# yblin/instant-ngp

Hardware: AMD Instinct MI355X
Metric: training samples/sec + PSNR@30s, NeRF Lego at 1/2/4/8 MI355X (higher is better)
Workload: dtype f16; 1 GPU; NerfNetwork training pass, C2 (configs/nerf/base.json fork: L=4 F=4 T=2^19, density 1x64 + rgb 2x64 fp16 MLPs), fwd+bwd+Adam/EMA; batch_per_gpu=262144, global_batch=262144, parallelism=dp1, launch=hip_graph

## Files before the change

### instant-ngp_amd/csrc/engine.hip

```cpp
#include <algorithm>
#include <cmath>
#include <cstring>
#include <memory>
#include <string>

#include "../../include/ngp_engine.h"
#include "common.h"
#include "engine_internal.h"
#include "grid_scatter.h"
#include "grid.h"
#include "json.h"
#include "mlp.h"
#include "optimizer.h"
#include "profiler.h"
#include "training.h"

static_assert(ngp::DENSITY_LAYOUT_ROW0 == ngp::MLP_LAYOUT_ROW0, "the row-0 density layout of mlp.h and engine_internal.h");

namespace ngp {

int device_cu_count() {
	static int cached = -1;
	if (cached < 0) {
		int dev = 0;
		NGP_HIP(hipGetDevice(&dev));
		NGP_HIP(hipDeviceGetAttribute(&cached, hipDeviceAttributeMultiprocessorCount, dev));
	}
	return cached;
}

struct DevBuf {
	void* p = nullptr;
	size_t bytes = 0;
	uint64_t* epoch = nullptr;
	void* get(size_t need) {
		if (need > bytes) {
			if (p) NGP_HIP(hipFree(p));
			p = nullptr;
			NGP_HIP(hipMalloc(&p, need));
			NGP_HIP(hipMemset(p, 0, need));
			bytes = need;
			if (epoch) ++*epoch;
		}
		return p;
	}
	~DevBuf() { if (p) (void)hipFree(p); }
};

struct Pcg32 {
	uint64_t state = 0x853c49e6748fea9bULL, inc = 0xda3e39cb94b95bdbULL;
	static constexpr uint64_t MULT = 0x5851f42d4c957f2dULL;
	Pcg32(uint64_t initstate, uint64_t initseq = 1u) {
		state = 0u; inc = (initseq << 1u) | 1u; next_uint(); state += initstate; next_uint();
	}
	uint32_t next_uint() {
		uint64_t old = state;
		state = old * MULT + inc;
		uint32_t xs = (uint32_t)(((old >> 18u) ^ old) >> 27u), rot = (uint32_t)(old >> 59u);
		return (xs >> rot) | (xs << ((~rot + 1u) & 31));
	}
	float next_float() { uint32_t u = (next_uint() >> 9) | 0x3f800000u; float f; memcpy(&f, &u, 4); return f - 1.0f; }
	void advance(uint64_t delta) {
		uint64_t cm = MULT, cp = inc, am = 1u, ap = 0u;
		while (delta > 0) {
			if (delta & 1) { am *= cm; ap = ap * cm + cp; }
			cp = (cm + 1) * cp; cm *= cm; delta /= 2;
		}
		state = am * state + ap;
	}
	void uniform(size_t n, float* out, float lo, float hi) {
		Pcg32 r = *this;
		for (size_t k = 0; k < n; ++k) out[k] = r.next_float() * (hi - lo) + lo;
		advance(n);
	}
};

static void init_mlp(const MlpDims& d, Pcg32& rng, float* p, float scale) {
	for (uint32_t l = 0; l <= d.n_hidden; ++l) {
		const uint32_t in = d.layer_in(l), out = d.layer_out(l);
		const float s = sqrtf(6.0f / (float)(in + out)) * scale;
		rng.uniform((size_t)in * out, p + d.layer_off(l), -s, s);
	}
}

static GridDesc parse_grid(uint32_t n_dims, const Json& j) {
	const std::string ot = j.string_or("otype", "HashGrid");
	NGP_CHECK(iequals(ot, "HashGrid") || iequals(ot, "DenseGrid") || iequals(ot, "Grid"),
	          "encoding: HashGrid and DenseGrid are implemented (got " + ot + ")");
	const std::string type = j.string_or("type", iequals(ot, "DenseGrid") ? "Dense" : "Hash");
	NGP_CHECK(iequals(type, "Hash") || iequals(type, "Dense"), "encoding: grid type Hash or Dense (got " + type + ")");
	NGP_CHECK(iequals(j.string_or("interpolation", "Linear"), "Linear"), "encoding: only linear interpolation is implemented");
	GridDesc g;
	grid_desc_init(g, n_dims, (uint32_t)j.number_or("n_levels", 16), (uint32_t)j.number_or("n_features_per_level", 2),
	               iequals(type, "Dense") ? GRID_LOG2_DENSE : (uint32_t)j.number_or("log2_hashmap_size", 19),
	               (uint32_t)j.number_or("base_resolution", 16), (float)j.number_or("per_level_scale", 2.0));
	return g;
}

static uint32_t parse_mlp_hidden(const Json& j, uint32_t* width) {
	const std::string ot = j.string_or("otype", "FullyFusedMLP");
	NGP_CHECK(iequals(ot, "FullyFusedMLP") || iequals(ot, "CutlassMLP") || iequals(ot, "MegakernelMLP"),
	          "network: only FullyFusedMLP-shaped networks are implemented (got " + ot + ")");
	NGP_CHECK(iequals(j.string_or("activation", "ReLU"), "ReLU"), "network: only ReLU hidden activation is implemented");
	NGP_CHECK(iequals(j.string_or("output_activation", "None"), "None"), "network: only output_activation None is implemented");
	*width = (uint32_t)j.number_or("n_neurons", 64);
	return (uint32_t)j.number_or("n_hidden_layers", 2);
}

}

using namespace ngp;

struct ngp_ctx {
	uint32_t n;
	const float* input;
	uint32_t input_stride;
	bool use_inference_params;
	uint64_t generation;
	bool density_only = false;
};

namespace ngp {
struct BwdExtra {
	float* dL_dinput = nullptr;
	uint32_t dinput_stride = 0;
	float dinput_scale = 1.f;
	bool density_only = false;
	const f16* ddens = nullptr;
	uint32_t ddens_stride = 0;
	bool inference = false;
};
}

struct ngp_model {
	bool nerf = true;
	GridDesc grid;
	uint32_t n_pos_dims = 3, n_dir_dims = 3, n_extra_dims = 0, dir_offset = 4, n_input_dims = 3, n_output_dims = 4;
	uint32_t enc_width = 16;
	NerfMlpPlan nplan;
	MlpPlan mplan;
	uint64_t mlp0_params = 0, mlp1_params = 0, grid_params = 0, n_params = 0;
	FragDesc* d_descs = nullptr;
	uint32_t* d_fragmap = nullptr;
	bool frags_current = false;
	uint32_t n_all_frags = 0;
	DevBuf frags, frags_inf, enc, denc, slabs, scatter_ws, out_ws, dl_ws, dsh_ws, dl1_ws;
	int grid_backward_mode = 0;
	uint32_t win_debug = 0;
	ScatterPlan sc_plan;
	uint32_t sc_plan_n = 0;
	bool sc_prepared = false;
	bool sc_hist_done = false;
	bool frags_async = false;
	uint32_t overlap = 0;
	bool fused_hist = true;
	bool fuse_infer = true;
	bool fuse_slabs = true;
	bool fuse_opt = true;
	bool fuse_mlp_opt = true;
	bool grid_bricks = false;
	hipStream_t side = nullptr;
	hipEvent_t ev_fork = nullptr, ev_join = nullptr, ev_frags = nullptr, ev_mlp = nullptr, ev_red = nullptr;
	f16 *params = nullptr, *inference_params = nullptr, *gradients = nullptr;
	void (*inference_hook)(void*, hipStream_t) = nullptr;
	void* inference_hook_ctx = nullptr;
	void sync_inference(hipStream_t s) { if (inference_hook) inference_hook(inference_hook_ctx, s); }
	float max_level = 1.0f;
	const float* max_level_per_sample = nullptr;
	bool grads_valid = true;
	const BwdParts* bwd_parts = nullptr;
	bool parts_ok(uint32_t n) const {
		return use_sorted(n) && fuse_slabs && !(overlap & 4) && !grid_bricks && grid.n_features >= 2;
	}
	uint64_t generation = 0;
	uint64_t ws_epoch = 0;
	std::unique_ptr<ngp_ctx> last_ctx;

	ngp_model() {
		for (DevBuf* b : {&frags, &frags_inf, &enc, &denc, &slabs, &scatter_ws, &out_ws, &dl_ws, &dsh_ws, &dl1_ws}) b->epoch = &ws_epoch;
	}

	~ngp_model() {
		if (d_descs) (void)hipFree(d_descs);
		if (d_fragmap) (void)hipFree(d_fragmap);
		for (hipEvent_t e : {ev_fork, ev_join, ev_frags, ev_mlp, ev_red})
			if (e) (void)hipEventDestroy(e);
		if (side) (void)hipStreamDestroy(side);
	}
	void reserve(uint32_t n) {
		enc.get((size_t)n * enc_width * sizeof(f16));
		denc.get((size_t)n * enc_width * sizeof(f16));
		const uint32_t blocks = nerf ? nerf_mlp_train_blocks(n) : mlp_train_blocks(n);
		slabs.get((size_t)blocks * n_matrix() * sizeof(float));
		frags.get((size_t)n_all_frags * 1024);
		frags_inf.get((size_t)n_all_frags * 1024);
		if (use_sorted(n)) {
			sorted_workspace(n);
			ensure_side_stream();
		}
	}
	void ensure_side_stream() {
		if (side) return;
		NGP_HIP(hipStreamCreateWithFlags(&side, hipStreamNonBlocking));
		NGP_HIP(hipEventCreateWithFlags(&ev_fork, hipEventDisableTiming));
		NGP_HIP(hipEventCreateWithFlags(&ev_join, hipEventDisableTiming));
		NGP_HIP(hipEventCreateWithFlags(&ev_frags, hipEventDisableTiming));
		NGP_HIP(hipEventCreateWithFlags(&ev_mlp, hipEventDisableTiming));
		NGP_HIP(hipEventCreateWithFlags(&ev_red, hipEventDisableTiming));
	}
	bool use_sorted(uint32_t n) const { return grid_backward_mode == 3 || (grid_backward_mode == 0 && n >= 4096); }
	bool grad32_ok(uint32_t n) const { return use_sorted(n) && fuse_slabs && !(overlap & 4) && grid.n_features >= 2; }
	bool side_prepare(uint32_t n) const { return use_sorted(n) && (overlap & 1); }
	const ScatterPlan& sc_plan_for(uint32_t n) {
		if (sc_plan_n != n) {
			sc_plan = make_scatter_plan(grid, n, grid_bricks);
			sc_plan_n = n;
			fb_dirty = true;
		}
		return sc_plan;
	}
	bool fb_dirty = true;
	void clear_brick_fallback(hipStream_t s, void* ws) {
		if (!fb_dirty) return;
		if (sc_plan.bk.LD) NGP_HIP(hipMemsetAsync((char*)ws + sc_plan.off_fb, 0, sc_plan.total - sc_plan.off_fb, s));
		fb_dirty = false;
	}
	void* sorted_workspace(uint32_t n) { return scatter_ws.get(sc_plan_for(n).total); }
	void prepare_grid_backward_async(hipStream_t s, uint32_t n, const float* in, uint32_t stride) {
		if (!side_prepare(n)) return;
		ensure_side_stream();
		void* ws = sorted_workspace(n);
		clear_brick_fallback(s, ws);
		GridBwdArgs b{n, in, stride, nullptr, 0, AoS, nullptr, max_level, max_level_per_sample};
		NGP_HIP(hipEventRecord(ev_fork, s));
		NGP_HIP(hipStreamWaitEvent(side, ev_fork, 0));
		if ((overlap & 2) && !frags_current) {
			prep(side, false);
			NGP_HIP(hipEventRecord(ev_frags, side));
			frags_async = true;
		}
		{
			ProfScope ps("grid_bwd_prepare", side);
			grid_scatter_prepare(grid, b, sc_plan, ws, side);
		}
		NGP_HIP(hipEventRecord(ev_join, side));
		sc_prepared = true;
	}

	const std::vector<FragDesc>& descs() const { return nerf ? nplan.descs : mplan.descs; }
	uint64_t grid_offset() const { return mlp0_params + mlp1_params; }
	uint64_t n_matrix() const { return mlp0_params + mlp1_params; }

	void finalize() {
		grid_params = grid.n_params();
		n_params = mlp0_params + mlp1_params + grid_params;
		const auto& d = descs();
		n_all_frags = (uint32_t)d.size();
		NGP_HIP(hipMalloc(&d_descs, d.size() * sizeof(FragDesc)));
		NGP_HIP(hipMemcpy(d_descs, d.data(), d.size() * sizeof(FragDesc), hipMemcpyHostToDevice));
		std::vector<uint32_t> map(2 * n_matrix(), ~0u);
		for (uint32_t f = 0; f < n_all_frags; ++f)
			for (uint32_t lane = 0; lane < 64; ++lane)
				for (uint32_t j = 0; j < 8; ++j) {
					const FragDesc& q = d[f];
					const uint32_t h = lane >> 5, r = 32 * q.tile + (lane & 31);
					const uint32_t k = q.perm ? 16 * q.step + 8 * (j >> 2) + 4 * h + (j & 3) : 16 * q.step + 8 * h + j;
					uint64_t pi;
					if (!q.transposed) {
						if (!(r < q.out_dim && k < q.in_dim)) continue;
						pi = q.woff + (uint64_t)r * q.in_dim + k;
					} else {
						if (!(r < q.in_dim && k < q.out_dim)) continue;
						pi = q.woff + (uint64_t)k * q.in_dim + r;
					}
					NGP_CHECK(pi < n_matrix() && map[2 * pi + q.transposed] == ~0u, "fragment map: parameter mapped twice");
					map[2 * pi + q.transposed] = (f * 64 + lane) * 8 + j;
				}
		NGP_HIP(hipMalloc(&d_fragmap, map.size() * sizeof(uint32_t)));
		NGP_HIP(hipMemcpy(d_fragmap, map.data(), map.size() * sizeof(uint32_t), hipMemcpyHostToDevice));
	}
	void require_params(bool inference) const {
		NGP_CHECK(inference ? inference_params != nullptr : params != nullptr,
		          "model has no parameters: call ngp_model_set_params or create a trainer first");
	}
	const f16* pick(bool inference) const { return inference ? inference_params : params; }
	bool fused_encoding_ok() const {
		return nerf && !max_level_per_sample && nerf_mlp_fused_encoding_ok(grid, enc_width) && nplan.enc_steps == 1 &&
		       nplan.d_hidden == 1 && nplan.r_hidden >= 1 && nplan.r_hidden <= 3;
	}
	bool fused_inference_ok() const { return fuse_infer && fused_encoding_ok(); }
	f16x8* prep(hipStream_t s, bool inference) {
		f16x8* f = (f16x8*)(inference ? frags_inf : frags).get((size_t)n_all_frags * 1024);
		if (inference) sync_inference(s);
		ProfScope ps("prepare_frags", s);
		prepare_frags(d_descs, n_all_frags, pick(inference), f, s);
		if (!inference) frags_current = true;
		return f;
	}
	void encode(hipStream_t s, uint32_t n, const float* in, uint32_t stride, f16* out, uint32_t out_stride, uint32_t layout, bool inference,
	            bool want_hist = false) {
		if (inference) sync_inference(s);
		GridFwdArgs a{n, in, stride, pick(inference) + grid_offset(), out, out_stride, layout, max_level, max_level_per_sample};
		if (enc_width > grid.n_levels * grid.n_features && layout == AoS && !grid_forward_rows_ok(grid, a)) {
			NGP_HIP(hipMemsetAsync(out, 0, (size_t)n * out_stride * sizeof(f16), s));
		}
		sc_hist_done = false;
		GridHist h;
		const bool fuse = want_hist && fused_hist && use_sorted(n) && !sc_prepared && grid_forward_rows_ok(grid, a) &&
		                  scatter_hist(grid, sc_plan_for(n), sorted_workspace(n), h);
		ProfScope ps("grid_forward", s);
		grid_forward(grid, a, s, fuse ? &h : nullptr);
		sc_hist_done = fuse;
	}
	void run_mlp(hipStream_t s, MlpMode mode, uint32_t n, const float* in, uint32_t stride, const f16* encbuf, f16* out,
	             uint32_t out_stride, uint32_t out_layout, const f16* dL, uint32_t dL_stride, f16* dL_denc, float* slab,
	             bool inference, const BwdExtra* ex = nullptr, f16* dL_dsh = nullptr) {
		f16x8* f;
		if (frags_async && !inference) {
			f = (f16x8*)frags.p;
			NGP_HIP(hipStreamWaitEvent(s, ev_frags, 0));
			frags_async = false;
		} else if (!inference && frags_current && frags.p) {
			f = (f16x8*)frags.p;
		} else {
			f = prep(s, inference);
		}
		if (nerf) {
			NerfMlpArgs a{};
			a.n = n; a.enc = encbuf; a.enc_stride = enc_width; a.coords = in; a.coord_stride = stride; a.dir_offset = dir_offset;
			a.frags = f; a.n_frags = n_all_frags; a.out = out; a.out_stride = out_stride; a.out_layout = out_layout;
			a.dL_dout = dL; a.dL_stride = dL_stride; a.dL_denc = dL_denc; a.denc_stride = enc_width; a.dw_slab = slab;
			a.n_matrix = (uint32_t)n_matrix(); a.density_woff = 0; a.rgb_woff = (uint32_t)mlp0_params;
			a.dL_dsh = dL_dsh;
			if (ex) { a.dL_ddens = ex->ddens; a.ddens_stride = ex->ddens_stride; }
			if (mode == MLP_INFER_ENC) {
				if (inference) sync_inference(s);
				a.table = pick(inference) + grid_offset(); a.max_level = max_level; a.gc = make_grid_const(grid);
			}
			ProfScope ps(mode == MLP_TRAIN ? "mlp_train" : mode == MLP_DENSITY ? "mlp_density"
			             : mode == MLP_INFER_ENC ? "mlp_infer_enc"
			             : mode == MLP_DENSITY_TRAIN ? "mlp_density_train" : "mlp_infer", s);
			nerf_mlp_run(nplan, mode, a, s);
		} else {
			MlpArgs a{};
			a.n = n; a.enc = encbuf; a.enc_stride = enc_width; a.frags = f; a.n_frags = n_all_frags;
			a.out = out; a.out_stride = out_stride; a.out_layout = out_layout; a.dL_dout = dL; a.dL_stride = dL_stride;
			a.dL_denc = dL_denc; a.denc_stride = enc_width; a.dw_slab = slab; a.n_matrix = (uint32_t)n_matrix();
			ProfScope ps(mode == MLP_TRAIN ? "mlp_train" : "mlp_infer", s);
			mlp_run(mplan, mode == MLP_DENSITY ? MLP_INFER : mode, a, s);
		}
	}
	void train_pass(hipStream_t s, uint32_t n, const float* in, uint32_t stride, const f16* encbuf, f16* out, uint32_t out_stride,
	                const void* dL, uint32_t dL_stride, int grad_mode, const BwdExtra& ex = BwdExtra{}, const FusedAdam* fopt = nullptr) {
		NGP_CHECK(gradients || grad_mode == NGP_GRAD_IGNORE, "model has no gradient buffer: call ngp_model_set_params");
		NGP_CHECK(!ex.density_only || (nerf && encbuf), "density backward: a NerfNetwork with its encoding");
		f16* dL_denc = (f16*)denc.get((size_t)n * enc_width * sizeof(f16));
		const uint32_t blocks = nerf ? nerf_mlp_train_blocks(n) : mlp_train_blocks(n);
		float* slab = (float*)slabs.get((size_t)blocks * n_matrix() * sizeof(float));
		f16* dsh = ex.dL_dinput && nerf && !ex.density_only ? (f16*)dsh_ws.get((size_t)n * 16 * sizeof(f16)) : nullptr;
		NGP_CHECK(encbuf, "train_pass: the encoding buffer");
		const MlpMode mode = ex.density_only ? MLP_DENSITY_TRAIN : MLP_TRAIN;
		run_mlp(s, mode, n, in, stride, encbuf, out, out_stride, AoS, (const f16*)dL, dL_stride, dL_denc, slab, ex.inference, &ex,
		        dsh);
		auto input_gradient = [&]() {
			if (!ex.dL_dinput) return;
			ProfScope ps("input_gradient", s);
			if (ex.inference) sync_inference(s);
			InputGradArgs ia{n, in, stride, pick(ex.inference) + grid_offset(), dL_denc, enc_width, max_level, max_level_per_sample, dsh,
			                 dir_offset, ex.dL_dinput, ex.dinput_stride, ex.dinput_scale};
			grid_input_gradient(grid, ia, s);
		};
		if (grad_mode == NGP_GRAD_IGNORE) {
			input_gradient();
			return;
		}
		grads_valid = !(fopt && (fopt->rec || fopt->g32));
		const bool ovl = use_sorted(n) && (overlap & 4);
		const bool fused = use_sorted(n) && !ovl && fuse_slabs && !ex.density_only;
		const uint32_t n_red = ex.density_only ? (uint32_t)mlp0_params : (uint32_t)n_matrix();
		SlabJob sj;
		sj.slabs = slab; sj.n_slabs = blocks; sj.n = n_red; sj.grad = gradients; sj.stride = (uint32_t)n_matrix();
		sj.accumulate = grad_mode == NGP_GRAD_ACCUMULATE;
		FusedAdam f32store;
		if (fopt && fopt->g32) {
			NGP_CHECK(fused && grad_mode == NGP_GRAD_OVERWRITE && !fopt->rec, "fp32 gradient store: fused slab reduction");
			sj.grad32 = fopt->g32;
			f32store.g32 = fopt->g32 + grid_offset();
			fopt = &f32store;
		}
		hipStream_t rs = s;
		if (ovl) {
			ensure_side_stream();
			NGP_HIP(hipEventRecord(ev_mlp, s));
			NGP_HIP(hipStreamWaitEvent(side, ev_mlp, 0));
			rs = side;
		}
		if (!fused) {
			ProfScope ps("reduce_slabs", rs);
			reduce_slabs(slab, blocks, n_red, gradients, grad_mode == NGP_GRAD_ACCUMULATE, rs, (uint32_t)n_matrix());
		}
		if (ovl) NGP_HIP(hipEventRecord(ev_red, side));
		GridBwdArgs b{n, in, stride, dL_denc, enc_width, AoS, gradients + grid_offset(), max_level, max_level_per_sample};
		FusedAdam fmlp;
		if (fopt && fopt->mlp_n) {
			NGP_CHECK(fused && grad_mode == NGP_GRAD_OVERWRITE && fopt->mlp_n == n_matrix(), "fused MLP update: slab reduction not fused");
			fmlp = *fopt;
			fmlp.frags = frags_current ? (f16*)frags.p : nullptr;
			fmlp.fragmap = d_fragmap;
			fopt = &fmlp;
		}
		scatter_grid_grad(s, b, grad_mode != NGP_GRAD_ACCUMULATE, fused ? &sj : nullptr, fopt);
		if (ovl) NGP_HIP(hipStreamWaitEvent(s, ev_red, 0));
		input_gradient();
	}
	void scatter_grid_grad(hipStream_t s, GridBwdArgs b, bool overwrite, const SlabJob* slab = nullptr, const FusedAdam* fopt = nullptr) {
		if (use_sorted(b.n)) {
			void* ws = sorted_workspace(b.n);
			clear_brick_fallback(s, ws);
			if (sc_prepared) {
				NGP_HIP(hipStreamWaitEvent(s, ev_join, 0));
				sc_prepared = false;
			} else {
				ProfScope ps("grid_bwd_prepare", s);
				grid_scatter_prepare(grid, b, sc_plan, ws, s, sc_hist_done);
			}
			sc_hist_done = false;
			ProfScope ps(fopt && fopt->rec ? "grid_backward_adam" : "grid_backward_sorted", s);
			grid_backward_sorted(grid, b, sc_plan, ws, s, overwrite, win_debug, slab, fopt,
			                     bwd_parts && !sc_plan.bk.LD && !(fopt && fopt->rec) ? bwd_parts : nullptr);
			return;
		}
		NGP_CHECK(!slab && !fopt, "fused slab reduction / optimizer need the sorted grid backward");
		if (overwrite) {
			ProfScope ps("grid_grad_zero", s);
			NGP_HIP(hipMemsetAsync(b.grad, 0, grid_params * sizeof(f16), s));
		}
		ProfScope ps("grid_backward", s);
		grid_backward(grid, b, s);
	}
};

struct ngp_trainer {
	ngp_model* model = nullptr;
	AdamConfig cfg;
	uint32_t step = 0;
	uint64_t n = 0;
	void* arena = nullptr;
	float *w32 = nullptr, *m1 = nullptr, *m2 = nullptr, *ema32 = nullptr;
	f16 *w16 = nullptr, *inf16 = nullptr, *g16 = nullptr;
	uint32_t* steps = nullptr;
	float* bias_tab = nullptr;
	AdamRec* rec = nullptr;
	bool inf_stale = false;
	bool w32_stale = false;
	void sync_w32() {
		if (!rec || !w32_stale) return;
		require_full_state("full-precision weights");
		NGP_HIP(hipDeviceSynchronize());
		adam_rec_weights((uint32_t)n, rec, w32, false, nullptr);
		NGP_HIP(hipDeviceSynchronize());
		w32_stale = false;
	}
	void materialize(hipStream_t s, bool force = false) {
		if (!rec || (!inf_stale && !force)) return;
		require_full_state("inference (EMA) parameters");
		AdamState st{w32, w16, g16, nullptr, nullptr, nullptr, nullptr, inf16, nullptr, nullptr, nullptr, 0, nullptr, rec};
		ema_materialize(cfg, (uint32_t)n, step, st, s);
		inf_stale = false;
	}
	static void materialize_hook(void* self, hipStream_t s) { ((ngp_trainer*)self)->materialize(s); }
	void bind_model() {
		ngp_model_set_params(model, w16, cfg.ema_decay > 0.f ? inf16 : w16, g16);
		if (rec) { model->inference_hook = materialize_hook; model->inference_hook_ctx = this; }
	}
	uint32_t* ctl = nullptr;
	ngp_allreduce_fn allreduce = nullptr;
	void* allreduce_user = nullptr;
	uint32_t world = 1;
	static constexpr uint64_t SHARD_PAD = 2048;
	uint32_t dp_rank = 0;
	bool dp_rank_known = false;
	bool shard_opt = true;
	bool shards_valid = true;
	float* g32 = nullptr;
	uint64_t g32_count = 0;
	uint64_t n_pad = 0;
	uint32_t dp_parts = 1;
	bool dp_wire16 = false;
	std::vector<uint64_t> pb;
	hipStream_t xs = nullptr;
	hipEvent_t ev_part[BwdParts::MAX] = {}, ev_xs = nullptr;
	struct PartStep {
		hipStream_t s = nullptr;
		ngp::Exchange e;
		float loss_scale = 1.f;
		const uint32_t* step_base = nullptr;
		uint32_t step_add = 0;
		bool wire16 = false, overlap = false;
		uint32_t issued = 0;
		int rc = NGP_OK;
	} ps_;
	BwdParts bparts;
	~ngp_trainer() {
		if (arena) (void)hipFree(arena);
		if (bias_tab) (void)hipFree(bias_tab);
		if (g32) (void)hipFree(g32);
		for (hipEvent_t ev : ev_part)
			if (ev) (void)hipEventDestroy(ev);
		if (ev_xs) (void)hipEventDestroy(ev_xs);
		if (xs) (void)hipStreamDestroy(xs);
	}
	ngp::Exchange exchange() const {
		ngp::Exchange e;
		e.fn = allreduce; e.user = allreduce_user; e.rank = dp_rank; e.world = world; e.world_factor = (float)world;
		e.rank_known = dp_rank_known;
		return e;
	}
	bool sharded(const ngp::Exchange& e) const {
// ... 62 lines not shown
	}
	static void part_done(void* self, uint32_t j, hipStream_t) { ((ngp_trainer*)self)->issue_part(j); }
	const BwdParts* begin_shard_step(hipStream_t s, float loss_scale, const ngp::Exchange& e, const uint32_t* step_base,
	                                 uint32_t step_add, uint32_t n_batch, bool stores_input) {
		ps_ = PartStep{};
		ps_.s = s; ps_.e = e; ps_.loss_scale = loss_scale; ps_.step_base = step_base; ps_.step_add = step_add;
		ps_.wire16 = dp_wire16;
		ngp_model* m = model;
		if (pb.size() < 3 || !m->parts_ok(n_batch) || !(stores_input || dp_wire16)) return nullptr;
		ensure_exchange_stream();
		ps_.overlap = true;
		const ScatterPlan& p = m->sc_plan_for(n_batch);
		if (p.bk.LD || pb[1] < m->grid_offset()) { ps_.overlap = false; return nullptr; }
		bparts = BwdParts{};
		bparts.k = (uint32_t)pb.size() - 1;
		const uint64_t go = m->grid_offset();
		for (uint32_t j = 0; j < bparts.k; ++j)
			bparts.vb_end[j] = j + 1 == bparts.k ? p.n_buckets : scatter_bucket_at_param(m->grid, p, pb[j + 1] > go ? pb[j + 1] - go : 0);
		bparts.after = part_done;
		bparts.user = this;
		return &bparts;
	}
	int shard_step(bool stored) {
		PartStep& q = ps_;
		hipStream_t s = q.s;
		ngp_model* m = model;
		if (q.issued == 0) {
			q.overlap = false;
			if (!stored && !q.wire16) widen_f16(g16, g32, n, s);
		}
		while (q.rc == NGP_OK && q.issued + 1 < pb.size()) issue_part((uint32_t)pb.size() - 2 - q.issued);
		if (q.rc != NGP_OK) return NGP_ERROR;
		if (q.overlap) {
			NGP_HIP(hipEventRecord(ev_xs, xs));
			NGP_HIP(hipStreamWaitEvent(s, ev_xs, 0));
		}
		if (!mlp_owned() && m->n_matrix() > 0) m->prep(s, false);
		inf_stale = w32_stale = true;
		if (q.e.world > 1) shards_valid = false;
		return NGP_OK;
	}
	void sync_device_step() { NGP_HIP(hipMemcpy(ctl, &step, sizeof(uint32_t), hipMemcpyHostToDevice)); }
	void run_step(hipStream_t s, float loss_scale, const uint32_t* step_base, uint32_t step_add, uint64_t n_first = 0) {
		ngp_model* m = model;
		const bool own = m->params == w16;
		AdamState st{w32, w16, g16, m1, m2, steps, ema32, inf16,
		             own && m->frags_current ? (f16*)m->frags.p : nullptr, m->d_fragmap, step_base, step_add,
		             step_base ? (const AdamConfig*)(ctl + CTL_CFG) : nullptr, rec, bias_tab};
		ProfScope ps("optimizer", s);
		adam_ema_update(cfg, (uint32_t)(n_first ? n_first : n), (uint32_t)m->n_matrix(), loss_scale, st, s);
		if (rec) inf_stale = w32_stale = true;
	}
	bool fused_update_ok(uint32_t n_batch) const {
		const ngp_model* m = model;
		return rec && !allreduce && m->fuse_opt && m->use_sorted(n_batch) && m->grid.n_features >= 2 && m->n_matrix() % 4 == 0 &&
		       m->grid_offset() % 2 == 0 && m->params == w16 && m->gradients == g16;
	}
	FusedAdam fused_update(float loss_scale, uint32_t n_batch) const {
		FusedAdam fa;
		const uint64_t go = model->grid_offset();
		fa.w16 = w16 + go; fa.rec = rec + go / 2;
		fa.loss_scale = loss_scale; fa.cfg = cfg; fa.step_add = step;
		fa.bias_tab = bias_tab;
		if (mlp_opt_in_backward(n_batch)) {
			fa.mlp_n = (uint32_t)model->n_matrix();
			fa.mlp_w16 = w16;
			fa.mlp_rec = rec;
		}
		return fa;
	}
	bool mlp_opt_in_backward(uint32_t n_batch) const {
		const ngp_model* m = model;
		return m->fuse_mlp_opt && m->fuse_slabs && !(m->overlap & 4) && m->use_sorted(n_batch) && m->n_matrix() > 0;
	}
	void mlp_step_done() {
		if (rec) inf_stale = w32_stale = true;
	}
};

struct ngp_graph {
	hipGraph_t graph = nullptr;
	hipGraphExec_t exec = nullptr;
	ngp_trainer* trainer = nullptr;
	uint32_t steps_per_launch = 1;
	uint64_t ws_epoch = 0;
	bool shards_stale = false;
	bool g16_stale = false;
	void launched() {
		trainer->step += steps_per_launch;
		if (steps_per_launch && trainer->rec) trainer->inf_stale = trainer->w32_stale = true;
		if (shards_stale) trainer->shards_valid = false;
		if (g16_stale) trainer->model->grads_valid = false;
	}
	~ngp_graph() {
		if (exec) (void)hipGraphExecDestroy(exec);
		if (graph) (void)hipGraphDestroy(graph);
	}
};

__global__ static void k_one_hot_f16(f16* out, uint32_t n, uint32_t width, uint32_t dim, f16 v) {
	const uint64_t i = blockIdx.x * (uint64_t)blockDim.x + threadIdx.x;
	if (i < (uint64_t)n * width) out[i] = (i % width) == dim ? v : (f16)0.f;
}
static void fill_one_hot_f16(f16* out, uint32_t n, uint32_t width, uint32_t dim, float v, hipStream_t s) {
	k_one_hot_f16<<<div_round_up((uint64_t)n * width, 256), 256, 0, s>>>(out, n, width, dim, (f16)v);
	NGP_HIP(hipGetLastError());
}

static thread_local std::string g_last_error;

#define NGP_TRY(...)                        \
	try {                                   \
		__VA_ARGS__;                        \
		return NGP_OK;                      \
	} catch (const std::exception& e) {     \
		g_last_error = e.what();            \
		return NGP_ERROR;                   \
	}

#define NGP_ARG(cond)                                                          \
	do {                                                                       \
		if (!(cond)) { g_last_error = "invalid argument: " #cond; return NGP_INVALID; } \
	} while (0)

static hipStream_t S(void* s) { return (hipStream_t)s; }

namespace ngp {
void set_last_error(const char* msg) { g_last_error = msg; }
}

extern "C" {

const char* ngp_last_error(void) { return g_last_error.c_str(); }
const char* ngp_version(void) { return "ngp-mi355x 0.1 (gfx950)"; }

int ngp_device_info(int* cu_count, char* name, size_t name_len) {
	NGP_TRY({
		int dev = 0;
		NGP_HIP(hipGetDevice(&dev));
		hipDeviceProp_t p;
		NGP_HIP(hipGetDeviceProperties(&p, dev));
		if (cu_count) *cu_count = p.multiProcessorCount;
		if (name && name_len) { strncpy(name, p.gcnArchName, name_len - 1); name[name_len - 1] = 0; }
	});
}

int ngp_malloc(void** ptr, size_t bytes) { NGP_ARG(ptr); NGP_TRY(NGP_HIP(hipMalloc(ptr, bytes))); }
int ngp_free(void* ptr) { NGP_TRY(NGP_HIP(hipFree(ptr))); }
int ngp_memcpy(void* dst, const void* src, size_t bytes, int kind) { NGP_TRY(NGP_HIP(hipMemcpy(dst, src, bytes, (hipMemcpyKind)kind))); }
int ngp_stream_synchronize(void* stream) { NGP_TRY(NGP_HIP(hipStreamSynchronize(S(stream)))); }

static void apply_env_options(ngp_model* m) {
	const char* env = getenv("NGP_MODEL_OPTS");
	if (!env || !*env) return;
	std::string all = env;
	size_t pos = 0;
	while (pos < all.size()) {
		size_t end = all.find(',', pos);
		if (end == std::string::npos) end = all.size();
		const std::string kv = all.substr(pos, end - pos);
		pos = end + 1;
		if (kv.empty()) continue;
		const size_t eq = kv.find('=');
		NGP_CHECK(eq != std::string::npos, "NGP_MODEL_OPTS: expected key=value, got " + kv);
		if (ngp_model_set_option(m, kv.substr(0, eq).c_str(), atof(kv.c_str() + eq + 1)) != NGP_OK) throw Error(g_last_error);
	}
}

int ngp_nerf_network_create(uint32_t n_pos_dims, uint32_t n_dir_dims, uint32_t n_extra_dims, uint32_t dir_offset,
                            const char* pos_encoding_json, const char* dir_encoding_json, const char* density_network_json,
                            const char* rgb_network_json, ngp_model** out) {
	NGP_ARG(out && pos_encoding_json && density_network_json && rgb_network_json);
	NGP_TRY({
		auto m = std::make_unique<ngp_model>();
		m->nerf = true;
		NGP_CHECK(n_pos_dims == 3, "NerfNetwork: n_pos_dims must be 3");
		NGP_CHECK(n_dir_dims == 3, "NerfNetwork: n_dir_dims must be 3");
		NGP_CHECK(n_extra_dims == 0, "NerfNetwork: extra dims (latent codes) are not implemented");
		m->n_pos_dims = n_pos_dims; m->n_dir_dims = n_dir_dims; m->n_extra_dims = n_extra_dims; m->dir_offset = dir_offset;
		m->grid = parse_grid(3, Json::parse(pos_encoding_json));
		if (dir_encoding_json) {
			Json d = Json::parse(dir_encoding_json);
			const Json* sh = &d;
			if (iequals(d.string_or("otype", ""), "Composite")) sh = &d["nested"].arr.at(0);
			NGP_CHECK(iequals(sh->string_or("otype", ""), "SphericalHarmonics") && (int)sh->number_or("degree", 4) == 4,
			          "NerfNetwork: dir_encoding must be SphericalHarmonics of degree 4");
		}
		uint32_t wd, wr;
		const uint32_t dh = parse_mlp_hidden(Json::parse(density_network_json), &wd);
		const uint32_t rh = parse_mlp_hidden(Json::parse(rgb_network_json), &wr);
		NGP_CHECK(wd == wr, "NerfNetwork: density and rgb networks must share n_neurons");
		m->enc_width = next_multiple(m->grid.n_levels * m->grid.n_features, 16);
		m->nplan = make_nerf_mlp_plan(m->enc_width, wd, dh, rh);
		m->mlp0_params = m->nplan.density.n_params();
		m->mlp1_params = m->nplan.rgb.n_params();
		m->n_input_dims = dir_offset + n_dir_dims + n_extra_dims;
		m->n_output_dims = 4;
		m->finalize();
		apply_env_options(m.get());
		*out = m.release();
	});
}

int ngp_network_with_input_encoding_create(uint32_t n_input_dims, uint32_t n_output_dims, const char* encoding_json,
                                           const char* network_json, ngp_model** out) {
	NGP_ARG(out && encoding_json && network_json);
	NGP_TRY({
		auto m = std::make_unique<ngp_model>();
		m->nerf = false;
		NGP_CHECK(n_input_dims == 2 || n_input_dims == 3, "NetworkWithInputEncoding: 2 or 3 input dims");
		NGP_CHECK(n_output_dims >= 1 && n_output_dims <= 16, "NetworkWithInputEncoding: 1..16 outputs");
		m->n_pos_dims = n_input_dims; m->n_input_dims = n_input_dims; m->n_output_dims = n_output_dims;
		m->grid = parse_grid(n_input_dims, Json::parse(encoding_json));
		uint32_t w;
		const uint32_t hid = parse_mlp_hidden(Json::parse(network_json), &w);
		m->enc_width = next_multiple(m->grid.n_levels * m->grid.n_features, 16);
		m->mplan = make_mlp_plan(m->enc_width, w, hid, 16);
		m->mlp0_params = m->mplan.mlp.n_params();
		m->mlp1_params = 0;
		m->finalize();
		apply_env_options(m.get());
		*out = m.release();
	});
}

void ngp_model_destroy(ngp_model* m) { delete m; }
uint64_t ngp_model_n_params(const ngp_model* m) { return m ? m->n_params : 0; }
uint64_t ngp_model_n_matrix_params(const ngp_model* m) { return m ? m->n_matrix() : 0; }
uint32_t ngp_model_input_width(const ngp_model* m) { return m ? m->n_input_dims : 0; }
uint32_t ngp_model_padded_output_width(const ngp_model* m) { return m ? 16 : 0; }
uint32_t ngp_model_output_width(const ngp_model* m) { return m ? m->n_output_dims : 0; }

int ngp_model_param_layout(const ngp_model* m, ngp_param_layout* o) {
	NGP_ARG(m && o);
	NGP_TRY({
		memset(o, 0, sizeof(*o));
		o->density_mlp_offset = 0; o->density_mlp_params = m->mlp0_params;
		o->rgb_mlp_offset = m->mlp0_params; o->rgb_mlp_params = m->mlp1_params;
		o->grid_offset = m->grid_offset(); o->grid_params = m->grid_params;
		o->grid_dims = m->grid.n_dims; o->grid_levels = m->grid.n_levels; o->grid_features = m->grid.n_features;
		o->grid_log2_hashmap = m->grid.log2_hashmap; o->grid_base_resolution = m->grid.base_resolution;
		o->grid_per_level_scale = m->grid.per_level_scale;
		memcpy(o->grid_level_offsets, m->grid.offsets, sizeof(o->grid_level_offsets));
		memcpy(o->grid_resolution, m->grid.resolution, sizeof(o->grid_resolution));
		memcpy(o->grid_scale, m->grid.scale, sizeof(o->grid_scale));
		o->encoding_width = m->enc_width;
	});
}

int ngp_model_set_params(ngp_model* m, void* params, void* inference_params, void* gradients) {
	NGP_ARG(m);
	NGP_TRY({
		m->inference_hook = nullptr;
		m->inference_hook_ctx = nullptr;
		m->params = (f16*)params;
		m->frags_current = false;
		m->inference_params = (f16*)(inference_params ? inference_params : params);
		m->gradients = (f16*)gradients;
	});
}

int ngp_model_initialize_params(const ngp_model* m, uint64_t seed, float* p, float scale) {
	NGP_ARG(m && p);
	NGP_TRY({
		Pcg32 rng(seed);
		if (m->nerf) {
			init_mlp(m->nplan.density, rng, p, scale);
			init_mlp(m->nplan.rgb, rng, p + m->mlp0_params, scale);
		} else {
			init_mlp(m->mplan.mlp, rng, p, scale);
		}
		rng.uniform(m->grid_params, p + m->grid_offset(), -1e-4f * scale, 1e-4f * scale);
	});
}

int ngp_model_set_max_level(ngp_model* m, float max_level, const float* per_sample) {
	NGP_ARG(m);
	NGP_TRY({ m->max_level = max_level; m->max_level_per_sample = per_sample; });
}

int ngp_model_set_option(ngp_model* m, const char* key, double value) {
	NGP_ARG(m && key);
	NGP_TRY({
		const std::string k = key;
		if (k == "grid_backward_mode") {
			NGP_CHECK(value == 0 || value == 1 || value == 3, "grid_backward_mode must be 0 (auto), 1 (direct), 3 (bucketed)");
			m->grid_backward_mode = (int)value;
		} else if (k == "overlap") {
			NGP_CHECK(value >= 0 && value <= 15, "overlap is a bitmask in [0, 15]");
			m->overlap = (uint32_t)value;
		} else if (k == "fused_hist") {
			m->fused_hist = value != 0;
		} else if (k == "fuse_infer") {
			m->fuse_infer = value != 0;
		} else if (k == "fuse_slabs") {
			m->fuse_slabs = value != 0;
		} else if (k == "fuse_opt") {
			m->fuse_opt = value != 0;
		} else if (k == "fuse_mlp_opt") {
			m->fuse_mlp_opt = value != 0;
		} else if (k == "grid_bricks") {
			m->grid_bricks = value != 0;
			m->sc_plan_n = 0;
		} else if (k == "win_debug") {
			m->win_debug = (uint32_t)value;
		} else {
			throw Error("unknown model option: " + k);
		}
		++m->ws_epoch;
	});
}

int ngp_model_query(const ngp_model* m, const char* key, double* value) {
	NGP_ARG(m && key && value);
	NGP_TRY({
		const std::string k = key;
		if (k == "grid_brick_levels") *value = m->sc_plan_n ? (double)(m->sc_plan.bk.LD - m->sc_plan.bk.LB) : 0.0;
		else throw Error("unknown model query: " + k);
	});
}

int ngp_model_reserve(ngp_model* m, uint32_t n) {
	NGP_ARG(m);
	NGP_TRY({ m->reserve(n); });
}

uint64_t ngp_model_workspace_epoch(const ngp_model* m) { return m ? m->ws_epoch : 0; }

int ngp_model_workspace(ngp_model* m, const char* name, void** ptr, uint64_t* bytes) {
	NGP_ARG(m && name && ptr);
	NGP_TRY({
		const std::string k(name);
		DevBuf* b = k == "encoding" ? &m->enc : k == "dL_dencoding" ? &m->denc : k == "dw_slabs" ? &m->slabs
		          : k == "dL_dsh" ? &m->dsh_ws : nullptr;
		NGP_CHECK(b, "ngp_model_workspace: unknown workspace '" + k + "' (encoding, dL_dencoding, dL_dsh, dw_slabs)");
		*ptr = b->p;
		if (bytes) *bytes = b->bytes;
	});
}

int ngp_encoding_forward(ngp_model* m, void* stream, uint32_t n, const float* input, uint32_t input_stride, void* output,
                         uint32_t output_stride, uint32_t output_layout, int use_inference_params) {
	NGP_ARG(m && (n == 0 || (input && output)) && output_layout <= 1);
	NGP_TRY({
		m->require_params(use_inference_params);
		m->encode(S(stream), n, input, input_stride, (f16*)output, output_stride, output_layout, use_inference_params);
	});
}

int ngp_encoding_backward(ngp_model* m, void* stream, uint32_t n, const float* input, uint32_t input_stride,
                          const void* dL_doutput, uint32_t dL_stride, uint32_t dL_layout, float* dL_dinput,
                          uint32_t dL_dinput_stride, int grad_mode) {
	NGP_ARG(m && (n == 0 || (input && dL_doutput)) && dL_layout <= 1 && grad_mode >= 0 && grad_mode <= NGP_GRAD_IGNORE);
	NGP_ARG(!dL_dinput || (dL_layout == NGP_LAYOUT_AOS && dL_dinput_stride >= m->grid.n_dims));
	NGP_TRY({
		if (n == 0) return NGP_OK;
		m->require_params(false);
		if (grad_mode != NGP_GRAD_IGNORE) {
			NGP_CHECK(m->gradients, "model has no gradient buffer");
			GridBwdArgs b{n, input, input_stride, (const f16*)dL_doutput, dL_stride, dL_layout, m->gradients + m->grid_offset(),
			              m->max_level, m->max_level_per_sample};
			m->scatter_grid_grad(S(stream), b, grad_mode != NGP_GRAD_ACCUMULATE);
		}
		if (dL_dinput) {
			ProfScope ps("input_gradient", S(stream));
			InputGradArgs ia{n, input, input_stride, m->params + m->grid_offset(), (const f16*)dL_doutput, dL_stride, m->max_level,
			                 m->max_level_per_sample, nullptr, 0, dL_dinput, dL_dinput_stride, 1.f};
			grid_input_gradient(m->grid, ia, S(stream));
		}
	});
}

}
int ngp::density_impl(ngp_model* m, void* stream, uint32_t n, const float* input, uint32_t input_stride, void* output,
                      uint32_t output_stride, uint32_t output_layout, int use_inference_params) {
	NGP_TRY({
		NGP_CHECK(m->nerf, "density() is a NerfNetwork method");
		if (n == 0) return NGP_OK;
		m->require_params(use_inference_params);
		f16* e = (f16*)m->enc.get((size_t)n * m->enc_width * sizeof(f16));
		m->encode(S(stream), n, input, input_stride, e, m->enc_width, AoS, use_inference_params);
		m->run_mlp(S(stream), MLP_DENSITY, n, input, input_stride, e, (f16*)output, output_stride, output_layout, nullptr, 0,
		           nullptr, nullptr, use_inference_params);
		m->generation++;
	});
}
extern "C" {

int ngp_inference(ngp_model* m, void* stream, uint32_t n, const float* input, uint32_t input_stride, void* output,
                  uint32_t output_stride, uint32_t output_layout, int use_inference_params) {
	NGP_ARG(m && (n == 0 || (input && output)) && (output_layout <= 1 || (output_layout == NGP_LAYOUT_AOS_RGBD && m->nerf &&
	                                                                        output_stride >= 4)));
	NGP_TRY({
		if (n == 0) return NGP_OK;
		m->require_params(use_inference_params);
		if (m->fused_inference_ok()) {
			m->run_mlp(S(stream), MLP_INFER_ENC, n, input, input_stride, nullptr, (f16*)output, output_stride, output_layout,
			           nullptr, 0, nullptr, nullptr, use_inference_params);
		} else {
			f16* e = (f16*)m->enc.get((size_t)n * m->enc_width * sizeof(f16));
			m->encode(S(stream), n, input, input_stride, e, m->enc_width, AoS, use_inference_params);
			m->run_mlp(S(stream), MLP_INFER, n, input, input_stride, e, (f16*)output, output_stride, output_layout, nullptr, 0,
			           nullptr, nullptr, use_inference_params);
		}
		m->generation++;
	});
}

int ngp_density(ngp_model* m, void* stream, uint32_t n, const float* input, uint32_t input_stride, void* output,
                uint32_t output_stride, uint32_t output_layout, int use_inference_params) {
	NGP_ARG(m && (n == 0 || (input && output)) && output_layout <= 1);
	return ngp::density_impl(m, stream, n, input, input_stride, output, output_stride, output_layout, use_inference_params);
}

int ngp_forward(ngp_model* m, void* stream, uint32_t n, const float* input, uint32_t input_stride, void* output,
                uint32_t output_stride, int use_inference_params, ngp_ctx** ctx) {
	NGP_ARG(m && ctx && (n == 0 || input));
	NGP_TRY({
		m->require_params(use_inference_params);
		f16* e = (f16*)m->enc.get((size_t)(n ? n : 1) * m->enc_width * sizeof(f16));
		m->generation++;
		if (n) {
			m->encode(S(stream), n, input, input_stride, e, m->enc_width, AoS, use_inference_params);
			if (output)
				m->run_mlp(S(stream), MLP_INFER, n, input, input_stride, e, (f16*)output, output_stride, AoS, nullptr, 0, nullptr,
				           nullptr, use_inference_params);
		}
		*ctx = new ngp_ctx{n, input, input_stride, (bool)use_inference_params, m->generation};
	});
}

static int check_dinput(const ngp_model* m, float* dL_dinput, uint32_t stride) {
	if (!dL_dinput) return NGP_OK;
	const uint32_t need = m->nerf ? m->dir_offset + 3 : m->n_pos_dims;
	if (stride < need) {
		g_last_error = "dL_dinput: stride smaller than the rows the input gradient writes";
		return NGP_INVALID;
	}
	return NGP_OK;
}

int ngp_backward(ngp_model* m, void* stream, ngp_ctx* ctx, const void* dL_doutput, uint32_t dL_stride, float* dL_dinput,
                 uint32_t dL_dinput_stride, int grad_mode) {
	NGP_ARG(m && ctx && (ctx->n == 0 || dL_doutput) && grad_mode >= 0 && grad_mode <= NGP_GRAD_IGNORE);
	if (check_dinput(m, dL_dinput, dL_dinput_stride) != NGP_OK) return NGP_INVALID;
	NGP_TRY({
		NGP_CHECK(ctx->generation == m->generation,
		          "backward: the forward context is stale (another forward/inference ran on this model since)");
		NGP_CHECK(!ctx->density_only, "backward: this context is from density_forward (use density_backward)");
		if (ctx->n == 0) return NGP_OK;
		BwdExtra ex;
		ex.dL_dinput = dL_dinput; ex.dinput_stride = dL_dinput_stride;
		ex.inference = ctx->use_inference_params;
		m->train_pass(S(stream), ctx->n, ctx->input, ctx->input_stride, (const f16*)m->enc.p, nullptr, 0, dL_doutput, dL_stride,
		              grad_mode, ex);
	});
}

int ngp_density_forward(ngp_model* m, void* stream, uint32_t n, const float* input, uint32_t input_stride, void* output,
                        uint32_t output_stride, int use_inference_params, ngp_ctx** ctx) {
	NGP_ARG(m && ctx && (n == 0 || input) && (!output || output_stride >= 16));
	NGP_TRY({
		NGP_CHECK(m->nerf, "density_forward is a NerfNetwork method");
		m->require_params(use_inference_params);
		f16* e = (f16*)m->enc.get((size_t)(n ? n : 1) * m->enc_width * sizeof(f16));
		m->generation++;
		if (n) {
			m->encode(S(stream), n, input, input_stride, e, m->enc_width, AoS, use_inference_params);
			if (output)
				m->run_mlp(S(stream), MLP_DENSITY, n, input, input_stride, e, (f16*)output, output_stride, AoS, nullptr, 0, nullptr,
				           nullptr, use_inference_params);
		}
		*ctx = new ngp_ctx{n, input, input_stride, (bool)use_inference_params, m->generation, true};
	});
}

int ngp_density_backward(ngp_model* m, void* stream, ngp_ctx* ctx, const void* dL_doutput, uint32_t dL_stride, float* dL_dinput,
                         uint32_t dL_dinput_stride, int grad_mode) {
	NGP_ARG(m && ctx && (ctx->n == 0 || dL_doutput) && dL_stride >= 16 && dL_stride % 4 == 0 && grad_mode >= 0 &&
	        grad_mode <= NGP_GRAD_IGNORE && (!dL_dinput || dL_dinput_stride >= 3));
	NGP_TRY({
		NGP_CHECK(m->nerf, "density_backward is a NerfNetwork method");
		NGP_CHECK(ctx->generation == m->generation,
		          "density_backward: the forward context is stale (another forward/inference ran on this model since)");
		NGP_CHECK(ctx->density_only, "density_backward: this context is from forward (use backward)");
		if (ctx->n == 0) return NGP_OK;
		BwdExtra ex;
		ex.dL_dinput = dL_dinput; ex.dinput_stride = dL_dinput_stride;
		ex.density_only = true; ex.ddens = (const f16*)dL_doutput; ex.ddens_stride = dL_stride;
		ex.inference = ctx->use_inference_params;
		m->train_pass(S(stream), ctx->n, ctx->input, ctx->input_stride, (const f16*)m->enc.p, nullptr, 0, nullptr, 0, grad_mode, ex);
	});
}

int ngp_input_gradient(ngp_model* m, void* stream, uint32_t dim, uint32_t n, const float* input, uint32_t input_stride,
                       float* d_dinput, uint32_t d_dinput_stride, float backprop_scale) {
	NGP_ARG(m && (n == 0 || (input && d_dinput)) && dim < 16 && backprop_scale != 0.f);
	if (check_dinput(m, d_dinput, d_dinput_stride) != NGP_OK) return NGP_INVALID;
	NGP_TRY({
		if (n == 0) return NGP_OK;
		m->require_params(false);
		hipStream_t s = S(stream);
		f16* e = (f16*)m->enc.get((size_t)n * m->enc_width * sizeof(f16));
		f16* dl = (f16*)m->dl1_ws.get((size_t)n * 16 * sizeof(f16));
		m->generation++;
		m->encode(s, n, input, input_stride, e, m->enc_width, AoS, false);
		fill_one_hot_f16(dl, n, 16, dim, backprop_scale, s);
		BwdExtra ex;
		ex.dL_dinput = d_dinput; ex.dinput_stride = d_dinput_stride; ex.dinput_scale = 1.f / backprop_scale;
		m->train_pass(s, n, input, input_stride, e, nullptr, 0, dl, 16, NGP_GRAD_IGNORE, ex);
	});
}

void ngp_ctx_destroy(ngp_ctx* ctx) { delete ctx; }

int ngp_forward_backward(ngp_model* m, void* stream, uint32_t n, const float* input, uint32_t input_stride, void* output,
                         uint32_t output_stride, const void* dL_doutput, uint32_t dL_stride, int grad_mode) {
	return ngp::forward_backward_with(m, stream, n, input, input_stride, output, output_stride, dL_doutput, dL_stride, grad_mode,
	                                  nullptr);
}
}

int ngp::forward_backward_with(ngp_model* m, void* stream, uint32_t n, const float* input, uint32_t input_stride, void* output,
                               uint32_t output_stride, const void* dL_doutput, uint32_t dL_stride, int grad_mode,
                               const FusedAdam* fopt) {
	NGP_ARG(m && (n == 0 || (input && dL_doutput)));
	NGP_TRY({
		if (n == 0) return NGP_OK;
		m->require_params(false);
		f16* e = (f16*)m->enc.get((size_t)n * m->enc_width * sizeof(f16));
		m->generation++;
		m->prepare_grid_backward_async(S(stream), n, input, input_stride);
		m->encode(S(stream), n, input, input_stride, e, m->enc_width, AoS, false, true);
		m->train_pass(S(stream), n, input, input_stride, e, (f16*)output, output_stride, dL_doutput, dL_stride, grad_mode,
		              BwdExtra{}, fopt);
	});
}
extern "C" {

static void parse_optimizer(const Json& j, AdamConfig& c) {
	const std::string ot = j.string_or("otype", "Adam");
	if (iequals(ot, "Ema")) {
		c.ema_decay = (float)j.number_or("decay", 0.99);
		parse_optimizer(j["nested"], c);
	} else if (iequals(ot, "ExponentialDecay")) {
		c.decay_start = (uint32_t)j.number_or("decay_start", 0);
		c.decay_interval = (uint32_t)j.number_or("decay_interval", 10000);
		c.decay_base = (float)j.number_or("decay_base", 0.1);
		parse_optimizer(j["nested"], c);
	} else if (iequals(ot, "Adam")) {
		c.lr = (float)j.number_or("learning_rate", 1e-3);
		c.beta1 = (float)j.number_or("beta1", 0.9);
		c.beta2 = (float)j.number_or("beta2", 0.999);
		c.eps = (float)j.number_or("epsilon", 1e-8);
		c.l2 = (float)j.number_or("l2_reg", 1e-8);
	} else {
		throw Error("optimizer: unsupported otype " + ot + " (Ema / ExponentialDecay / Adam implemented)");
	}
}

int ngp_trainer_create(ngp_model* m, const char* optimizer_json, uint64_t seed, ngp_trainer** out) {
	NGP_ARG(m && out);
	NGP_TRY({
		auto t = std::make_unique<ngp_trainer>();
		t->model = m;
		if (optimizer_json) parse_optimizer(Json::parse(optimizer_json), t->cfg);
		if (const char* e = getenv("NGP_EMA_CLOSED_FORM")) t->cfg.ema_closed_form = atoi(e) != 0;
		NGP_HIP(hipMalloc(&t->bias_tab, (size_t)BIAS_TAB_CAP * 2 * sizeof(float)));
		adam_bias_table(t->bias_tab, t->cfg.beta1, t->cfg.beta2, nullptr);
		NGP_HIP(hipDeviceSynchronize());
		const uint64_t n = m->n_params;
		t->n = n;
		auto al = [](size_t b) { return (b + 255) / 256 * 256; };
		const size_t b32 = al(n * 4), b16 = al((n + ngp_trainer::SHARD_PAD) * 2);
		bool lazy = n >= (1ull << 20);
		if (const char* e = getenv("NGP_LAZY_EMA")) lazy = atoi(e) != 0;
		lazy = lazy && n % 4 == 0;
		const size_t brec = al((n + ngp_trainer::SHARD_PAD) / 2 * sizeof(AdamRec));
		const size_t total = b32 + (lazy ? brec : 4 * b32) + 3 * b16 + 256 ;
		NGP_HIP(hipMalloc(&t->arena, total));
		char* p = (char*)t->arena;
		t->w32 = (float*)p; p += b32;
		if (lazy) {
			t->rec = (AdamRec*)p; p += brec;
		} else {
			t->m1 = (float*)p; p += b32;
			t->m2 = (float*)p; p += b32;
			t->ema32 = (float*)p; p += b32;
			t->steps = (uint32_t*)p; p += b32;
		}
		t->w16 = (f16*)p; p += b16;
		t->inf16 = (f16*)p; p += b16;
		t->g16 = (f16*)p; p += b16;
		t->ctl = (uint32_t*)p; p += 256;
		NGP_HIP(hipMemset(t->arena, 0, total));
		std::vector<float> host(n);
		if (ngp_model_initialize_params(m, seed, host.data(), 1.0f) != NGP_OK) throw Error(g_last_error);
		*out = t.release();
		if (ngp_trainer_set_params_full_precision(*out, host.data(), n) != NGP_OK) throw Error(g_last_error);
	});
}

void ngp_trainer_destroy(ngp_trainer* t) {
	if (!t) return;
	if (t->model && t->model->params == t->w16) ngp_model_set_params(t->model, nullptr, nullptr, nullptr);
	delete t;
}

int ngp_trainer_optimizer_step(ngp_trainer* t, void* stream, float loss_scale) {
	NGP_ARG(t && loss_scale > 0.f);
	NGP_TRY({
		t->run_step(S(stream), loss_scale, nullptr, t->step);
		t->step++;
	});
}

int ngp_loss_evaluate(int loss_type, void* stream, uint32_t n, uint32_t dims, const void* output, uint32_t output_stride,
                      const float* target, uint32_t target_stride, float loss_scale, void* dL_doutput, uint32_t dL_stride,
                      float* values, float* loss_sum) {
	NGP_ARG(loss_type >= 0 && (n == 0 || (output && target && dL_doutput)));
// ... 403 lines not shown
```

### instant-ngp_amd/csrc/grid.h

```cpp
#pragma once
#include "common.h"

namespace ngp {

struct GridDesc {
	uint32_t n_dims = 3, n_levels = 16, n_features = 2, log2_hashmap = 19, base_resolution = 16;
	float per_level_scale = 2.0f;
	uint32_t offsets[33] = {};
	float scale[32] = {};
	uint32_t resolution[32] = {};
	uint32_t n_entries() const { return offsets[n_levels]; }
	uint64_t n_params() const { return (uint64_t)offsets[n_levels] * n_features; }
};

constexpr uint32_t GRID_LOG2_DENSE = 31;
void grid_desc_init(GridDesc& g, uint32_t D, uint32_t L, uint32_t F, uint32_t log2T, uint32_t Nmin, float b);

enum Layout : uint32_t { AoS = 0, SoA = 1 };

struct GridFwdArgs {
	uint32_t n;
	const float* pos;
	uint32_t pos_stride;
	const f16* table;
	f16* out;
	uint32_t out_stride;
	uint32_t out_layout;
	float max_level;
	const float* max_level_per_sample;
};

struct GridBwdArgs {
	uint32_t n;
	const float* pos;
	uint32_t pos_stride;
	const f16* dL_dy;
	uint32_t dy_stride;
	uint32_t dy_layout;
	f16* grad;
	float max_level;
	const float* max_level_per_sample;
	uint32_t level_begin = 0;
};

struct GridHist {
	uint32_t* hist;
	uint32_t B, n_chunks, chunk;
	uint32_t vb_base[33];
	uint32_t brick_first = 0, brick_levels = 0, n_bricks = 0, brick_cells = 8, bricks_per_dim = 0, brick_vb0 = 0;
};

void grid_forward(const GridDesc& g, const GridFwdArgs& a, hipStream_t stream, const GridHist* hist = nullptr);
bool grid_forward_rows_ok(const GridDesc& g, const GridFwdArgs& a);
void grid_backward(const GridDesc& g, const GridBwdArgs& a, hipStream_t stream);

struct InputGradArgs {
	uint32_t n;
	const float* pos; uint32_t pos_stride;
	const f16* table;
	const f16* dL_dy; uint32_t dy_stride;
	float max_level; const float* max_level_per_sample;
	const f16* dL_dsh;
	uint32_t dir_offset;
	float* out; uint32_t out_stride;
	float out_scale;
};
void grid_input_gradient(const GridDesc& g, const InputGradArgs& a, hipStream_t stream);

struct GridConst {
	uint32_t n_levels, n_features;
	uint32_t offsets[33];
	float scale[32];
	uint32_t resolution[32];
	uint32_t hashed;
};

__device__ __forceinline__ uint32_t grid_index3(uint32_t T, uint32_t res, uint32_t x, uint32_t y, uint32_t z) {
	uint32_t stride = 1, index = 0;
	index += x * stride; stride *= res;
	if (stride <= T) { index += y * stride; stride *= res; }
	if (stride <= T) { index += z * stride; stride *= res; }
	if (T < stride) index = x ^ (y * 2654435761u) ^ (z * 805459861u);
	return index % T;
}

__device__ __forceinline__ uint32_t grid_index2(uint32_t T, uint32_t res, uint32_t x, uint32_t y) {
	uint32_t stride = 1, index = 0;
	index += x * stride; stride *= res;
	if (stride <= T) { index += y * stride; stride *= res; }
	if (T < stride) index = x ^ (y * 2654435761u);
	return index % T;
}

template <uint32_t D>
__device__ __forceinline__ uint32_t corner_index(const GridConst& c, uint32_t l, const uint32_t* base, uint32_t corner) {
	const uint32_t x = base[0] + (corner & 1u);
	const uint32_t y = base[1] + ((corner >> 1) & 1u);
	if ((c.hashed >> l) & 1u) {
		const uint32_t mask = c.offsets[l + 1] - c.offsets[l] - 1u;
		if constexpr (D == 3) {
			const uint32_t z = base[2] + ((corner >> 2) & 1u);
			return c.offsets[l] + ((x ^ (y * 2654435761u) ^ (z * 805459861u)) & mask);
		} else {
			return c.offsets[l] + ((x ^ (y * 2654435761u)) & mask);
		}
	}
	const uint32_t res = c.resolution[l];
	uint32_t idx;
	if constexpr (D == 3) {
		const uint32_t z = base[2] + ((corner >> 2) & 1u);
		idx = x + res * (y + res * z);
	} else {
		idx = x + res * y;
	}
	const uint32_t T = c.offsets[l + 1] - c.offsets[l];
	if (__builtin_expect(idx >= T, 0)) idx %= T;
	return c.offsets[l] + idx;
}

template <uint32_t D>
__device__ __forceinline__ void corner_indices(const GridConst& c, uint32_t l, const uint32_t* base, uint32_t* idx) {
	const uint32_t res = c.resolution[l], T = c.offsets[l + 1] - c.offsets[l];
	uint64_t vol = res;
#pragma unroll
	for (uint32_t d = 1; d < D; ++d) vol *= res;
	bool fast = !((c.hashed >> l) & 1u) && vol <= T;
#pragma unroll
	for (uint32_t d = 0; d < D; ++d) fast = fast && base[d] < res;
	if (__builtin_expect(fast, 1)) {
		const uint32_t r2 = res * res;
		const uint32_t i0 = D == 3 ? base[0] + res * (base[1] + res * base[2]) : base[0] + res * base[1];
#pragma unroll
		for (uint32_t k = 0; k < (1u << D); ++k) {
			const uint32_t id = i0 + (k & 1u) + (((k >> 1) & 1u) ? res : 0u) + ((D == 3 && ((k >> 2) & 1u)) ? r2 : 0u);
			idx[k] = c.offsets[l] + min(id, id - T);
		}
	} else {
#pragma unroll
		for (uint32_t k = 0; k < (1u << D); ++k) idx[k] = corner_index<D>(c, l, base, k);
	}
}

template <uint32_t F> struct GridVec;
template <> struct GridVec<1> { typedef f16 T; typedef f16 __attribute__((ext_vector_type(2), aligned(2))) P; };
template <> struct GridVec<2> { typedef f16x2 T; typedef f16 __attribute__((ext_vector_type(4), aligned(4))) P; };
template <> struct GridVec<4> { typedef f16x4 T; typedef f16 __attribute__((ext_vector_type(8), aligned(8))) P; };
template <> struct GridVec<8> { typedef f16x8 T; typedef f16x8 P; };

#ifndef NGP_GATHER16
#define NGP_GATHER16 0
#endif
template <uint32_t D>
__device__ __forceinline__ void gather_pairs_f2(const uint32_t* idx, const f16* __restrict__ table, f16x2* v);
template <uint32_t D, uint32_t F>
__device__ __forceinline__ void gather_corners(const GridConst& c, uint32_t l, const uint32_t* base, const f16* __restrict__ table,
                                               typename GridVec<F>::T* v) {
	typedef typename GridVec<F>::T V;
	typedef typename GridVec<F>::P P;
	if constexpr (F == 2 && NGP_GATHER16) {
		uint32_t idx[1u << D];
#pragma unroll
		for (uint32_t k = 0; k < (1u << D); ++k) idx[k] = corner_index<D>(c, l, base, k);
		gather_pairs_f2<D>(idx, table, v);
	} else if constexpr (F == 2 || F == 4) {
#pragma unroll
		for (uint32_t k = 0; k < (1u << D); k += 2) {
			const uint32_t i0 = corner_index<D>(c, l, base, k), i1 = corner_index<D>(c, l, base, k + 1);
			const uint32_t lo_i = min(i0, i1);
			if (max(i0, i1) == lo_i + 1u) {
				const P p = *(const P*)(table + (size_t)lo_i * F);
				V lo, hi;
#pragma unroll
				for (uint32_t f = 0; f < F; ++f) { lo[f] = p[f]; hi[f] = p[F + f]; }
				const bool swap = i1 < i0;
				v[k] = swap ? hi : lo;
				v[k + 1] = swap ? lo : hi;
			} else {
				v[k] = *(const V*)(table + (size_t)i0 * F);
				v[k + 1] = *(const V*)(table + (size_t)i1 * F);
			}
		}
	} else {
#pragma unroll
		for (uint32_t k = 0; k < (1u << D); ++k) v[k] = *(const V*)(table + (size_t)corner_index<D>(c, l, base, k) * F);
	}
}
__device__ __forceinline__ f16x2 pick4(const uint32_t (&g)[4], uint32_t i) {
	const uint32_t lo = (i & 1u) ? g[1] : g[0], hi = (i & 1u) ? g[3] : g[2];
	return __builtin_bit_cast(f16x2, (i & 2u) ? hi : lo);
}
template <uint32_t D>
__device__ __forceinline__ void gather_pairs_f2(const uint32_t* idx, const f16* __restrict__ table, f16x2* v) {
	typedef GridVec<2>::P P;
#pragma unroll
	for (uint32_t k = 0; k < (1u << D); k += 2) {
		const uint32_t i0 = idx[k], i1 = idx[k + 1];
		const uint32_t lo_i = min(i0, i1);
		if ((i0 >> 2) == (i1 >> 2)) {
			const uint32_t* gp = (const uint32_t*)(table + (size_t)(i0 & ~3u) * 2);
			typedef uint32_t u32x4g __attribute__((ext_vector_type(4)));
			const u32x4g q = *(const u32x4g*)gp;
			const uint32_t g[4] = {q[0], q[1], q[2], q[3]};
			v[k] = pick4(g, i0 & 3u);
			v[k + 1] = pick4(g, i1 & 3u);
		} else if (max(i0, i1) == lo_i + 1u) {
			const P p = *(const P*)(table + (size_t)lo_i * 2);
			const f16x2 a{p[0], p[1]}, b{p[2], p[3]};
			const bool swap = i1 < i0;
			v[k] = swap ? b : a;
			v[k + 1] = swap ? a : b;
		} else {
			v[k] = *(const f16x2*)(table + (size_t)i0 * 2);
			v[k + 1] = *(const f16x2*)(table + (size_t)i1 * 2);
		}
	}
}

template <uint32_t D, uint32_t F>
__device__ __forceinline__ void gather_corners_at(const uint32_t* idx, const f16* __restrict__ table, typename GridVec<F>::T* v) {
	typedef typename GridVec<F>::T V;
	typedef typename GridVec<F>::P P;
	if constexpr (F == 2 && NGP_GATHER16) {
		gather_pairs_f2<D>(idx, table, v);
	} else if constexpr (F == 2 || F == 4) {
#pragma unroll
		for (uint32_t k = 0; k < (1u << D); k += 2) {
			const uint32_t i0 = idx[k], i1 = idx[k + 1];
			const uint32_t lo_i = min(i0, i1);
			if (max(i0, i1) == lo_i + 1u) {
				const P p = *(const P*)(table + (size_t)lo_i * F);
				V lo, hi;
#pragma unroll
				for (uint32_t f = 0; f < F; ++f) { lo[f] = p[f]; hi[f] = p[F + f]; }
				const bool swap = i1 < i0;
				v[k] = swap ? hi : lo;
				v[k + 1] = swap ? lo : hi;
			} else {
				v[k] = *(const V*)(table + (size_t)i0 * F);
				v[k + 1] = *(const V*)(table + (size_t)i1 * F);
			}
		}
	} else {
#pragma unroll
		for (uint32_t k = 0; k < (1u << D); ++k) v[k] = *(const V*)(table + (size_t)idx[k] * F);
	}
}

template <uint32_t D>
__device__ __forceinline__ float corner_weight(const float* frac, uint32_t corner) {
	float w = 1.0f;
#pragma unroll
	for (uint32_t d = 0; d < D; ++d) w *= ((corner >> d) & 1u) ? frac[d] : 1.0f - frac[d];
	return w;
}

template <uint32_t D>
__device__ __forceinline__ void level_setup(const GridConst& c, uint32_t l, const float* x, float* frac, uint32_t* base) {
#pragma unroll
	for (uint32_t d = 0; d < D; ++d) {
		float p = __builtin_fmaf(c.scale[l], x[d], 0.5f);
		float t = floorf(p);
		base[d] = (uint32_t)(int)t;
		frac[d] = p - t;
	}
}

__device__ __forceinline__ uint32_t brick_of(const GridConst& c, uint32_t f, uint32_t K, uint32_t NB, const float* x) {
	uint32_t id = 0, mul = 1;
#pragma unroll
	for (uint32_t d = 0; d < 3; ++d) {
		const int cell = (int)floorf(__builtin_fmaf(c.scale[f], x[d], 0.5f));
		const int b = cell < 0 ? 0 : min(cell / (int)K, (int)NB - 1);
		id += (uint32_t)b * mul;
		mul *= NB;
	}
	return id;
}

__device__ __forceinline__ void hist_add(uint32_t* h, uint32_t j, uint32_t few_bits) {
	if (few_bits > 4) { atomicAdd(&h[j], 1u); return; }
	uint64_t peers = __ballot(1);
	for (uint32_t b = 0; b < few_bits; ++b) {
		const uint64_t m = __ballot((j >> b) & 1u);
		peers &= ((j >> b) & 1u) ? m : ~m;
	}
	if (__lane_id() == (uint32_t)(__ffsll((unsigned long long)peers) - 1)) atomicAdd(&h[j], (uint32_t)__popcll(peers));
}

GridConst make_grid_const(const GridDesc& g);
int device_cu_count();

}
```

### instant-ngp_amd/csrc/grid.hip

```cpp
#include "grid.h"

#include <algorithm>

#include <cmath>
#include <cstring>

namespace ngp {

void grid_desc_init(GridDesc& g, uint32_t D, uint32_t L, uint32_t F, uint32_t log2T, uint32_t Nmin, float b) {
	NGP_CHECK(D == 2 || D == 3, "GridEncoding: n_dims must be 2 or 3");
	NGP_CHECK(L >= 1 && L <= 32, "GridEncoding: n_levels must be in [1, 32]");
	NGP_CHECK(F == 1 || F == 2 || F == 4 || F == 8, "GridEncoding: n_features_per_level must be 1, 2, 4 or 8");
	NGP_CHECK((log2T >= 4 && log2T <= 28) || log2T == GRID_LOG2_DENSE, "GridEncoding: log2_hashmap_size out of range");
	g = GridDesc{};
	g.n_dims = D; g.n_levels = L; g.n_features = F; g.log2_hashmap = log2T; g.base_resolution = Nmin;
	g.per_level_scale = b;
	const float log2b = log2f(b);
	uint32_t off = 0;
	for (uint32_t l = 0; l < L; ++l) {
		float s = exp2f((float)l * log2b) * (float)Nmin - 1.0f;
		uint32_t res = (uint32_t)ceilf(s) + 1u;
		g.scale[l] = s;
		g.resolution[l] = res;
		const uint32_t max_params = 0xffffffffu / 2;
		uint32_t n;
		if (powf((float)res, (float)D) > (float)max_params) n = max_params;
		else { n = 1; for (uint32_t d = 0; d < D; ++d) n *= res; }
		n = (n + 7u) / 8u * 8u;
		if (n > (1u << log2T)) n = 1u << log2T;
		g.offsets[l] = off;
		off += n;
	}
	g.offsets[L] = off;
}

GridConst make_grid_const(const GridDesc& g) {
	GridConst c;
	c.n_levels = g.n_levels;
	c.n_features = g.n_features;
	memcpy(c.offsets, g.offsets, sizeof(c.offsets));
	memcpy(c.scale, g.scale, sizeof(c.scale));
	memcpy(c.resolution, g.resolution, sizeof(c.resolution));
	c.hashed = 0;
	for (uint32_t l = 0; l < g.n_levels; ++l) {
		const uint32_t T = g.offsets[l + 1] - g.offsets[l];
		uint32_t stride = g.resolution[l];
		for (uint32_t d = 1; d < g.n_dims; ++d)
			if (stride <= T) stride *= g.resolution[l];
		if (T < stride) {
			NGP_CHECK((T & (T - 1)) == 0, "GridEncoding: hashed level size must be a power of two");
			c.hashed |= 1u << l;
		}
	}
	return c;
}

template <uint32_t F> struct FeatVec;
template <> struct FeatVec<1> { typedef f16 T; };
template <> struct FeatVec<2> { typedef f16x2 T; };
template <> struct FeatVec<4> { typedef f16x4 T; };
template <> struct FeatVec<8> { typedef f16x8 T; };

template <uint32_t D, uint32_t F>
__global__ void __launch_bounds__(256) k_grid_forward(const GridConst c, const GridFwdArgs a) {
	typedef typename FeatVec<F>::T V;
	const uint32_t i = blockIdx.x * blockDim.x + threadIdx.x;
	if (i >= a.n) return;
	float x[D];
#pragma unroll
	for (uint32_t d = 0; d < D; ++d) x[d] = a.pos[(size_t)i * a.pos_stride + d];
	const float ml = (a.max_level_per_sample ? a.max_level_per_sample[i] : a.max_level) * (float)c.n_levels;
	for (uint32_t l = 0; l < c.n_levels; ++l) {
		float acc[F];
#pragma unroll
		for (uint32_t f = 0; f < F; ++f) acc[f] = 0.f;
		if (!((float)l >= ml + 1e-3f)) {
			float frac[D]; uint32_t base[D];
			level_setup<D>(c, l, x, frac, base);
			V v[1u << D];
			gather_corners<D, F>(c, l, base, a.table, v);
#pragma unroll
			for (uint32_t k = 0; k < (1u << D); ++k) {
				const float w = corner_weight<D>(frac, k);
				if constexpr (F == 1) acc[0] = __builtin_fmaf(w, (float)v[k], acc[0]);
				else {
#pragma unroll
					for (uint32_t f = 0; f < F; ++f) acc[f] = __builtin_fmaf(w, (float)v[k][f], acc[f]);
				}
			}
		}
#pragma unroll
		for (uint32_t f = 0; f < F; ++f) asm volatile("" : "+v"(acc[f]));
		if (a.out_layout == AoS) {
			V o;
			if constexpr (F == 1) o = (f16)acc[0];
			else {
#pragma unroll
				for (uint32_t f = 0; f < F; ++f) o[f] = (f16)acc[f];
			}
			*(V*)(a.out + (size_t)i * a.out_stride + l * F) = o;
		} else {
#pragma unroll
			for (uint32_t f = 0; f < F; ++f) a.out[(size_t)(l * F + f) * a.out_stride + i] = (f16)acc[f];
		}
	}
}

#ifndef NGP_FWD_FASTIDX
#define NGP_FWD_FASTIDX 1
#endif
template <uint32_t D, uint32_t F, bool HIST>
__global__ void __launch_bounds__(HIST ? 512 : 256) k_grid_forward_rows(const GridConst c, const GridFwdArgs a, const GridHist h) {
	typedef typename FeatVec<F>::T V;
	constexpr uint32_t MAXL = 32 / F;
	extern __shared__ __attribute__((aligned(16))) uint32_t hl[];
	if constexpr (HIST) {
		for (uint32_t j = threadIdx.x; j < h.vb_base[c.n_levels]; j += blockDim.x) hl[j] = 0;
		__syncthreads();
	}
	const uint32_t i = blockIdx.x * blockDim.x + threadIdx.x;
	if (i < a.n) {
	float x[D];
#pragma unroll
	for (uint32_t d = 0; d < D; ++d) x[d] = a.pos[(size_t)i * a.pos_stride + d];
	const float ml = (a.max_level_per_sample ? a.max_level_per_sample[i] : a.max_level) * (float)c.n_levels;
	if constexpr (HIST && D == 3) {
		if (h.brick_levels) atomicAdd(&hl[h.brick_vb0 + brick_of(c, h.brick_levels - 1, h.brick_cells, h.bricks_per_dim, x)], 1u);
	}
	f16 row[32];
#pragma unroll
	for (uint32_t l = 0; l < MAXL; ++l) {
		float acc[F];
#pragma unroll
		for (uint32_t f = 0; f < F; ++f) acc[f] = 0.f;
		const bool active = l < c.n_levels && !((float)l >= ml + 1e-3f);
		const bool count = HIST && !(l >= h.brick_first && l < h.brick_levels);
		if (count && l < c.n_levels && !active) {
			float frac[D]; uint32_t base[D];
			level_setup<D>(c, l, x, frac, base);
#pragma unroll
			for (uint32_t k = 0; k < (1u << D); ++k)
				atomicAdd(&hl[h.vb_base[l] + ((corner_index<D>(c, l, base, k) - c.offsets[l]) >> h.B)], 1u);
		}
		if (active) {
			float frac[D]; uint32_t base[D];
			level_setup<D>(c, l, x, frac, base);
			V v[1u << D];
			if constexpr (NGP_FWD_FASTIDX && F >= 4) {
				uint32_t cidx[1u << D];
				corner_indices<D>(c, l, base, cidx);
				if (count) {
#pragma unroll
					for (uint32_t k = 0; k < (1u << D); ++k) atomicAdd(&hl[h.vb_base[l] + ((cidx[k] - c.offsets[l]) >> h.B)], 1u);
				}
				gather_corners_at<D, F>(cidx, a.table, v);
			} else {
				if (count) {
#pragma unroll
					for (uint32_t k = 0; k < (1u << D); ++k)
						atomicAdd(&hl[h.vb_base[l] + ((corner_index<D>(c, l, base, k) - c.offsets[l]) >> h.B)], 1u);
				}
				gather_corners<D, F>(c, l, base, a.table, v);
			}
#pragma unroll
			for (uint32_t k = 0; k < (1u << D); ++k) {
				const float w = corner_weight<D>(frac, k);
				if constexpr (F == 1) acc[0] = __builtin_fmaf(w, (float)v[k], acc[0]);
				else {
#pragma unroll
					for (uint32_t f = 0; f < F; ++f) acc[f] = __builtin_fmaf(w, (float)v[k][f], acc[f]);
				}
			}
		}
#pragma unroll
		for (uint32_t f = 0; f < F; ++f) {
			asm volatile("" : "+v"(acc[f]));
			row[l * F + f] = (f16)acc[f];
		}
	}
	f16x8* dst = (f16x8*)(a.out + (size_t)i * a.out_stride);
#pragma unroll
	for (uint32_t q = 0; q < 4; ++q) {
		if (8 * q >= a.out_stride) break;
		dst[q] = f16x8{row[8 * q], row[8 * q + 1], row[8 * q + 2], row[8 * q + 3],
		               row[8 * q + 4], row[8 * q + 5], row[8 * q + 6], row[8 * q + 7]};
	}
	}
	if constexpr (HIST) {
		__syncthreads();
		for (uint32_t j = threadIdx.x; j < h.vb_base[c.n_levels]; j += blockDim.x) h.hist[(size_t)blockIdx.x * h.vb_base[c.n_levels] + j] = hl[j];
	}
}

template <uint32_t D, uint32_t F>
__global__ void __launch_bounds__(256) k_grid_backward(const GridConst c, const GridBwdArgs a) {
	constexpr uint32_t P = F >= 2 ? F / 2 : 1;
	const uint32_t t = blockIdx.x * blockDim.x + threadIdx.x;
	const uint32_t i = t / (2 * P);
	const uint32_t sub = t % (2 * P);
	const uint32_t xbit = sub / P, pair = sub % P;
	if (i >= a.n) return;
	float x[D];
#pragma unroll
	for (uint32_t d = 0; d < D; ++d) x[d] = a.pos[(size_t)i * a.pos_stride + d];
	const float ml = (a.max_level_per_sample ? a.max_level_per_sample[i] : a.max_level) * (float)c.n_levels;
	for (uint32_t l = a.level_begin; l < c.n_levels; ++l) {
		if ((float)l > ml + 1e-3f) break;
		float g0, g1;
		const uint32_t f0 = l * F + (F >= 2 ? 2 * pair : 0);
		if (a.dy_layout == AoS) {
			if constexpr (F >= 2) {
				f16x2 g = *(const f16x2*)(a.dL_dy + (size_t)i * a.dy_stride + f0);
				g0 = (float)g[0]; g1 = (float)g[1];
			} else {
				g0 = (float)a.dL_dy[(size_t)i * a.dy_stride + f0]; g1 = 0.f;
			}
		} else {
			g0 = (float)a.dL_dy[(size_t)f0 * a.dy_stride + i];
			g1 = F >= 2 ? (float)a.dL_dy[(size_t)(f0 + 1) * a.dy_stride + i] : 0.f;
		}
		float frac[D]; uint32_t base[D];
		level_setup<D>(c, l, x, frac, base);
#pragma unroll
		for (uint32_t q = 0; q < (1u << (D - 1)); ++q) {
			const uint32_t k = xbit | (q << 1);
			const float w = corner_weight<D>(frac, k);
			const uint32_t e = corner_index<D>(c, l, base, k);
			if constexpr (F >= 2) {
				atomic_add_f16x2(a.grad + (size_t)e * F + 2 * pair, f16x2{to_f16(w * g0), to_f16(w * g1)});
			} else {
				const size_t idx = e;
				f16x2 v = (idx & 1) ? f16x2{(f16)0.f, to_f16(w * g0)} : f16x2{to_f16(w * g0), (f16)0.f};
				atomic_add_f16x2(a.grad + (idx & ~(size_t)1), v);
			}
		}
	}
}

bool grid_forward_rows_ok(const GridDesc& g, const GridFwdArgs& a) {
	return a.out_layout == AoS && a.out_stride % 8 == 0 && a.out_stride <= 32 && g.n_levels * g.n_features <= a.out_stride &&
	       ((uintptr_t)a.out & 15) == 0;
}

template <uint32_t D>
static void launch_fwd(uint32_t F, const GridConst& c, const GridFwdArgs& a, hipStream_t s, bool rows, const GridHist* h) {
	const dim3 grid(div_round_up(a.n, 256)), block(256);
	if (h) {
		NGP_CHECK(rows && h->chunk == 512, "grid forward histogram: needs the row kernel and 512-sample chunks");
		const dim3 grid_h(div_round_up(a.n, 512));
		NGP_CHECK(grid_h.x == h->n_chunks, "grid forward histogram: chunk count mismatch");
		const size_t lds = (size_t)h->vb_base[c.n_levels] * 4;
		auto go = [&](auto kern) {
			ensure_dynamic_lds((const void*)kern, lds);
			kern<<<grid_h, 512, lds, s>>>(c, a, *h);
		};
		switch (F) {
			case 1: go(k_grid_forward_rows<D, 1, true>); return;
			case 2: go(k_grid_forward_rows<D, 2, true>); return;
			case 4: go(k_grid_forward_rows<D, 4, true>); return;
			case 8: go(k_grid_forward_rows<D, 8, true>); return;
			default: throw Error("GridEncoding: unsupported F");
		}
	}
	const GridHist none{};
	if (rows) {
		switch (F) {
			case 1: k_grid_forward_rows<D, 1, false><<<grid, block, 0, s>>>(c, a, none); return;
			case 2: k_grid_forward_rows<D, 2, false><<<grid, block, 0, s>>>(c, a, none); return;
			case 4: k_grid_forward_rows<D, 4, false><<<grid, block, 0, s>>>(c, a, none); return;
			case 8: k_grid_forward_rows<D, 8, false><<<grid, block, 0, s>>>(c, a, none); return;
			default: throw Error("GridEncoding: unsupported F");
		}
	}
	switch (F) {
		case 1: k_grid_forward<D, 1><<<grid, block, 0, s>>>(c, a); break;
		case 2: k_grid_forward<D, 2><<<grid, block, 0, s>>>(c, a); break;
		case 4: k_grid_forward<D, 4><<<grid, block, 0, s>>>(c, a); break;
		case 8: k_grid_forward<D, 8><<<grid, block, 0, s>>>(c, a); break;
		default: throw Error("GridEncoding: unsupported F");
	}
}

template <uint32_t D>
static void launch_bwd(uint32_t F, const GridConst& c, const GridBwdArgs& a, hipStream_t s) {
	const uint32_t P = F >= 2 ? F / 2 : 1;
	const dim3 grid(div_round_up((uint64_t)a.n * 2 * P, 256)), block(256);
	switch (F) {
		case 1: k_grid_backward<D, 1><<<grid, block, 0, s>>>(c, a); break;
		case 2: k_grid_backward<D, 2><<<grid, block, 0, s>>>(c, a); break;
		case 4: k_grid_backward<D, 4><<<grid, block, 0, s>>>(c, a); break;
		case 8: k_grid_backward<D, 8><<<grid, block, 0, s>>>(c, a); break;
		default: throw Error("GridEncoding: unsupported F");
	}
}

template <uint32_t D, uint32_t F>
__global__ void __launch_bounds__(256) k_input_grad(const GridConst c, const InputGradArgs a) {
	typedef typename FeatVec<F>::T V;
	const uint32_t i = blockIdx.x * blockDim.x + threadIdx.x;
	if (i >= a.n) return;
	const float* xp = a.pos + (size_t)i * a.pos_stride;
	float x[D];
#pragma unroll
	for (uint32_t d = 0; d < D; ++d) x[d] = xp[d];
	const float ml = (a.max_level_per_sample ? a.max_level_per_sample[i] : a.max_level) * (float)c.n_levels;
	const f16* gy = a.dL_dy + (size_t)i * a.dy_stride;
	float acc[D];
#pragma unroll
	for (uint32_t d = 0; d < D; ++d) acc[d] = 0.f;
	for (uint32_t l = 0; l < c.n_levels; ++l) {
		if ((float)l >= ml + 1e-3f) continue;
		float frac[D];
		uint32_t base[D];
		level_setup<D>(c, l, x, frac, base);
		float g[F];
#pragma unroll
		for (uint32_t f = 0; f < F; ++f) g[f] = (float)gy[l * F + f];
		float la[D];
#pragma unroll
		for (uint32_t d = 0; d < D; ++d) la[d] = 0.f;
#pragma unroll
		for (uint32_t k = 0; k < (1u << D); ++k) {
			const V v = *(const V*)(a.table + (size_t)corner_index<D>(c, l, base, k) * F);
			float gs = 0.f;
#pragma unroll
			for (uint32_t f = 0; f < F; ++f) {
				if constexpr (F == 1) gs = gs + g[0] * (float)v;
				else gs = gs + g[f] * (float)v[f];
			}
#pragma unroll
			for (uint32_t d = 0; d < D; ++d) {
				float wo = 1.f;
#pragma unroll
				for (uint32_t e = 0; e < D; ++e)
					if (e != d) wo = wo * (((k >> e) & 1u) ? frac[e] : 1.f - frac[e]);
				const float t = wo * gs;
				la[d] = ((k >> d) & 1u) ? la[d] + t : la[d] - t;
			}
		}
#pragma unroll
		for (uint32_t d = 0; d < D; ++d) acc[d] = acc[d] + c.scale[l] * la[d];
	}
	float* o = a.out + (size_t)i * a.out_stride;
#pragma unroll
	for (uint32_t d = 0; d < D; ++d) o[d] = acc[d] * a.out_scale;
	if (a.dL_dsh) {
		const float* dp = a.pos + (size_t)i * a.pos_stride + a.dir_offset;
		const float X = dp[0] * 2.f - 1.f, Y = dp[1] * 2.f - 1.f, Z = dp[2] * 2.f - 1.f;
		float s[16];
#pragma unroll
		for (int k = 0; k < 16; ++k) s[k] = (float)a.dL_dsh[(size_t)i * 16 + k];
		const float A = 0.48860251190291987f, B = 1.0925484305920792f, C = 0.94617469575755997f, E = 0.54627421529603959f,
		            G = 0.59004358992664352f, H = 2.8906114426405538f, I = 0.45704579946446572f, J = 0.3731763325901154f,
		            K = 1.4453057213202769f;
		const float X2 = X * X, Y2 = Y * Y, Z2 = Z * Z;
		float gx = 0.f, gy2 = 0.f, gz = 0.f;
		gx = gx + s[3] * (-A);
		gx = gx + s[4] * (B * Y);
		gx = gx + s[7] * (-B * Z);
		gx = gx + s[8] * (2.f * E * X);
		gx = gx + s[9] * (-6.f * G * X * Y);
		gx = gx + s[10] * (H * Y * Z);
		gx = gx + s[13] * (I * (1.f - 5.f * Z2));
		gx = gx + s[14] * (2.f * K * X * Z);
		gx = gx + s[15] * (3.f * G * (Y2 - X2));
		gy2 = gy2 + s[1] * (-A);
		gy2 = gy2 + s[4] * (B * X);
		gy2 = gy2 + s[5] * (-B * Z);
		gy2 = gy2 + s[8] * (-2.f * E * Y);
		gy2 = gy2 + s[9] * (3.f * G * (Y2 - X2));
		gy2 = gy2 + s[10] * (H * X * Z);
		gy2 = gy2 + s[11] * (I * (1.f - 5.f * Z2));
		gy2 = gy2 + s[14] * (-2.f * K * Y * Z);
		gy2 = gy2 + s[15] * (6.f * G * X * Y);
		gz = gz + s[2] * A;
		gz = gz + s[5] * (-B * Y);
		gz = gz + s[6] * (2.f * C * Z);
		gz = gz + s[7] * (-B * X);
		gz = gz + s[10] * (H * X * Y);
		gz = gz + s[11] * (-10.f * I * Y * Z);
		gz = gz + s[12] * (J * (15.f * Z2 - 3.f));
		gz = gz + s[13] * (-10.f * I * X * Z);
		gz = gz + s[14] * (K * (X2 - Y2));
		float* od = o + a.dir_offset;
		od[0] = 2.f * gx * a.out_scale;
		od[1] = 2.f * gy2 * a.out_scale;
		od[2] = 2.f * gz * a.out_scale;
	}
}

template <uint32_t D>
static void launch_input_grad(uint32_t F, const GridConst& c, const InputGradArgs& a, hipStream_t s) {
	const dim3 grid(div_round_up(a.n, 256)), block(256);
	switch (F) {
		case 1: k_input_grad<D, 1><<<grid, block, 0, s>>>(c, a); break;
		case 2: k_input_grad<D, 2><<<grid, block, 0, s>>>(c, a); break;
		case 4: k_input_grad<D, 4><<<grid, block, 0, s>>>(c, a); break;
		case 8: k_input_grad<D, 8><<<grid, block, 0, s>>>(c, a); break;
		default: throw Error("GridEncoding: unsupported F");
	}
}

void grid_input_gradient(const GridDesc& g, const InputGradArgs& a, hipStream_t stream) {
	if (a.n == 0) return;
	NGP_CHECK(!a.dL_dsh || g.n_dims == 3, "input gradient: the SH direction encoding needs a 3D grid");
	GridConst c = make_grid_const(g);
	if (g.n_dims == 3) launch_input_grad<3>(g.n_features, c, a, stream);
	else launch_input_grad<2>(g.n_features, c, a, stream);
	NGP_HIP(hipGetLastError());
}

void grid_forward(const GridDesc& g, const GridFwdArgs& a, hipStream_t stream, const GridHist* hist) {
	if (a.n == 0) return;
	GridConst c = make_grid_const(g);
	const bool rows = grid_forward_rows_ok(g, a);
	if (g.n_dims == 3) launch_fwd<3>(g.n_features, c, a, stream, rows, hist);
	else launch_fwd<2>(g.n_features, c, a, stream, rows, hist);
	NGP_HIP(hipGetLastError());
}

void grid_backward(const GridDesc& g, const GridBwdArgs& a, hipStream_t stream) {
	if (a.n == 0) return;
	GridConst c = make_grid_const(g);
	if (g.n_dims == 3) launch_bwd<3>(g.n_features, c, a, stream);
	else launch_bwd<2>(g.n_features, c, a, stream);
	NGP_HIP(hipGetLastError());
}

}
```

### instant-ngp_amd/csrc/grid_scatter.h

```cpp
#pragma once
#include "grid.h"
#include "optimizer.h"
#include "slab_reduce.h"

namespace ngp {

enum : uint32_t { SC_STORE_F16 = 0, SC_FUSED_ADAM = 1, SC_STORE_F32 = 2 };

struct BrickConst {
	uint32_t LB = 0, LD = 0;
	uint32_t vb0 = 0;
	uint32_t K = 8, NB = 0, NBK = 0, R = 0;
	uint32_t W[4] = {}, regoff[4] = {};
	uint16_t lo[4][32] = {};
};

struct ScatterPlan {
	uint32_t B = 0;
	uint32_t n_buckets = 0;
	uint32_t spb = 0;
	uint32_t n_chunks = 0;
	uint32_t max_lb = 0;
	uint64_t n_items = 0;
	uint32_t split_limit = 0;
	uint32_t part = 0;
	uint32_t max_split_blocks = 0;
	uint32_t max_split_buckets = 0;
	uint32_t xcd_map = 2;
	uint32_t bt = 1024;
	BrickConst bk;
	uint32_t brick_part = 1024;
	size_t off_hist = 0, off_cur = 0, off_tot = 0, off_split = 0, off_lo = 0, off_splitb = 0, off_scratch = 0, off_idx = 0, off_val = 0,
	       off_bp = 0,
	       off_fb = 0,
	       total = 0;
};

ScatterPlan make_scatter_plan(const GridDesc& g, uint32_t n, bool bricks = true);
void grid_scatter_prepare(const GridDesc& g, const GridBwdArgs& b, const ScatterPlan& p, void* workspace, hipStream_t s,
                          bool hist_done = false);
bool scatter_hist(const GridDesc& g, const ScatterPlan& p, void* workspace, GridHist& h);
struct BwdParts {
	static constexpr uint32_t MAX = 8;
	uint32_t k = 0;
	uint32_t vb_end[MAX] = {};
	void (*after)(void* user, uint32_t part, hipStream_t s) = nullptr;
	void* user = nullptr;
};
uint32_t scatter_bucket_at_param(const GridDesc& g, const ScatterPlan& p, uint64_t param);
void grid_backward_sorted(const GridDesc& g, const GridBwdArgs& b, const ScatterPlan& p, void* workspace,
                          hipStream_t s, bool overwrite, uint32_t debug = 0, const SlabJob* slab = nullptr,
                          const FusedAdam* fused = nullptr, const BwdParts* parts = nullptr);

}
```

### instant-ngp_amd/csrc/grid_scatter.hip

```cpp
#include "grid_scatter.h"

#include <algorithm>
#include <cmath>
#include <cstdlib>

namespace ngp {

namespace {

#ifndef NGP_SC_FASTIDX
#define NGP_SC_FASTIDX 1
#endif
#ifndef NGP_SC_PAIR_RANK
#define NGP_SC_PAIR_RANK 1
#endif
#ifndef NGP_ACC_TAIL_BATCH
#define NGP_ACC_TAIL_BATCH 1
#endif
#ifndef NGP_ACC_SKIP0
#define NGP_ACC_SKIP0 1
#endif
constexpr uint32_t SC_THREADS = 256;
constexpr uint32_t SC_BT = 1024;
constexpr size_t SC_LDS_BYTES = 64 * 1024;
constexpr size_t SC_LDS_PAD_BYTES = 8 * 8;
constexpr size_t SC_LIST_BYTES = 4096 * 2;
constexpr float FIX_SCALE = 16777216.0f;

template <uint32_t F> struct ValVec;
template <> struct ValVec<1> { typedef f16 T; };
template <> struct ValVec<2> { typedef f16x2 T; };
template <> struct ValVec<4> { typedef f16x4 T; };
template <> struct ValVec<8> { typedef f16x8 T; };

__device__ __forceinline__ uint32_t wave_inclusive_scan(uint32_t x) {
	uint32_t s = x;
	s += __builtin_amdgcn_update_dpp(0u, x, 0x111, 0xf, 0xf, true);
	s += __builtin_amdgcn_update_dpp(0u, x, 0x112, 0xf, 0xf, true);
	s += __builtin_amdgcn_update_dpp(0u, x, 0x113, 0xf, 0xf, true);
	s += __builtin_amdgcn_update_dpp(0u, s, 0x114, 0xf, 0xe, false);
	s += __builtin_amdgcn_update_dpp(0u, s, 0x118, 0xf, 0xc, false);
	s += __builtin_amdgcn_update_dpp(0u, s, 0x142, 0xa, 0xf, false);
	s += __builtin_amdgcn_update_dpp(0u, s, 0x143, 0xc, 0xf, false);
	return s;
}

template <uint32_t NT>
__device__ __forceinline__ void block_exclusive_scan(const uint32_t* cnt, uint32_t* off, uint32_t n, uint32_t* wsum) {
	uint32_t carry = 0;
	for (uint32_t b0 = 0; b0 < n; b0 += NT) {
		const uint32_t b = b0 + threadIdx.x;
		const uint32_t v = b < n ? cnt[b] : 0u;
		const uint32_t incl = wave_inclusive_scan(v);
		if ((threadIdx.x & 63) == 63) wsum[threadIdx.x >> 6] = incl;
		__syncthreads();
		uint32_t pre = carry;
		for (uint32_t w = 0; w < (threadIdx.x >> 6); ++w) pre += wsum[w];
		if (b < n) off[b] = pre + incl - v;
#pragma unroll
		for (uint32_t w = 0; w < NT / 64; ++w) carry += wsum[w];
		__syncthreads();
	}
	if (threadIdx.x == 0) off[n] = carry;
}

__device__ __forceinline__ uint32_t bucket_rank(uint32_t* lh, uint32_t j, uint32_t few_bits) {
	if (few_bits > 4) return atomicAdd(&lh[j], 1u);
	uint64_t peers = __ballot(1);
	for (uint32_t b = 0; b < few_bits; ++b) {
		const uint64_t m = __ballot((j >> b) & 1u);
		peers &= ((j >> b) & 1u) ? m : ~m;
	}
	const uint32_t lane = __lane_id();
	const uint32_t leader = __ffsll((unsigned long long)peers) - 1;
	uint32_t base = 0;
	if (lane == leader) base = atomicAdd(&lh[j], (uint32_t)__popcll(peers));
	base = __shfl(base, leader);
	return base + (uint32_t)__popcll(peers & ((1ull << lane) - 1ull));
}

__device__ __forceinline__ uint32_t bucket_rank_cnt(uint32_t* lh, uint32_t j, uint32_t cnt, uint32_t few_bits) {
	if (few_bits > 4) return cnt ? atomicAdd(&lh[j], cnt) : 0u;
	uint64_t peers = __ballot(cnt != 0);
	if (peers == 0ull) return 0u;
	for (uint32_t b = 0; b < few_bits; ++b) {
		const uint64_t m = __ballot((j >> b) & 1u);
		peers &= ((j >> b) & 1u) ? m : ~m;
	}
	const uint64_t two = __ballot(cnt == 2);
	const uint32_t lane = __lane_id();
	const uint32_t leader = peers ? (uint32_t)(__ffsll((unsigned long long)peers) - 1) : lane;
	uint32_t base = 0;
	if (cnt && lane == leader) base = atomicAdd(&lh[j], (uint32_t)(__popcll(peers) + __popcll(peers & two)));
	base = __shfl(base, leader);
	const uint64_t below = peers & ((1ull << lane) - 1ull);
	return base + (uint32_t)(__popcll(below) + __popcll(below & two));
}

template <uint32_t D>
__device__ __forceinline__ void load_pos(const GridBwdArgs& a, uint32_t i, float* x) {
#pragma unroll
	for (uint32_t d = 0; d < D; ++d) x[d] = a.pos[(size_t)i * a.pos_stride + d];
}

struct Levels {
	uint32_t vb_base[33];
};

template <uint32_t F>
__device__ __forceinline__ typename ValVec<F>::T brick_item_hi(uint32_t i) {
	typename ValVec<F>::T v{};
	const f16 h = __builtin_bit_cast(f16, (uint16_t)(i >> 16));
	if constexpr (F == 1) v = h; else v[0] = h;
	return v;
}
template <uint32_t F>
__device__ __forceinline__ uint32_t brick_item(const uint16_t* item_idx, const f16* item_val, uint32_t t) {
	return (uint32_t)item_idx[t] | ((uint32_t)__builtin_bit_cast(uint16_t, item_val[(size_t)t * F]) << 16);
}
struct BrickFallback {
	unsigned long long* fix;
	uint32_t* flag;
};

template <uint32_t D, uint32_t CHUNK>
__global__ void __launch_bounds__(SC_THREADS) k_sc_hist(const GridConst c, const Levels lv, const BrickConst bk, const GridBwdArgs a,
                                                        uint32_t B, uint32_t n_chunks, uint32_t* __restrict__ hist) {
	extern __shared__ uint32_t h[];
	const uint32_t chunk = blockIdx.x, l = blockIdx.y;
	if (l >= bk.LB && l < bk.LD) {
		if constexpr (D == 3) {
			if (l + 1 != bk.LD) return;
			for (uint32_t j = threadIdx.x; j < bk.NBK; j += blockDim.x) h[j] = 0;
			__syncthreads();
			for (uint32_t q = 0; q < CHUNK / SC_THREADS; ++q) {
				const uint32_t i = chunk * CHUNK + q * SC_THREADS + threadIdx.x;
				if (i >= a.n) continue;
				float x[3];
				load_pos<3>(a, i, x);
				atomicAdd(&h[brick_of(c, l, bk.K, bk.NB, x)], 1u);
			}
			__syncthreads();
			for (uint32_t j = threadIdx.x; j < bk.NBK; j += blockDim.x) hist[(size_t)chunk * lv.vb_base[c.n_levels] + bk.vb0 + j] = h[j];
		}
		return;
	}
	const uint32_t nvb = lv.vb_base[l + 1] - lv.vb_base[l];
	const uint32_t few_bits = nvb <= 1 ? 0u : nvb <= 2 ? 1u : nvb <= 4 ? 2u : nvb <= 8 ? 3u : nvb <= 16 ? 4u : 32u;
	for (uint32_t j = threadIdx.x; j < nvb; j += blockDim.x) h[j] = 0;
	__syncthreads();
	const uint32_t off_l = c.offsets[l];
#pragma unroll
	for (uint32_t q = 0; q < CHUNK / SC_THREADS; ++q) {
		const uint32_t i = chunk * CHUNK + q * SC_THREADS + threadIdx.x;
		if (i >= a.n) continue;
		float x[D];
		load_pos<D>(a, i, x);
		float frac[D]; uint32_t base[D];
		level_setup<D>(c, l, x, frac, base);
		uint32_t cidx[1u << D];
		corner_indices<D>(c, l, base, cidx);
#pragma unroll
		for (uint32_t k = 0; k < (1u << D); ++k) hist_add(h, (cidx[k] - off_l) >> B, few_bits);
	}
	__syncthreads();
	for (uint32_t j = threadIdx.x; j < nvb; j += blockDim.x) hist[(size_t)chunk * lv.vb_base[c.n_levels] + lv.vb_base[l] + j] = h[j];
}

constexpr uint32_t SCAN_SEG = 16, SCAN_REG = 32;
__global__ void __launch_bounds__(64 * SCAN_SEG) k_sc_scan(const uint32_t* __restrict__ hist, uint32_t n_chunks, uint32_t n_vb,
                                                         uint32_t* __restrict__ cur, uint32_t* __restrict__ tot) {
	__shared__ uint32_t seg_sum[SCAN_SEG][64];
	const uint32_t lane = threadIdx.x & 63, seg = threadIdx.x >> 6;
	const uint32_t vb = blockIdx.x * 64 + lane;
	const uint32_t per = (n_chunks + SCAN_SEG - 1) / SCAN_SEG;
	const uint32_t c0 = min(seg * per, n_chunks), c1 = min(c0 + per, n_chunks);
	if (per <= SCAN_REG) {
		uint32_t v[SCAN_REG], sum = 0;
#pragma unroll
		for (uint32_t u = 0; u < SCAN_REG; ++u) v[u] = (vb < n_vb && c0 + u < c1) ? hist[(size_t)(c0 + u) * n_vb + vb] : 0u;
#pragma unroll
		for (uint32_t u = 0; u < SCAN_REG; ++u) sum += v[u];
		seg_sum[seg][lane] = sum;
		__syncthreads();
		uint32_t run = 0, total = 0;
		for (uint32_t q = 0; q < SCAN_SEG; ++q) {
			const uint32_t x = seg_sum[q][lane];
			if (q < seg) run += x;
			total += x;
		}
		if (vb >= n_vb) return;
#pragma unroll
		for (uint32_t u = 0; u < SCAN_REG; ++u) {
			if (c0 + u < c1) cur[(size_t)(c0 + u) * n_vb + vb] = run;
			run += v[u];
		}
		if (seg == 0) tot[vb] = total;
		return;
	}
	constexpr uint32_t U = 8;
	uint32_t sum = 0;
	if (vb < n_vb) {
		uint32_t c = c0;
		for (; c + U <= c1; c += U) {
			uint32_t v[U];
#pragma unroll
			for (uint32_t u = 0; u < U; ++u) v[u] = hist[(size_t)(c + u) * n_vb + vb];
#pragma unroll
			for (uint32_t u = 0; u < U; ++u) sum += v[u];
		}
		for (; c < c1; ++c) sum += hist[(size_t)c * n_vb + vb];
	}
	seg_sum[seg][lane] = sum;
	__syncthreads();
	uint32_t run = 0, total = 0;
	for (uint32_t q = 0; q < SCAN_SEG; ++q) {
		const uint32_t v = seg_sum[q][lane];
		if (q < seg) run += v;
		total += v;
	}
	if (vb >= n_vb) return;
	uint32_t c = c0;
	for (; c + U <= c1; c += U) {
		uint32_t v[U];
#pragma unroll
		for (uint32_t u = 0; u < U; ++u) v[u] = hist[(size_t)(c + u) * n_vb + vb];
#pragma unroll
		for (uint32_t u = 0; u < U; ++u) {
			cur[(size_t)(c + u) * n_vb + vb] = run;
			run += v[u];
		}
	}
	for (; c < c1; ++c) {
		const uint32_t v = hist[(size_t)c * n_vb + vb];
		cur[(size_t)c * n_vb + vb] = run;
		run += v;
	}
	if (seg == 0) tot[vb] = total;
}

constexpr uint32_t SC_PLAN_THREADS = 1024;
template <uint32_t SC_PLAN_K>
__global__ void __launch_bounds__(SC_PLAN_THREADS) k_sc_plan(const uint32_t* __restrict__ tot, uint32_t n_vb, uint32_t split_limit,
                                                             uint32_t part, uint32_t* __restrict__ lo_out,
                                                             uint32_t* __restrict__ split, uint32_t* __restrict__ splitb,
                                                             uint32_t brick_vb0, uint32_t n_bricks, uint32_t brick_part, uint32_t* __restrict__ bp,
                                                             uint32_t* __restrict__ fb_flag) {
	if (fb_flag && threadIdx.x == 0) *fb_flag = 0u;
	__shared__ uint32_t wsum[3][SC_PLAN_THREADS / 64];
	const uint32_t lane = threadIdx.x & 63, wave = threadIdx.x >> 6;
	constexpr bool VEC = SC_PLAN_K % 4 == 0;
	uint32_t K = min(SC_PLAN_K, (n_vb + SC_PLAN_THREADS - 1) / SC_PLAN_THREADS);
	if (VEC) K = (K + 3) & ~3u;
	uint32_t c_lo = 0, c_parts = 0, c_sb = 0;
	for (uint32_t b0 = 0; b0 < n_vb; b0 += SC_PLAN_THREADS * K) {
		const uint32_t v0 = b0 + threadIdx.x * K;
		uint32_t t[SC_PLAN_K];
		if (VEC) {
#pragma unroll
			for (uint32_t k = 0; k < SC_PLAN_K; k += 4) {
				if (k < K && v0 + k + 3 < n_vb) {
					const uint4 q = *(const uint4*)(tot + v0 + k);
					t[k] = q.x; t[k + 1] = q.y; t[k + 2] = q.z; t[k + 3] = q.w;
				} else {
#pragma unroll
					for (uint32_t j = 0; j < 4; ++j) t[k + j] = (k + j < K && v0 + k + j < n_vb) ? tot[v0 + k + j] : 0u;
				}
			}
		} else {
#pragma unroll
			for (uint32_t k = 0; k < SC_PLAN_K; ++k) t[k] = (k < K && v0 + k < n_vb) ? tot[v0 + k] : 0u;
		}
		uint32_t s0 = 0, s1 = 0, s2 = 0;
#pragma unroll
		for (uint32_t k = 0; k < SC_PLAN_K; ++k) {
			const bool brick = v0 + k - brick_vb0 < n_bricks;
			const uint32_t sp = (brick ? t[k] > 0 : t[k] > split_limit) ? 1u : 0u;
			const uint32_t pk = brick ? brick_part : part;
			s0 += t[k]; s1 += sp ? (t[k] + pk - 1) / pk : 0u; s2 += brick ? 0u : sp;
		}
		const uint32_t i0 = wave_inclusive_scan(s0), i1 = wave_inclusive_scan(s1), i2 = wave_inclusive_scan(s2);
		if (lane == 63) { wsum[0][wave] = i0; wsum[1][wave] = i1; wsum[2][wave] = i2; }
		__syncthreads();
		uint32_t p0 = c_lo, p1 = c_parts, p2 = c_sb;
		for (uint32_t w = 0; w < SC_PLAN_THREADS / 64; ++w) {
			if (w < wave) { p0 += wsum[0][w]; p1 += wsum[1][w]; p2 += wsum[2][w]; }
			c_lo += wsum[0][w]; c_parts += wsum[1][w]; c_sb += wsum[2][w];
		}
		__syncthreads();
		uint32_t lo = p0 + i0 - s0, first = p1 + i1 - s1, b = p2 + i2 - s2;
		if (VEC) {
			uint32_t l = lo;
#pragma unroll
			for (uint32_t k = 0; k < SC_PLAN_K; k += 4) {
				const uint32_t l0 = l, l1 = l0 + t[k], l2 = l1 + t[k + 1], l3 = l2 + t[k + 2];
				l = l3 + t[k + 3];
				if (k < K && v0 + k + 3 < n_vb) {
					*(uint4*)(lo_out + v0 + k) = uint4{l0, l1, l2, l3};
				} else {
					const uint32_t lv[4] = {l0, l1, l2, l3};
#pragma unroll
					for (uint32_t j = 0; j < 4; ++j)
						if (k + j < K && v0 + k + j < n_vb) lo_out[v0 + k + j] = lv[j];
				}
			}
		}
#pragma unroll
		for (uint32_t k = 0; k < SC_PLAN_K; ++k) {
			if (k >= K || v0 + k >= n_vb) break;
			const uint32_t vb = v0 + k, tk = t[k];
			if (!VEC) lo_out[vb] = lo;
			if (vb - brick_vb0 < n_bricks) {
				const uint32_t parts = (tk + brick_part - 1) / brick_part;
				bp[2 * (vb - brick_vb0)] = first; bp[2 * (vb - brick_vb0) + 1] = parts;
				for (uint32_t q = 0; q < parts; ++q) {
					uint32_t* d = split + 2 + 3 * (size_t)(first + q);
					d[0] = vb; d[1] = lo + q * brick_part; d[2] = min(lo + (q + 1) * brick_part, lo + tk);
				}
				first += parts;
			} else if (tk > split_limit) {
				const uint32_t parts = (tk + part - 1) / part;
				splitb[3 * b] = vb; splitb[3 * b + 1] = first; splitb[3 * b + 2] = parts;
				for (uint32_t q = 0; q < parts; ++q) {
					uint32_t* d = split + 2 + 3 * (size_t)(first + q);
					d[0] = vb; d[1] = lo + q * part; d[2] = min(lo + (q + 1) * part, lo + tk);
				}
				first += parts;
				++b;
			}
			lo += tk;
		}
	}
	if (threadIdx.x == 0) { split[0] = c_parts; split[1] = c_sb; }
}

template <uint32_t F, uint32_t SC_CHUNK, uint32_t SC_ST>
__device__ void scatter_bricks(const GridConst& c, const BrickConst& bk, const GridBwdArgs& a, uint32_t n_vb, uint32_t chunk,
                               const uint32_t* __restrict__ cur_t, const uint32_t* __restrict__ lo_vb,
                               uint16_t* __restrict__ item_idx, f16* __restrict__ item_val, uint32_t* lds, uint32_t* wsum) {
	typedef typename ValVec<F>::T V;
	constexpr uint32_t SC_SSPT = SC_CHUNK / SC_ST;
	const uint32_t nvb = bk.NBK;
	uint32_t* cur = lds;
	uint32_t* lh = cur + nvb;
	uint32_t* loff = lh + nvb;
	uint16_t* st_b = (uint16_t*)(loff + nvb + 1);
	uint32_t* st_i = (uint32_t*)(((uintptr_t)(st_b + SC_CHUNK) + 15) & ~(uintptr_t)15);
	for (uint32_t j = threadIdx.x; j < nvb; j += blockDim.x) {
		cur[j] = lo_vb[bk.vb0 + j] + cur_t[(size_t)chunk * n_vb + bk.vb0 + j];
		lh[j] = 0;
	}
	__syncthreads();
	uint32_t e[SC_SSPT], r[SC_SSPT];
#pragma unroll
	for (uint32_t q = 0; q < SC_SSPT; ++q) {
		const uint32_t i = chunk * SC_CHUNK + q * SC_ST + threadIdx.x;
		if (i >= a.n) continue;
		float x[3];
		load_pos<3>(a, i, x);
		e[q] = brick_of(c, bk.LD - 1, bk.K, bk.NB, x);
		r[q] = atomicAdd(&lh[e[q]], 1u);
	}
	__syncthreads();
	block_exclusive_scan<SC_ST>(lh, loff, nvb, wsum);
	__syncthreads();
#pragma unroll
	for (uint32_t q = 0; q < SC_SSPT; ++q) {
		const uint32_t i = chunk * SC_CHUNK + q * SC_ST + threadIdx.x;
		if (i >= a.n) continue;
		const uint32_t slot = loff[e[q]] + r[q];
		st_b[slot] = (uint16_t)e[q];
		st_i[slot] = i;
	}
	__syncthreads();
	const uint32_t n_it = loff[nvb];
	for (uint32_t t = threadIdx.x; t < n_it; t += blockDim.x) {
		const uint32_t j = st_b[t], i = st_i[t];
		const uint32_t gpos = cur[j] + (t - loff[j]);
		item_idx[gpos] = (uint16_t)(i & 0xffffu);
		*(V*)(item_val + (size_t)gpos * F) = brick_item_hi<F>(i);
	}
}

template <uint32_t D, uint32_t F, uint32_t SC_CHUNK, uint32_t SC_ST>
__global__ void __launch_bounds__(SC_ST) k_sc_scatter(const GridConst c, const Levels lv, const BrickConst bk, const GridBwdArgs a, uint32_t B,
                                                      uint32_t n_vb, uint32_t n_chunks, uint32_t xcd_map, const uint32_t* __restrict__ cur_t,
                                                      const uint32_t* __restrict__ lo_vb, uint16_t* __restrict__ item_idx,
                                                      f16* __restrict__ item_val, uint32_t debug) {
	typedef typename ValVec<F>::T V;
	constexpr uint32_t NC = 1u << D;
	constexpr uint32_t NIT = SC_CHUNK * NC;
	constexpr uint32_t SC_SSPT = SC_CHUNK / SC_ST;
	extern __shared__ uint32_t lds[];
	__shared__ uint32_t wsum[SC_ST / 64];
	const uint32_t n_slots = c.n_levels - (bk.LD - bk.LB) + (bk.LD ? 1u : 0u);
	uint32_t chunk, l;
	if (xcd_map == 1) {
		const uint32_t slot = blockIdx.x >> 3;
		l = slot % n_slots;
		chunk = (slot / n_slots) * 8 + (blockIdx.x & 7);
	} else if (xcd_map == 2) {
		const uint32_t slot = blockIdx.x >> 3, cpx = (n_chunks + 7) >> 3;
		l = slot % n_slots;
		chunk = (blockIdx.x & 7) * cpx + slot / n_slots;
		if (slot / n_slots >= cpx) return;
	} else {
		chunk = blockIdx.x % n_chunks;
		l = blockIdx.x / n_chunks;
	}
	if (chunk >= n_chunks) return;
	if (bk.LD && l >= bk.LB) {
		if constexpr (D == 3) {
			if (l == bk.LB) {
				scatter_bricks<F, SC_CHUNK, SC_ST>(c, bk, a, n_vb, chunk, cur_t, lo_vb, item_idx, item_val, lds, wsum);
				return;
			}
		}
		l = l - bk.LB - 1 + bk.LD;
	}
	const uint32_t nvb = lv.vb_base[l + 1] - lv.vb_base[l];
	uint32_t* cur = lds;
	uint32_t* lh = cur + nvb;
	uint32_t* loff = lh + nvb;
	uint16_t* st_b = (uint16_t*)(loff + nvb + 1);
	uint16_t* st_idx = st_b + NIT;
	V* st_val = (V*)(((uintptr_t)(st_idx + NIT) + 15) & ~(uintptr_t)15);
	for (uint32_t j = threadIdx.x; j < nvb; j += blockDim.x) {
		const uint32_t vb = lv.vb_base[l] + j;
		cur[j] = lo_vb[vb] + cur_t[(size_t)chunk * n_vb + vb];
		lh[j] = 0;
	}
	__syncthreads();
	const uint32_t off_l = c.offsets[l];
	const uint32_t mask = (1u << B) - 1u;
	const uint32_t few_bits = nvb <= 1 ? 0u : nvb <= 2 ? 1u : nvb <= 4 ? 2u : nvb <= 8 ? 3u : nvb <= 16 ? 4u : 32u;
	uint32_t e[SC_SSPT][NC], r[SC_SSPT][NC];
	V val[SC_SSPT][NC];
	uint32_t n_have = 0;
#pragma unroll
	for (uint32_t q = 0; q < SC_SSPT; ++q) {
		const uint32_t i = chunk * SC_CHUNK + q * SC_ST + threadIdx.x;
		if (i >= a.n) continue;
		n_have = q + 1;
		float x[D];
		load_pos<D>(a, i, x);
		const float ml = (a.max_level_per_sample ? a.max_level_per_sample[i] : a.max_level) * (float)c.n_levels;
		const bool active = !((float)l > ml + 1e-3f);
		float g[F];
		if (a.dy_layout == AoS) {
			V gv;
			if (active) gv = *(const V*)(a.dL_dy + (size_t)i * a.dy_stride + l * F);
#pragma unroll
			for (uint32_t f = 0; f < F; ++f) {
				if constexpr (F == 1) g[f] = active ? (float)gv : 0.f;
				else g[f] = active ? (float)gv[f] : 0.f;
			}
		} else {
#pragma unroll
			for (uint32_t f = 0; f < F; ++f) g[f] = active ? (float)a.dL_dy[(size_t)(l * F + f) * a.dy_stride + i] : 0.f;
		}
		float frac[D]; uint32_t base[D];
		level_setup<D>(c, l, x, frac, base);
#if NGP_SC_FASTIDX
		uint32_t cidx[NC];
		corner_indices<D>(c, l, base, cidx);
#endif
#pragma unroll
		for (uint32_t k = 0; k < NC; ++k) {
#if NGP_SC_FASTIDX
			e[q][k] = cidx[k] - off_l;
#else
			e[q][k] = corner_index<D>(c, l, base, k) - off_l;
#endif
#if NGP_SC_PAIR_RANK
			if (k & 1u) {
				const uint32_t j0 = e[q][k - 1] >> B, j1 = e[q][k] >> B;
				const bool same = j0 == j1;
				const uint32_t r0 = bucket_rank_cnt(lh, j0, same ? 2u : 1u, few_bits);
				const uint32_t r1 = bucket_rank_cnt(lh, j1, same ? 0u : 1u, few_bits);
				r[q][k - 1] = r0;
				r[q][k] = same ? r0 + 1u : r1;
			}
#else
			r[q][k] = bucket_rank(lh, e[q][k] >> B, few_bits);
#endif
			const float w = corner_weight<D>(frac, k);
			if constexpr (F == 1) val[q][k] = to_f16(w * g[0]);
			else {
#pragma unroll
				for (uint32_t f = 0; f < F; ++f) val[q][k][f] = to_f16(w * g[f]);
			}
		}
	}
	__syncthreads();
	block_exclusive_scan<SC_ST>(lh, loff, nvb, wsum);
	__syncthreads();
#pragma unroll
	for (uint32_t q = 0; q < SC_SSPT; ++q) {
		if (q >= n_have) break;
#pragma unroll
		for (uint32_t k = 0; k < NC; ++k) {
			const uint32_t j = e[q][k] >> B;
			const uint32_t slot = loff[j] + r[q][k];
			st_b[slot] = (uint16_t)j;
			st_idx[slot] = (uint16_t)(e[q][k] & mask);
			st_val[slot] = val[q][k];
		}
	}
	__syncthreads();
	const uint32_t n_it = loff[nvb];
	if (!(debug & 8))
		for (uint32_t t = threadIdx.x; t < n_it; t += blockDim.x) {
			const uint32_t j = st_b[t];
			const uint32_t gpos = cur[j] + (t - loff[j]);
			item_idx[gpos] = st_idx[t];
			*(V*)(item_val + (size_t)gpos * F) = st_val[t];
		}
}

template <uint32_t F>
__device__ __forceinline__ void accumulate_items(unsigned long long* acc, uint32_t NE, uint32_t lo, uint32_t hi,
                                                 const uint16_t* __restrict__ item_idx, const f16* __restrict__ item_val,
                                                 uint32_t debug = 0) {
	typedef typename ValVec<F>::T V;
	if (debug & 32) {
		float sum = 0.f;
		for (uint32_t t = lo + threadIdx.x; t < hi; t += blockDim.x) {
			const V vv = *(const V*)(item_val + (size_t)t * F);
			if constexpr (F == 1) sum += (float)vv; else sum += (float)vv[0];
			sum += (float)item_idx[t];
		}
		acc[threadIdx.x] = (unsigned long long)sum;
		return;
	}
	constexpr uint32_t U = 8;
	const uint32_t NEP = NE + 1;
	const uint32_t rot = (debug & 64) ? 0u : threadIdx.x % F;
	auto add_item = [&](uint32_t j, const V& vv) {
#pragma unroll
		for (uint32_t k = 0; k < F; ++k) {
			const uint32_t f = (k + rot) & (F - 1);
			float x;
			if constexpr (F == 1) x = (float)vv;
			else {
				x = (float)vv[0];
#pragma unroll
				for (uint32_t q = 1; q < F; ++q) x = f == q ? (float)vv[q] : x;
			}
#if NGP_ACC_SKIP0
			if (x != 0.f) atomicAdd(&acc[f * NEP + j], (unsigned long long)(long long)(x * FIX_SCALE));
#else
			atomicAdd(&acc[f * NEP + j], (unsigned long long)(long long)(x * FIX_SCALE));
#endif
		}
	};
	const uint32_t step = blockDim.x * U;
	uint32_t t0 = lo;
	for (; t0 + step <= hi; t0 += step) {
		uint32_t j[U];
		V v[U];
#pragma unroll
		for (uint32_t u = 0; u < U; ++u) {
			const uint32_t t = t0 + u * blockDim.x + threadIdx.x;
			j[u] = item_idx[t];
			v[u] = *(const V*)(item_val + (size_t)t * F);
		}
#pragma unroll
		for (uint32_t u = 0; u < U; ++u) add_item(j[u], v[u]);
	}
	if (!NGP_ACC_TAIL_BATCH || F != 2) {
		for (uint32_t t = t0 + threadIdx.x; t < hi; t += blockDim.x) add_item(item_idx[t], *(const V*)(item_val + (size_t)t * F));
		return;
	}
	if (t0 >= hi) return;
	{
		uint32_t j[U];
		V v[U];
#pragma unroll
		for (uint32_t u = 0; u < U; ++u) {
			const uint32_t t = min(t0 + u * blockDim.x + threadIdx.x, hi - 1);
			j[u] = item_idx[t];
			v[u] = *(const V*)(item_val + (size_t)t * F);
		}
#pragma unroll
		for (uint32_t u = 0; u < U; ++u)
			if (t0 + u * blockDim.x + threadIdx.x < hi) add_item(j[u], v[u]);
	}
}

__device__ __forceinline__ float fix_to_f32(unsigned long long q) { return (float)((double)(long long)q * (1.0 / FIX_SCALE)); }

template <uint32_t F>
__device__ void accumulate_brick(const GridConst& c, const BrickConst& bk, const GridBwdArgs& a, uint32_t vb, uint32_t lo, uint32_t hi,
                                 const uint16_t* __restrict__ item_idx, const f16* __restrict__ item_val, unsigned long long* acc,
                                 unsigned long long* __restrict__ dst, uint32_t NE, const BrickFallback& fb) {
	typedef typename ValVec<F>::T V;
	const uint32_t RP = bk.R + 1;
	for (uint32_t k = threadIdx.x; k < RP * F; k += blockDim.x) acc[k] = 0ull;
	__syncthreads();
	const uint32_t b3[3] = {vb % bk.NB, (vb / bk.NB) % bk.NB, vb / (bk.NB * bk.NB)};
	const uint32_t ns = hi - lo, rot = threadIdx.x % F;
	for (uint32_t w = threadIdx.x; w < ns * (bk.LD - bk.LB); w += blockDim.x) {
		const uint32_t l = bk.LB + w / ns, i = brick_item<F>(item_idx, item_val, lo + w % ns);
		float x[3];
		load_pos<3>(a, i, x);
		const float ml = (a.max_level_per_sample ? a.max_level_per_sample[i] : a.max_level) * (float)c.n_levels;
		if ((float)l > ml + 1e-3f) continue;
		float g[F];
		if (a.dy_layout == AoS) {
			const V gv = *(const V*)(a.dL_dy + (size_t)i * a.dy_stride + l * F);
#pragma unroll
			for (uint32_t f = 0; f < F; ++f) {
				if constexpr (F == 1) g[f] = (float)gv; else g[f] = (float)gv[f];
			}
		} else {
#pragma unroll
			for (uint32_t f = 0; f < F; ++f) g[f] = (float)a.dL_dy[(size_t)(l * F + f) * a.dy_stride + i];
		}
		float frac[3]; uint32_t base[3];
		level_setup<3>(c, l, x, frac, base);
		const uint32_t W = bk.W[l], res = c.resolution[l];
		uint32_t r0[3];
		bool lo_in[3], hi_in[3];
#pragma unroll
		for (uint32_t d = 0; d < 3; ++d) {
			r0[d] = base[d] - bk.lo[l][b3[d]];
			lo_in[d] = base[d] <= res;
			hi_in[d] = base[d] + 1u <= res;
		}
#pragma unroll
		for (uint32_t k = 0; k < 8; ++k) {
			const uint32_t rx = r0[0] + (k & 1u), ry = r0[1] + ((k >> 1) & 1u), rz = r0[2] + ((k >> 2) & 1u);
			const float wk = corner_weight<3>(frac, k);
			const bool in = rx < W && ry < W && rz < W && ((k & 1u) ? hi_in[0] : lo_in[0]) && ((k & 2u) ? hi_in[1] : lo_in[1]) &&
			                ((k & 4u) ? hi_in[2] : lo_in[2]);
			const uint32_t local = bk.regoff[l] + rx + W * (ry + W * rz);
#pragma unroll
			for (uint32_t q = 0; q < F; ++q) {
				const uint32_t f = (q + rot) & (F - 1);
				float gf = g[0];
#pragma unroll
				for (uint32_t u = 1; u < F; ++u) gf = f == u ? g[u] : gf;
				const float v = (float)to_f16(wk * gf);
				if (v == 0.f) continue;
				const unsigned long long fx = (unsigned long long)(long long)(v * FIX_SCALE);
				if (__builtin_expect(in, 1)) atomicAdd(&acc[f * RP + local], fx);
				else {
					atomicAdd(&fb.fix[(size_t)corner_index<3>(c, l, base, k) * F + f], fx);
					*fb.flag = 1u;
				}
			}
		}
	}
	__syncthreads();
	for (uint32_t k = threadIdx.x; k < bk.R * F; k += blockDim.x) dst[(k / bk.R) * NE + k % bk.R] = acc[(k / bk.R) * RP + k % bk.R];
}

template <uint32_t F>
__device__ __forceinline__ void brick_entry_sums(const GridConst& c, const BrickConst& bk, uint32_t e, uint32_t NE,
                                                 const uint32_t* __restrict__ bp, const unsigned long long* __restrict__ scratch,
                                                 const BrickFallback& fb, bool fb_used, unsigned long long (&q)[F]) {
#pragma unroll
	for (uint32_t f = 0; f < F; ++f) q[f] = 0ull;
	uint32_t l = 0;
	while (c.offsets[l + 1] <= e) ++l;
	const int res = (int)c.resolution[l], idx = (int)(e - c.offsets[l]);
	const int cc[3] = {idx % res, (idx / res) % res, idx / (res * res)};
	const uint32_t W = bk.W[l];
	auto range = [&](int v, uint32_t& b0, uint32_t& b1) {
		b0 = bk.NB; b1 = 0;
		for (uint32_t b = 0; b < bk.NB; ++b) {
			const int lb = bk.lo[l][b];
			if (lb <= v && v < lb + (int)W) { b0 = min(b0, b); b1 = b + 1; }
		}
	};
	auto cands = [&](int t, int* v, int* bo) {
		int n = 0;
		if (t >= 0) { v[n] = t; bo[n] = 0; ++n; }
		if (t == 0) { v[n] = res; bo[n] = 1; ++n; }
		if (t == -1) { v[n] = res - 1; bo[n] = 1; ++n; }
		return n;
	};
	int va[2], ba[2];
	const int na = cands(cc[0], va, ba);
	for (int ia = 0; ia < na; ++ia) {
		int vb_[2], bb[2];
		const int nb = cands(cc[1] - ba[ia], vb_, bb);
		for (int ib = 0; ib < nb; ++ib) {
			int vc[2], bc[2];
			const int nc = cands(cc[2] - bb[ib], vc, bc);
			for (int ic = 0; ic < nc; ++ic) {
				const int v3[3] = {va[ia], vb_[ib], vc[ic]};
				uint32_t b0[3], b1[3];
#pragma unroll
				for (int d = 0; d < 3; ++d) range(v3[d], b0[d], b1[d]);
				for (uint32_t bz = b0[2]; bz < b1[2]; ++bz)
					for (uint32_t by = b0[1]; by < b1[1]; ++by)
						for (uint32_t bx = b0[0]; bx < b1[0]; ++bx) {
							const uint32_t b = bx + bk.NB * (by + bk.NB * bz);
							const uint32_t first = bp[2 * b], parts = bp[2 * b + 1];
							const uint32_t local = bk.regoff[l] + (uint32_t)(v3[0] - bk.lo[l][bx]) +
							                       W * ((uint32_t)(v3[1] - bk.lo[l][by]) + W * (uint32_t)(v3[2] - bk.lo[l][bz]));
							for (uint32_t p = 0; p < parts; ++p) {
								const unsigned long long* src = scratch + (size_t)(first + p) * NE * F + local;
#pragma unroll
								for (uint32_t f = 0; f < F; ++f) q[f] += src[(size_t)f * NE];
							}
						}
			}
		}
	}
	if (fb_used) {
		unsigned long long* src = fb.fix + (size_t)e * F;
#pragma unroll
		for (uint32_t f = 0; f < F; ++f) {
			const unsigned long long v = src[f];
			if (v) { q[f] += v; src[f] = 0ull; }
		}
	}
}

__device__ __forceinline__ void bucket_entries(const GridConst& c, const Levels& lv, uint32_t B, uint32_t vb, uint32_t& e0, uint32_t& n_e) {
	uint32_t l = 0;
	while (lv.vb_base[l + 1] <= vb) ++l;
	const uint32_t j = vb - lv.vb_base[l];
	e0 = c.offsets[l] + (j << B);
	n_e = min(1u << B, c.offsets[l + 1] - e0);
}

template <uint32_t F>
__device__ __forceinline__ void pair_slots(uint32_t k, uint32_t NE, uint32_t& a, uint32_t& b) {
	if constexpr (F == 1) { a = 2 * k; b = 2 * k + 1; }
	else {
		const uint32_t j = k / (F / 2), fp = k % (F / 2);
		a = (2 * fp) * NE + j; b = (2 * fp + 1) * NE + j;
	}
}

template <bool G32>
__device__ __forceinline__ void store_pair(f16* grad, float* g32, size_t k, float s0, float s1) {
	if constexpr (G32) {
		typedef float f32x2 __attribute__((ext_vector_type(2)));
		((f32x2*)g32)[k] = f32x2{(float)(f16)s0, (float)(f16)s1};
	} else {
		((f16x2*)grad)[k] = f16x2{(f16)s0, (f16)s1};
	}
}

template <uint32_t F, uint32_t MODE>
__global__ void __launch_bounds__(SC_BT) k_sc_accumulate(const GridConst c, const Levels lv, const BrickConst bk, const GridBwdArgs a,
                                                         const uint32_t* __restrict__ tot,
                                                         const uint32_t* __restrict__ lo_arr, uint32_t B, uint32_t split_limit,
                                                         uint32_t max_parts, const uint16_t* __restrict__ item_idx,
                                                         const f16* __restrict__ item_val, f16* __restrict__ grad, bool overwrite,
                                                         const uint32_t* __restrict__ split, unsigned long long* __restrict__ scratch,
                                                         uint32_t debug, const FusedAdam fa, const BrickFallback fb, uint32_t vb_off,
                                                         uint32_t part_lo, uint32_t part_hi) {
	constexpr bool FUSED = MODE == SC_FUSED_ADAM, G32 = MODE == SC_STORE_F32;
	extern __shared__ unsigned long long acc[];
	const uint32_t NE = 1u << B, NEP = NE + 1;
	if (blockIdx.x < max_parts) {
		if (blockIdx.x >= split[0]) return;
		const uint32_t* d = split + 2 + 3 * (size_t)blockIdx.x;
		if (d[0] < part_lo || d[0] >= part_hi) return;
		const uint32_t lo = d[1], hi = d[2];
		if (d[0] - bk.vb0 < bk.NBK) {
			accumulate_brick<F>(c, bk, a, d[0] - bk.vb0, lo, hi, item_idx, item_val, acc, scratch + (size_t)blockIdx.x * NE * F, NE, fb);
			return;
		}
		for (uint32_t k = threadIdx.x; k < NEP * F; k += blockDim.x) acc[k] = 0ull;
		__syncthreads();
		if (!(debug & 1)) accumulate_items<F>(acc, NE, lo, hi, item_idx, item_val, debug);
		__syncthreads();
		unsigned long long* dst = scratch + (size_t)blockIdx.x * NE * F;
		for (uint32_t k = threadIdx.x; k < NE * F; k += blockDim.x) dst[k] = acc[(k / NE) * NEP + k % NE];
		return;
	}
	const uint32_t vb = blockIdx.x - max_parts + vb_off;
	if (vb - bk.vb0 < bk.NBK) return;
	const uint32_t t = tot[vb];
	if (t > split_limit) return;
	uint32_t e0, n_e;
	bucket_entries(c, lv, B, vb, e0, n_e);
	f16* g = grad + (size_t)e0 * F;
	if (t == 0) {
		if (overwrite && !FUSED)
			for (uint32_t k = threadIdx.x; k < n_e * F / 2; k += blockDim.x) store_pair<G32>(grad, fa.g32, (size_t)e0 * F / 2 + k, 0.f, 0.f);
		return;
	}
	const uint32_t lo = lo_arr[vb];
	for (uint32_t k = threadIdx.x; k < NEP * F; k += blockDim.x) acc[k] = 0ull;
	__syncthreads();
	if (!(debug & 1)) accumulate_items<F>(acc, NE, lo, lo + t, item_idx, item_val, debug);
	__syncthreads();
	if constexpr (FUSED) {
		if (t >= 2 * n_e) {
			for (uint32_t k = threadIdx.x; k < n_e * F / 2; k += blockDim.x) {
				uint32_t ia, ib;
				pair_slots<F>(k, NEP, ia, ib);
				fused_adam_pair(fa, e0 * F / 2 + k, (f16)fix_to_f32(acc[ia]), (f16)fix_to_f32(acc[ib]));
			}
			return;
		}
		__shared__ uint32_t n_list;
		uint16_t* list = (uint16_t*)(acc + NEP * F);
		if (threadIdx.x == 0) n_list = 0;
		__syncthreads();
		const uint32_t lane = threadIdx.x & 63;
		for (uint32_t k = threadIdx.x; k < n_e * F / 2; k += blockDim.x) {
			uint32_t ia, ib;
			pair_slots<F>(k, NEP, ia, ib);
			const f16 h0 = (f16)fix_to_f32(acc[ia]), h1 = (f16)fix_to_f32(acc[ib]);
			const bool act = (float)h0 / fa.loss_scale != 0.f || (float)h1 / fa.loss_scale != 0.f;
			const unsigned long long m = __ballot(act);
			if (m == 0ull) continue;
			const uint32_t leader = __ffsll((long long)m) - 1;
			uint32_t base = 0;
			if (lane == leader) base = atomicAdd(&n_list, (uint32_t)__popcll(m));
			base = __shfl(base, leader);
			if (act) list[base + __popcll(m & ((1ull << lane) - 1ull))] = (uint16_t)k;
		}
		__syncthreads();
		const uint32_t na = n_list;
		for (uint32_t i = threadIdx.x; i < na; i += blockDim.x) {
			const uint32_t k = list[i];
			uint32_t ia, ib;
			pair_slots<F>(k, NEP, ia, ib);
			fused_adam_pair(fa, e0 * F / 2 + k, (f16)fix_to_f32(acc[ia]), (f16)fix_to_f32(acc[ib]));
		}
		return;
	}
	for (uint32_t k = threadIdx.x; k < n_e * F / 2; k += blockDim.x) {
		uint32_t ia, ib;
		pair_slots<F>(k, NEP, ia, ib);
		float s0 = fix_to_f32(acc[ia]), s1 = fix_to_f32(acc[ib]);
		if (!G32 && !overwrite) {
			const f16x2 o = ((const f16x2*)g)[k];
			s0 += (float)o[0];
			s1 += (float)o[1];
		}
		store_pair<G32>(grad, fa.g32, (size_t)e0 * F / 2 + k, s0, s1);
	}
}

template <uint32_t F, uint32_t MODE>
__global__ void __launch_bounds__(SC_THREADS) k_sc_split_reduce(const GridConst c, const Levels lv, uint32_t B,
                                                                const uint32_t* __restrict__ split, const uint32_t* __restrict__ splitb,
                                                                const unsigned long long* __restrict__ scratch, f16* __restrict__ grad,
                                                                bool overwrite, const SlabJob sj, uint32_t slab_x0, const FusedAdam fa,
                                                                const BrickConst bk, const uint32_t* __restrict__ bp, const BrickFallback fb,
                                                                uint32_t fin_x0, uint32_t part_lo, uint32_t part_hi) {
	static_assert(SC_THREADS == SLAB_THREADS, "slab blocks share the split-reduce block shape");
	constexpr bool FUSED = MODE == SC_FUSED_ADAM, G32 = MODE == SC_STORE_F32;
	if (blockIdx.x >= fin_x0) {
		constexpr uint32_t EPT = F == 1 ? 2 : 1;
		const uint32_t blk = blockIdx.y * (gridDim.x - fin_x0) + (blockIdx.x - fin_x0);
		const uint32_t e0 = c.offsets[bk.LB] + (blk * blockDim.x + threadIdx.x) * EPT;
		if (e0 >= c.offsets[bk.LD]) return;
		const uint32_t NE = 1u << B;
		const bool used = *fb.flag != 0u;
		float s[EPT * F];
#pragma unroll
		for (uint32_t u = 0; u < EPT; ++u) {
			unsigned long long q[F];
			brick_entry_sums<F>(c, bk, e0 + u, NE, bp, scratch, fb, used, q);
#pragma unroll
			for (uint32_t f = 0; f < F; ++f) s[u * F + f] = fix_to_f32(q[f]);
		}
#pragma unroll
		for (uint32_t h = 0; h < EPT * F / 2; ++h) {
			const uint32_t k = e0 * F / 2 + h;
			float s0 = s[2 * h], s1 = s[2 * h + 1];
			if (FUSED) {
				fused_adam_pair(fa, k, (f16)s0, (f16)s1);
				continue;
			}
			if (!G32 && !overwrite) {
				const f16x2 o = ((const f16x2*)grad)[k];
				s0 += (float)o[0];
				s1 += (float)o[1];
			}
			store_pair<G32>(grad, fa.g32, k, s0, s1);
		}
		return;
	}
	if (blockIdx.x >= slab_x0) {
		const uint32_t blk = blockIdx.y * (fin_x0 - slab_x0) + (blockIdx.x - slab_x0);
		if (blk >= slab_blocks(sj.n)) return;
		if (!FUSED || fa.mlp_n == 0) {
			reduce_slabs_block(sj, blk);
			return;
		}
		__shared__ f16 gsh[32];
		reduce_slabs_block(sj, blk, gsh);
		__syncthreads();
		const uint32_t i0 = blk * 32 + 4 * threadIdx.x;
		if (threadIdx.x >= 8 || i0 >= fa.mlp_n) return;
		AdamState st{};
		st.w16 = fa.mlp_w16; st.rec = fa.mlp_rec; st.frags = fa.frags; st.fragmap = fa.fragmap; st.bias_tab = fa.bias_tab;
		const AdamConfig cfg = fa.cfg_dev ? *fa.cfg_dev : fa.cfg;
		const uint32_t step = (fa.step_base ? *fa.step_base : 0u) + fa.step_add;
		LazyGroup G;
		G.i0 = i0;
#pragma unroll
		for (int k = 0; k < 4; ++k) {
			G.g[k] = (float)gsh[4 * threadIdx.x + k] / fa.loss_scale;
			G.act[k] = true;
		}
		G.any[0] = G.any[1] = true;
#pragma unroll
		for (int r = 0; r < 2; ++r) {
			const f32x4* rp = (const f32x4*)(fa.mlp_rec + (i0 >> 1) + r);
			G.q[r][0] = rp[0]; G.q[r][1] = rp[1]; G.q[r][2] = rp[2];
		}
		lazy_update(st, cfg, step, fa.mlp_n, G);
		return;
	}
	if (blockIdx.x >= split[1]) return;
	const uint32_t vb = splitb[3 * blockIdx.x], first = splitb[3 * blockIdx.x + 1], parts = splitb[3 * blockIdx.x + 2];
	if (vb < part_lo || vb >= part_hi) return;
	const uint32_t NE = 1u << B;
	uint32_t e0, n_e;
	bucket_entries(c, lv, B, vb, e0, n_e);
	f16* g = grad + (size_t)e0 * F;
	const uint32_t k = blockIdx.y * blockDim.x + threadIdx.x;
	if (k < n_e * F / 2) {
		uint32_t ia, ib;
		pair_slots<F>(k, NE, ia, ib);
		const size_t pstride = (size_t)NE * F;
		const unsigned long long* src = scratch + (size_t)first * pstride;
		unsigned long long q0 = 0, q1 = 0;
		uint32_t p = 0;
		for (; p + 8 <= parts; p += 8) {
			unsigned long long x0[8], x1[8];
#pragma unroll
			for (int u = 0; u < 8; ++u) { x0[u] = src[(p + u) * pstride + ia]; x1[u] = src[(p + u) * pstride + ib]; }
#pragma unroll
			for (int u = 0; u < 8; ++u) { q0 += x0[u]; q1 += x1[u]; }
		}
		for (; p < parts; ++p) { q0 += src[p * pstride + ia]; q1 += src[p * pstride + ib]; }
		float s0 = fix_to_f32(q0), s1 = fix_to_f32(q1);
		if (FUSED) {
			fused_adam_pair(fa, e0 * F / 2 + k, (f16)s0, (f16)s1);
			return;
		}
		if (!G32 && !overwrite) {
			const f16x2 o = ((const f16x2*)g)[k];
			s0 += (float)o[0];
			s1 += (float)o[1];
		}
		store_pair<G32>(grad, fa.g32, (size_t)e0 * F / 2 + k, s0, s1);
	}
}

size_t scatter_lds_bytes(uint32_t max_lb, uint32_t chunk, uint32_t D, uint32_t F) {
	const size_t nit = (size_t)chunk << D;
	return (size_t)(3 * max_lb + 1) * 4 + nit * 4 + 16 + nit * F * 2;
}

Levels make_levels(const GridDesc& g, uint32_t B, const BrickConst& bk) {
	Levels lv{};
	uint32_t vb = 0;
	for (uint32_t l = 0; l < g.n_levels; ++l) {
		lv.vb_base[l] = vb;
		if (bk.LD && l == bk.LB) vb += bk.NBK;
		else if (!(l >= bk.LB && l < bk.LD)) vb += (g.offsets[l + 1] - g.offsets[l] + (1u << B) - 1) >> B;
	}
	for (uint32_t l = g.n_levels; l <= 32; ++l) lv.vb_base[l] = vb;
	return lv;
}

template <uint32_t D>
void launch_backward(uint32_t F, const GridConst& c, const Levels& lv, const GridBwdArgs& a, const ScatterPlan& p, char* ws,
                     hipStream_t s, bool overwrite, uint32_t debug, const SlabJob* slab, const FusedAdam& fa, const BwdParts* parts) {
	const uint32_t* tot = (const uint32_t*)(ws + p.off_tot);
	const uint32_t* cur_t = (const uint32_t*)(ws + p.off_cur);
	const uint32_t* split = (const uint32_t*)(ws + p.off_split);
	const uint32_t* lo = (const uint32_t*)(ws + p.off_lo);
	const uint32_t* splitb = (const uint32_t*)(ws + p.off_splitb);
	unsigned long long* scratch = (unsigned long long*)(ws + p.off_scratch);
	uint16_t* idx = (uint16_t*)(ws + p.off_idx);
	f16* val = (f16*)(ws + p.off_val);
	const uint32_t* bp = (const uint32_t*)(ws + p.off_bp);
	const BrickFallback fb{(unsigned long long*)(ws + p.off_fb), (uint32_t*)(ws + p.off_fb + (size_t)c.offsets[p.bk.LD] * c.n_features * 8)};
	const size_t lds_s = scatter_lds_bytes(p.max_lb, p.spb, D, F);
	const uint32_t xcd_map = p.xcd_map;
	const uint32_t n_slots = c.n_levels - (p.bk.LD - p.bk.LB) + (p.bk.LD ? 1u : 0u);
	const dim3 grid_s(xcd_map ? (uint32_t)div_round_up(p.n_chunks, 8) * 8 * n_slots : p.n_chunks * n_slots);
	auto go = [&](auto scatter, auto accum, auto splitr) {
		ensure_dynamic_lds((const void*)scatter, lds_s);
		if (!(debug & 4))
			scatter<<<grid_s, p.spb == 512 ? 512 : 1024, lds_s, s>>>(c, lv, p.bk, a, p.B, p.n_buckets, p.n_chunks, xcd_map, cur_t, lo, idx, val,
			                                                          debug);
		NGP_HIP(hipGetLastError());
		const size_t lds_a = ((size_t)8 << p.B) * c.n_features + SC_LDS_PAD_BYTES + (fa.rec ? SC_LIST_BYTES : 0);
		ensure_dynamic_lds((const void*)accum, lds_a);
		const bool parted = parts && parts->k > 0;
		const uint32_t gy = (uint32_t)div_round_up(((size_t)1 << p.B) * c.n_features / 2, SC_THREADS);
		const SlabJob sj = slab ? *slab : SlabJob{};
		const uint32_t slab_x = slab ? (uint32_t)div_round_up(slab_blocks(sj.n), gy) : 0u;
		const size_t fin_entries = (size_t)c.offsets[p.bk.LD] - c.offsets[p.bk.LB];
		const size_t fin_threads = c.n_features == 1 ? div_round_up(fin_entries, 2) : fin_entries;
		const uint32_t fin_x = (uint32_t)div_round_up(div_round_up(fin_threads, SC_THREADS), gy);
		if (!parted) {
			accum<<<p.max_split_blocks + p.n_buckets, p.bt, lds_a, s>>>(c, lv, p.bk, a, tot, lo, p.B, p.split_limit, p.max_split_blocks,
			                                                             idx, val, a.grad, overwrite, split, scratch, debug, fa, fb, 0u,
			                                                             0u, ~0u);
			NGP_HIP(hipGetLastError());
			const dim3 grid_r(p.max_split_buckets + slab_x + fin_x, gy);
			splitr<<<grid_r, SC_THREADS, 0, s>>>(c, lv, p.B, split, splitb, scratch, a.grad, overwrite, sj, p.max_split_buckets, fa, p.bk, bp,
			                                     fb, p.max_split_buckets + slab_x, 0u, ~0u);
			NGP_HIP(hipGetLastError());
			return;
		}
		NGP_CHECK(!p.bk.LD, "grid backward parts: not with bricks");
		for (uint32_t jj = 0; jj < parts->k; ++jj) {
			const uint32_t j = parts->k - 1 - jj;
			const uint32_t v0 = j ? std::min(parts->vb_end[j - 1], p.n_buckets) : 0u;
			const uint32_t v1 = j + 1 == parts->k ? p.n_buckets : std::min(parts->vb_end[j], p.n_buckets);
			NGP_CHECK(v0 <= v1, "grid backward parts: bucket ranges out of order");
			accum<<<p.max_split_blocks + (v1 - v0), p.bt, lds_a, s>>>(c, lv, p.bk, a, tot, lo, p.B, p.split_limit, p.max_split_blocks,
			                                                           idx, val, a.grad, overwrite, split, scratch, debug, fa, fb, v0,
			                                                           v0, v1);
			NGP_HIP(hipGetLastError());
			const uint32_t sx = j == 0 ? slab_x : 0u;
			const dim3 grid_r(p.max_split_buckets + sx, gy);
			splitr<<<grid_r, SC_THREADS, 0, s>>>(c, lv, p.B, split, splitb, scratch, a.grad, overwrite, sj, p.max_split_buckets, fa, p.bk, bp,
			                                     fb, p.max_split_buckets + sx, v0, v1);
			NGP_HIP(hipGetLastError());
			if (parts->after) parts->after(parts->user, j, s);
		}
	};
	auto by_chunk = [&](auto sc512, auto sc1024, auto accum, auto splitr) {
		if (p.spb == 512) go(sc512, accum, splitr);
		else go(sc1024, accum, splitr);
	};
#define NGP_SC_F(FF)                                                                                                 \
	if (fa.rec) by_chunk(k_sc_scatter<D, FF, 512, 512>, k_sc_scatter<D, FF, 1024, 1024>, k_sc_accumulate<FF, SC_FUSED_ADAM>, \
	                     k_sc_split_reduce<FF, SC_FUSED_ADAM>);                                                      \
	else if (fa.g32) by_chunk(k_sc_scatter<D, FF, 512, 512>, k_sc_scatter<D, FF, 1024, 1024>,                       \
	                          k_sc_accumulate<FF, SC_STORE_F32>, k_sc_split_reduce<FF, SC_STORE_F32>);              \
	else by_chunk(k_sc_scatter<D, FF, 512, 512>, k_sc_scatter<D, FF, 1024, 1024>, k_sc_accumulate<FF, SC_STORE_F16>,  \
	              k_sc_split_reduce<FF, SC_STORE_F16>)
	switch (F) {
		case 1: NGP_SC_F(1); break;
		case 2: NGP_SC_F(2); break;
		case 4: NGP_SC_F(4); break;
		case 8: NGP_SC_F(8); break;
		default: throw Error("grid backward: unsupported F");
	}
#undef NGP_SC_F
}

static BrickConst make_bricks(const GridDesc& g, uint32_t n, uint32_t B, uint32_t brick_part) {
	BrickConst best;
	if (g.n_dims != 3) return best;
	if (const char* e = getenv("NGP_SC_BRICKS")) { if (atoi(e) == 0) return best; }
	double min_cells = 3.0;
	if (const char* e = getenv("NGP_SC_BRICK_MIN_CELLS")) min_cells = atof(e);
	const uint32_t F = g.n_features, NE = 1u << B;
	uint32_t dense = 0;
	while (dense < g.n_levels && dense < 4) {
		const uint64_t r = g.resolution[dense];
		if (r * r * r != g.offsets[dense + 1] - g.offsets[dense]) break;
		++dense;
	}
	double best_save = 0.0;
	for (uint32_t LD = 1; LD <= dense; ++LD)
		for (uint32_t LB = 0; LB < LD; ++LB) {
			BrickConst bk;
			bk.LB = LB; bk.LD = LD; bk.K = 8;
			const uint32_t f = LD - 1, cells = g.resolution[f];
			bk.NB = (cells + bk.K - 1) / bk.K;
			if (bk.NB < 2 || bk.NB > 32) continue;
			if ((double)bk.K * g.scale[LB] / g.scale[f] < min_cells) continue;
			bk.NBK = bk.NB * bk.NB * bk.NB;
			bool ok = true;
			for (uint32_t l = LB; l < LD && ok; ++l) {
				uint32_t W = 0;
				for (uint32_t b = 0; b < bk.NB; ++b) {
					int64_t c_lo, c_hi;
					if (l == f) { c_lo = (int64_t)bk.K * b; c_hi = c_lo + bk.K; }
					else {
						const double sl = g.scale[l], sf = g.scale[f];
						const double lower = sl * ((double)bk.K * b - 0.5) / sf + 0.5, upper = sl * ((double)bk.K * b + bk.K - 0.5) / sf + 0.5;
						c_lo = (int64_t)std::floor(lower) - 1;
						c_hi = (int64_t)std::floor(upper) + 2;
					}
					c_lo = std::max<int64_t>(c_lo, 0);
					c_hi = std::min<int64_t>(c_hi, (int64_t)g.resolution[l]);
					bk.lo[l][b] = (uint16_t)c_lo;
					W = std::max<uint32_t>(W, (uint32_t)(c_hi - c_lo + 1));
				}
				bk.W[l] = W;
				bk.regoff[l] = bk.R;
				bk.R += W * W * W;
				ok = bk.R <= NE;
			}
			if (!ok) continue;
			const double parts = std::max((double)std::min<uint64_t>(bk.NBK, n), (double)n / brick_part);
			const double slabs = parts * bk.R * F * 8;
			const double items = (double)n * (LD - LB) * 8 * (2 + 2 * F);
			const double save = 0.75 * items - slabs;
			if (save > best_save) { best_save = save; best = bk; }
		}
	if (best.LD)
		for (uint32_t l = 0; l < best.LB; ++l) best.vb0 += (g.offsets[l + 1] - g.offsets[l] + NE - 1) >> B;
	return best;
}

}

ScatterPlan make_scatter_plan(const GridDesc& g, uint32_t n, bool bricks) {
	ScatterPlan p;
	const uint32_t F = g.n_features;
	p.B = 0;
	size_t lds_budget = SC_LDS_BYTES;
	if (const char* e = getenv("NGP_SC_LDS_KB")) lds_budget = std::min<size_t>(SC_LDS_BYTES, (size_t)atoi(e) * 1024);
	while (((size_t)2 << p.B) * F * 8 <= lds_budget && p.B < 16) ++p.B;
	if (const char* e = getenv("NGP_SC_BRICK_PART")) p.brick_part = std::max(1, atoi(e));
	if (bricks) p.bk = make_bricks(g, n, p.B, p.brick_part);
	const Levels lv = make_levels(g, p.B, p.bk);
	p.n_buckets = lv.vb_base[g.n_levels];
	p.max_lb = p.bk.NBK;
	for (uint32_t l = 0; l < g.n_levels; ++l) p.max_lb = std::max(p.max_lb, lv.vb_base[l + 1] - lv.vb_base[l]);
	NGP_CHECK((size_t)p.max_lb * 4 <= 32 * 1024, "grid backward: level too large for the bucket histogram");
	const uint64_t items_per_sample = ((uint64_t)(g.n_levels - (p.bk.LD - p.bk.LB)) << g.n_dims) + (p.bk.LD ? 1u : 0u);
	p.spb = 512;
	if (512ull * items_per_sample < 16ull * p.n_buckets && scatter_lds_bytes(p.max_lb, 1024, g.n_dims, F) <= 160 * 1024) p.spb = 1024;
	if (const char* e = getenv("NGP_SC_CHUNK")) p.spb = (uint32_t)atoi(e);
	NGP_CHECK(p.spb == 512 || p.spb == 1024, "grid backward: chunk must be 512 or 1024 samples");
	NGP_CHECK(scatter_lds_bytes(p.max_lb, p.spb, g.n_dims, F) <= 160 * 1024, "grid backward: scatter chunk exceeds LDS");
	p.n_chunks = (uint32_t)div_round_up(n, p.spb);
	p.n_items = (uint64_t)n * items_per_sample;
	NGP_CHECK(p.n_items < (1ull << 32), "grid backward: too many contributions for 32-bit offsets");
	p.split_limit = 49152;
	p.part = 49152;
	if (const char* e = getenv("NGP_SC_PART")) p.part = (uint32_t)atoi(e);
	if (const char* e = getenv("NGP_SC_LIMIT")) p.split_limit = (uint32_t)atoi(e);
	p.max_split_blocks = (uint32_t)(div_round_up(p.n_items, (uint64_t)p.part) + div_round_up(p.n_items, (uint64_t)p.split_limit) + 1);
	if (p.bk.LD) p.max_split_blocks += (uint32_t)(std::min<uint64_t>(p.bk.NBK, n) + div_round_up((uint64_t)n, (uint64_t)p.brick_part));
	p.max_split_buckets = (uint32_t)(div_round_up(p.n_items, (uint64_t)p.split_limit) + 1);
	p.xcd_map = 2;
	if (const char* e = getenv("NGP_SC_XCD")) p.xcd_map = (uint32_t)atoi(e);
	p.bt = F == 2 ? 512 : 1024;
	if (const char* e = getenv("NGP_SC_BT")) p.bt = (uint32_t)atoi(e);
	NGP_CHECK(p.bt >= 64 && p.bt <= SC_BT && p.bt % 64 == 0, "grid backward: NGP_SC_BT must be a multiple of 64 up to 1024");
	const uint64_t len = (uint64_t)p.n_buckets * p.n_chunks;
	NGP_CHECK(len < (1ull << 31), "grid backward: bucket histogram too large");
	auto align = [](size_t v) { return (v + 255) / 256 * 256; };
	p.off_hist = 0;
	p.off_cur = align(p.off_hist + len * 4);
	p.off_tot = align(p.off_cur + len * 4);
	p.off_split = align(p.off_tot + (size_t)p.n_buckets * 4);
	p.off_lo = align(p.off_split + (2 + 3 * (size_t)p.max_split_blocks) * 4);
	p.off_splitb = align(p.off_lo + (size_t)p.n_buckets * 4);
	p.off_scratch = align(p.off_splitb + 3 * (size_t)p.max_split_buckets * 4);
	p.off_idx = align(p.off_scratch + (size_t)p.max_split_blocks * ((size_t)1 << p.B) * g.n_features * 8);
	p.off_val = align(p.off_idx + p.n_items * 2);
	p.off_bp = align(p.off_val + p.n_items * F * 2);
	p.off_fb = align(p.off_bp + (size_t)p.bk.NBK * 8);
	p.total = align(p.off_fb + (size_t)g.offsets[p.bk.LD] * F * 8 + 4);
	return p;
}

bool scatter_hist(const GridDesc& g, const ScatterPlan& p, void* workspace, GridHist& h) {
	if ((size_t)p.n_buckets * 4 > 48 * 1024 || p.spb != 512) return false;
	const Levels lv = make_levels(g, p.B, p.bk);
	h.hist = (uint32_t*)((char*)workspace + p.off_hist);
	h.B = p.B; h.n_chunks = p.n_chunks; h.chunk = p.spb;
	for (int l = 0; l <= 32; ++l) h.vb_base[l] = lv.vb_base[l];
	h.brick_first = p.bk.LB; h.brick_levels = p.bk.LD; h.n_bricks = p.bk.NBK; h.brick_cells = p.bk.K; h.bricks_per_dim = p.bk.NB;
	h.brick_vb0 = p.bk.vb0;
	return true;
}

void grid_scatter_prepare(const GridDesc& g, const GridBwdArgs& a, const ScatterPlan& p, void* workspace, hipStream_t s, bool hist_done) {
	if (a.n == 0) return;
	char* ws = (char*)workspace;
	uint32_t* hist = (uint32_t*)(ws + p.off_hist);
	if (!hist_done) {
		const GridConst c = make_grid_const(g);
		const Levels lv = make_levels(g, p.B, p.bk);
		const dim3 grid_h(p.n_chunks, g.n_levels);
		const size_t lds_h = (size_t)p.max_lb * 4;
		auto go = [&](auto k3, auto k2) {
			if (g.n_dims == 3) k3<<<grid_h, SC_THREADS, lds_h, s>>>(c, lv, p.bk, a, p.B, p.n_chunks, hist);
			else k2<<<grid_h, SC_THREADS, lds_h, s>>>(c, lv, p.bk, a, p.B, p.n_chunks, hist);
		};
		if (p.spb == 512) go(k_sc_hist<3, 512>, k_sc_hist<2, 512>);
		else go(k_sc_hist<3, 1024>, k_sc_hist<2, 1024>);
		NGP_HIP(hipGetLastError());
	}
	k_sc_scan<<<div_round_up(p.n_buckets, 64), 64 * SCAN_SEG, 0, s>>>(hist, p.n_chunks, p.n_buckets, (uint32_t*)(ws + p.off_cur), (uint32_t*)(ws + p.off_tot));
	NGP_HIP(hipGetLastError());
	const auto plan = p.n_buckets <= SC_PLAN_THREADS ? k_sc_plan<1> : p.n_buckets <= 8 * SC_PLAN_THREADS ? k_sc_plan<8> : k_sc_plan<32>;
	plan<<<1, SC_PLAN_THREADS, 0, s>>>((const uint32_t*)(ws + p.off_tot), p.n_buckets, p.split_limit, p.part,
	                                        (uint32_t*)(ws + p.off_lo), (uint32_t*)(ws + p.off_split), (uint32_t*)(ws + p.off_splitb),
	                                        p.bk.vb0, p.bk.NBK, p.brick_part, (uint32_t*)(ws + p.off_bp),
	                                        p.bk.LD ? (uint32_t*)(ws + p.off_fb + (size_t)g.offsets[p.bk.LD] * g.n_features * 8) : nullptr);
	NGP_HIP(hipGetLastError());
}

uint32_t scatter_bucket_at_param(const GridDesc& g, const ScatterPlan& p, uint64_t param) {
	const Levels lv = make_levels(g, p.B, p.bk);
	for (uint32_t vb = 0; vb < p.n_buckets; ++vb) {
		uint32_t l = 0;
		while (lv.vb_base[l + 1] <= vb) ++l;
		const uint64_t e1 = std::min<uint64_t>((uint64_t)g.offsets[l] + ((uint64_t)(vb - lv.vb_base[l] + 1) << p.B), g.offsets[l + 1]);
		if (e1 * g.n_features > param) return vb;
	}
	return p.n_buckets;
}

void grid_backward_sorted(const GridDesc& g, const GridBwdArgs& b, const ScatterPlan& p, void* workspace, hipStream_t s,
                          bool overwrite, uint32_t debug, const SlabJob* slab, const FusedAdam* fused, const BwdParts* parts) {
	if (b.n == 0) return;
	NGP_CHECK(b.level_begin == 0, "grid_backward_sorted handles all levels");
	NGP_CHECK(!fused || (overwrite && g.n_features >= 2), "fused optimizer: overwrite mode, F >= 2");
	NGP_CHECK(!parts || !parts->k || (!p.bk.LD && !(fused && fused->rec) && parts->k <= BwdParts::MAX),
	          "grid backward parts: not with bricks or the fused update");
	const GridConst c = make_grid_const(g);
	const Levels lv = make_levels(g, p.B, p.bk);
	const FusedAdam fa = fused ? *fused : FusedAdam{};
	if (g.n_dims == 3) launch_backward<3>(g.n_features, c, lv, b, p, (char*)workspace, s, overwrite, debug, slab, fa, parts);
	else launch_backward<2>(g.n_features, c, lv, b, p, (char*)workspace, s, overwrite, debug, slab, fa, parts);
}

}
```

Before: 1.655 billion samples/s.

## Accumulate small coarse grid levels directly in LDS, skipping sort/scatter

Adds a direct-accumulation path for hash-grid backward. Coarse levels whose whole table fits in two LDS buckets are handled by blocks that walk sample ranges and atomically accumulate fixed-point gradients into shared memory, writing per-part partials that the existing split reduce combines. These levels are then dropped from the histogram, scatter and sorted-item pipeline, which removes their items from the sort. An optional mode (off by default) moves the bucket planning into the scatter and accumulate kernels so the separate plan launch is skipped. The cost is more kernel template variants, more scratch space, and LDS atomic contention on these small levels.

```diff
diff --git a/instant-ngp_amd/csrc/engine.hip b/instant-ngp_amd/csrc/engine.hip
--- a/instant-ngp_amd/csrc/engine.hip
+++ b/instant-ngp_amd/csrc/engine.hip
@@ -159,6 +159,8 @@
 	bool fuse_opt = true;
 	bool fuse_mlp_opt = true;
 	bool grid_bricks = false;
+	bool grid_direct = true;
+	bool grid_plan_inline = false;
 	hipStream_t side = nullptr;
 	hipEvent_t ev_fork = nullptr, ev_join = nullptr, ev_frags = nullptr, ev_mlp = nullptr, ev_red = nullptr;
 	f16 *params = nullptr, *inference_params = nullptr, *gradients = nullptr;
@@ -213,7 +215,7 @@
 	bool side_prepare(uint32_t n) const { return use_sorted(n) && (overlap & 1); }
 	const ScatterPlan& sc_plan_for(uint32_t n) {
 		if (sc_plan_n != n) {
-			sc_plan = make_scatter_plan(grid, n, grid_bricks);
+			sc_plan = make_scatter_plan(grid, n, grid_bricks, grid_direct, grid_plan_inline);
 			sc_plan_n = n;
 			fb_dirty = true;
 		}
@@ -882,6 +884,12 @@
 		} else if (k == "grid_bricks") {
 			m->grid_bricks = value != 0;
 			m->sc_plan_n = 0;
+		} else if (k == "grid_direct") {
+			m->grid_direct = value != 0;
+			m->sc_plan_n = 0;
+		} else if (k == "grid_plan_inline") {
+			m->grid_plan_inline = value != 0;
+			m->sc_plan_n = 0;
 		} else if (k == "win_debug") {
 			m->win_debug = (uint32_t)value;
 		} else {
@@ -896,6 +904,9 @@
 	NGP_TRY({
 		const std::string k = key;
 		if (k == "grid_brick_levels") *value = m->sc_plan_n ? (double)(m->sc_plan.bk.LD - m->sc_plan.bk.LB) : 0.0;
+		else if (k == "grid_direct_levels") *value = m->sc_plan_n ? (double)m->sc_plan.direct_levels : 0.0;
+		else if (k == "grid_direct_part") *value = (double)make_scatter_plan(m->grid, 4096, false).direct_part;
+		else if (k == "grid_plan_inline") *value = m->sc_plan_n && m->sc_plan.plan_inline ? 1.0 : 0.0;
 		else throw Error("unknown model query: " + k);
 	});
 }
diff --git a/instant-ngp_amd/csrc/grid.h b/instant-ngp_amd/csrc/grid.h
--- a/instant-ngp_amd/csrc/grid.h
+++ b/instant-ngp_amd/csrc/grid.h
@@ -48,6 +48,7 @@
 	uint32_t B, n_chunks, chunk;
 	uint32_t vb_base[33];
 	uint32_t brick_first = 0, brick_levels = 0, n_bricks = 0, brick_cells = 8, bricks_per_dim = 0, brick_vb0 = 0;
+	uint32_t direct_levels = 0;
 };
 
 void grid_forward(const GridDesc& g, const GridFwdArgs& a, hipStream_t stream, const GridHist* hist = nullptr);
diff --git a/instant-ngp_amd/csrc/grid.hip b/instant-ngp_amd/csrc/grid.hip
--- a/instant-ngp_amd/csrc/grid.hip
+++ b/instant-ngp_amd/csrc/grid.hip
@@ -134,7 +134,7 @@
 #pragma unroll
 		for (uint32_t f = 0; f < F; ++f) acc[f] = 0.f;
 		const bool active = l < c.n_levels && !((float)l >= ml + 1e-3f);
-		const bool count = HIST && !(l >= h.brick_first && l < h.brick_levels);
+		const bool count = HIST && !(l >= h.brick_first && l < h.brick_levels) && l >= h.direct_levels;
 		if (count && l < c.n_levels && !active) {
 			float frac[D]; uint32_t base[D];
 			level_setup<D>(c, l, x, frac, base);
diff --git a/instant-ngp_amd/csrc/grid_scatter.h b/instant-ngp_amd/csrc/grid_scatter.h
--- a/instant-ngp_amd/csrc/grid_scatter.h
+++ b/instant-ngp_amd/csrc/grid_scatter.h
@@ -29,6 +29,9 @@
 	uint32_t xcd_map = 2;
 	uint32_t bt = 1024;
 	BrickConst bk;
+	uint32_t direct_mask = 0, direct_levels = 0, direct_buckets = 0;
+	uint32_t direct_part = 0, direct_parts = 0;
+	bool plan_inline = false;
 	uint32_t brick_part = 1024;
 	size_t off_hist = 0, off_cur = 0, off_tot = 0, off_split = 0, off_lo = 0, off_splitb = 0, off_scratch = 0, off_idx = 0, off_val = 0,
 	       off_bp = 0,
@@ -36,7 +39,7 @@
 	       total = 0;
 };
 
-ScatterPlan make_scatter_plan(const GridDesc& g, uint32_t n, bool bricks = true);
+ScatterPlan make_scatter_plan(const GridDesc& g, uint32_t n, bool bricks = true, bool direct = true, bool plan_inline = false);
 void grid_scatter_prepare(const GridDesc& g, const GridBwdArgs& b, const ScatterPlan& p, void* workspace, hipStream_t s,
                           bool hist_done = false);
 bool scatter_hist(const GridDesc& g, const ScatterPlan& p, void* workspace, GridHist& h);
diff --git a/instant-ngp_amd/csrc/grid_scatter.hip b/instant-ngp_amd/csrc/grid_scatter.hip
--- a/instant-ngp_amd/csrc/grid_scatter.hip
+++ b/instant-ngp_amd/csrc/grid_scatter.hip
@@ -105,6 +105,8 @@
 
 struct Levels {
 	uint32_t vb_base[33];
+	uint32_t nd = 0, dS = 0, dP = 0;
+	uint32_t level_items = 0;
 };
 
 template <uint32_t F>
@@ -146,6 +148,10 @@
 		return;
 	}
 	const uint32_t nvb = lv.vb_base[l + 1] - lv.vb_base[l];
+	if (l < lv.nd) {
+		for (uint32_t j = threadIdx.x; j < nvb; j += blockDim.x) hist[(size_t)chunk * lv.vb_base[c.n_levels] + lv.vb_base[l] + j] = 0;
+		return;
+	}
 	const uint32_t few_bits = nvb <= 1 ? 0u : nvb <= 2 ? 1u : nvb <= 4 ? 2u : nvb <= 8 ? 3u : nvb <= 16 ? 4u : 32u;
 	for (uint32_t j = threadIdx.x; j < nvb; j += blockDim.x) h[j] = 0;
 	__syncthreads();
@@ -245,14 +251,15 @@
                                                              uint32_t part, uint32_t* __restrict__ lo_out,
                                                              uint32_t* __restrict__ split, uint32_t* __restrict__ splitb,
                                                              uint32_t brick_vb0, uint32_t n_bricks, uint32_t brick_part, uint32_t* __restrict__ bp,
-                                                             uint32_t* __restrict__ fb_flag) {
+                                                             uint32_t* __restrict__ fb_flag, uint32_t nd_b, uint32_t dP) {
 	if (fb_flag && threadIdx.x == 0) *fb_flag = 0u;
 	__shared__ uint32_t wsum[3][SC_PLAN_THREADS / 64];
 	const uint32_t lane = threadIdx.x & 63, wave = threadIdx.x >> 6;
 	constexpr bool VEC = SC_PLAN_K % 4 == 0;
 	uint32_t K = min(SC_PLAN_K, (n_vb + SC_PLAN_THREADS - 1) / SC_PLAN_THREADS);
 	if (VEC) K = (K + 3) & ~3u;
-	uint32_t c_lo = 0, c_parts = 0, c_sb = 0;
+	for (uint32_t v = threadIdx.x; v < nd_b; v += SC_PLAN_THREADS) { splitb[3 * v] = v; splitb[3 * v + 1] = v * dP; splitb[3 * v + 2] = dP; }
+	uint32_t c_lo = 0, c_parts = nd_b * dP, c_sb = nd_b;
 	for (uint32_t b0 = 0; b0 < n_vb; b0 += SC_PLAN_THREADS * K) {
 		const uint32_t v0 = b0 + threadIdx.x * K;
 		uint32_t t[SC_PLAN_K];
@@ -334,6 +341,43 @@
 	if (threadIdx.x == 0) { split[0] = c_parts; split[1] = c_sb; }
 }
 
+struct PlanShared {
+	uint32_t wsum[3][SC_PLAN_THREADS / 64];
+	uint32_t res[3];
+};
+template <class Fn>
+__device__ __forceinline__ void plan_scan(const uint32_t* __restrict__ tot, uint32_t n_vb, uint32_t split_limit, uint32_t part,
+                                          uint32_t first0, uint32_t sb0, PlanShared& sh, Fn visit) {
+	const uint32_t lane = threadIdx.x & 63, wave = threadIdx.x >> 6, nw = blockDim.x >> 6;
+	uint32_t c0 = 0, c1 = first0, c2 = sb0;
+	for (uint32_t b0 = 0; b0 < n_vb; b0 += blockDim.x) {
+		const uint32_t vb = b0 + threadIdx.x;
+		const uint32_t t = vb < n_vb ? tot[vb] : 0u;
+		const uint32_t sp = t > split_limit ? 1u : 0u, np = sp ? (t + part - 1) / part : 0u;
+		const uint32_t i0 = wave_inclusive_scan(t), i1 = wave_inclusive_scan(np), i2 = wave_inclusive_scan(sp);
+		if (lane == 63) { sh.wsum[0][wave] = i0; sh.wsum[1][wave] = i1; sh.wsum[2][wave] = i2; }
+		__syncthreads();
+		uint32_t p0 = c0, p1 = c1, p2 = c2;
+		for (uint32_t w = 0; w < nw; ++w) {
+			if (w < wave) { p0 += sh.wsum[0][w]; p1 += sh.wsum[1][w]; p2 += sh.wsum[2][w]; }
+			c0 += sh.wsum[0][w]; c1 += sh.wsum[1][w]; c2 += sh.wsum[2][w];
+		}
+		__syncthreads();
+		if (vb < n_vb) visit(vb, t, p0 + i0 - t, p1 + i1 - np, p2 + i2 - sp, np);
+	}
+}
+__device__ __forceinline__ uint32_t plan_bucket_lo(const uint32_t* __restrict__ tot, uint32_t level_items, uint32_t vb0, uint32_t vb,
+                                                   PlanShared& sh) {
+	uint32_t sum = 0;
+	for (uint32_t j = vb0 + threadIdx.x; j < vb; j += blockDim.x) sum += tot[j];
+	sum = wave_inclusive_scan(sum);
+	if ((threadIdx.x & 63) == 63) sh.wsum[0][threadIdx.x >> 6] = sum;
+	__syncthreads();
+	uint32_t lo = level_items;
+	for (uint32_t w = 0; w < (blockDim.x >> 6); ++w) lo += sh.wsum[0][w];
+	return __builtin_amdgcn_readfirstlane(lo);
+}
+
 template <uint32_t F, uint32_t SC_CHUNK, uint32_t SC_ST>
 __device__ void scatter_bricks(const GridConst& c, const BrickConst& bk, const GridBwdArgs& a, uint32_t n_vb, uint32_t chunk,
                                const uint32_t* __restrict__ cur_t, const uint32_t* __restrict__ lo_vb,
@@ -382,18 +426,18 @@
 	}
 }
 
-template <uint32_t D, uint32_t F, uint32_t SC_CHUNK, uint32_t SC_ST>
+template <uint32_t D, uint32_t F, uint32_t SC_CHUNK, uint32_t SC_ST, bool INL = false>
 __global__ void __launch_bounds__(SC_ST) k_sc_scatter(const GridConst c, const Levels lv, const BrickConst bk, const GridBwdArgs a, uint32_t B,
                                                       uint32_t n_vb, uint32_t n_chunks, uint32_t xcd_map, const uint32_t* __restrict__ cur_t,
                                                       const uint32_t* __restrict__ lo_vb, uint16_t* __restrict__ item_idx,
-                                                      f16* __restrict__ item_val, uint32_t debug) {
+                                                      f16* __restrict__ item_val, uint32_t debug, const uint32_t* __restrict__ tot) {
 	typedef typename ValVec<F>::T V;
 	constexpr uint32_t NC = 1u << D;
 	constexpr uint32_t NIT = SC_CHUNK * NC;
 	constexpr uint32_t SC_SSPT = SC_CHUNK / SC_ST;
 	extern __shared__ uint32_t lds[];
 	__shared__ uint32_t wsum[SC_ST / 64];
-	const uint32_t n_slots = c.n_levels - (bk.LD - bk.LB) + (bk.LD ? 1u : 0u);
+	const uint32_t n_slots = c.n_levels - (bk.LD - bk.LB) + (bk.LD ? 1u : 0u) - lv.nd;
 	uint32_t chunk, l;
 	if (xcd_map == 1) {
 		const uint32_t slot = blockIdx.x >> 3;
@@ -418,6 +462,7 @@
 		}
 		l = l - bk.LB - 1 + bk.LD;
 	}
+	l += lv.nd;
 	const uint32_t nvb = lv.vb_base[l + 1] - lv.vb_base[l];
 	uint32_t* cur = lds;
 	uint32_t* lh = cur + nvb;
@@ -425,10 +470,19 @@
 	uint16_t* st_b = (uint16_t*)(loff + nvb + 1);
 	uint16_t* st_idx = st_b + NIT;
 	V* st_val = (V*)(((uintptr_t)(st_idx + NIT) + 15) & ~(uintptr_t)15);
-	for (uint32_t j = threadIdx.x; j < nvb; j += blockDim.x) {
-		const uint32_t vb = lv.vb_base[l] + j;
-		cur[j] = lo_vb[vb] + cur_t[(size_t)chunk * n_vb + vb];
-		lh[j] = 0;
+	if constexpr (INL) {
+		block_exclusive_scan<SC_ST>(tot + lv.vb_base[l], loff, nvb, wsum);
+		const uint32_t level_items = a.n * NC * (l - lv.nd);
+		for (uint32_t j = threadIdx.x; j < nvb; j += blockDim.x) {
+			cur[j] = level_items + loff[j] + cur_t[(size_t)chunk * n_vb + lv.vb_base[l] + j];
+			lh[j] = 0;
+		}
+	} else {
+		for (uint32_t j = threadIdx.x; j < nvb; j += blockDim.x) {
+			const uint32_t vb = lv.vb_base[l] + j;
+			cur[j] = lo_vb[vb] + cur_t[(size_t)chunk * n_vb + vb];
+			lh[j] = 0;
+		}
 	}
 	__syncthreads();
 	const uint32_t off_l = c.offsets[l];
@@ -747,7 +801,103 @@
 	}
 }
 
-template <uint32_t F, uint32_t MODE>
+template <uint32_t D, uint32_t F, uint32_t FT>
+__device__ __forceinline__ void direct_samples(const GridConst& c, const GridBwdArgs& a, uint32_t l, uint32_t i0, uint32_t i1, uint32_t f0,
+                                               uint32_t t0, uint32_t TE, unsigned long long* acc) {
+	typedef typename ValVec<F>::T V;
+	constexpr uint32_t NC = 1u << D, U = 2;
+	const uint32_t TEP = TE + 1, off_l = c.offsets[l] + t0, rot = threadIdx.x % FT;
+	for (uint32_t ib = i0 + threadIdx.x; ib < i1; ib += blockDim.x * U) {
+		float x[U][D], g[U][FT];
+		bool active[U];
+#pragma unroll
+		for (uint32_t u = 0; u < U; ++u) {
+			const uint32_t i = min(ib + u * blockDim.x, i1 - 1);
+			load_pos<D>(a, i, x[u]);
+			const float ml = (a.max_level_per_sample ? a.max_level_per_sample[i] : a.max_level) * (float)c.n_levels;
+			active[u] = !((float)l > ml + 1e-3f) && ib + u * blockDim.x < i1;
+			if (a.dy_layout == AoS) {
+				const V gv = *(const V*)(a.dL_dy + (size_t)i * a.dy_stride + l * F);
+#pragma unroll
+				for (uint32_t f = 0; f < FT; ++f) {
+					if constexpr (F == 1) g[u][f] = (float)gv;
+					else {
+						float t = (float)gv[f];
+#pragma unroll
+						for (uint32_t q = 1; q < F / FT; ++q) t = f0 == q * FT ? (float)gv[q * FT + f] : t;
+						g[u][f] = t;
+					}
+				}
+			} else {
+#pragma unroll
+				for (uint32_t f = 0; f < FT; ++f) g[u][f] = (float)a.dL_dy[(size_t)(l * F + f0 + f) * a.dy_stride + i];
+			}
+		}
+#pragma unroll
+		for (uint32_t u = 0; u < U; ++u) {
+			if (!active[u]) continue;
+			float frac[D]; uint32_t base[D];
+			level_setup<D>(c, l, x[u], frac, base);
+			uint32_t cidx[NC];
+			corner_indices<D>(c, l, base, cidx);
+#pragma unroll
+			for (uint32_t k = 0; k < NC; ++k) {
+				const uint32_t e = cidx[k] - off_l;
+				if (e >= TE) continue;
+				const float w = corner_weight<D>(frac, k);
+#pragma unroll
+				for (uint32_t q = 0; q < FT; ++q) {
+					const uint32_t f = (q + rot) & (FT - 1);
+					float gf = g[u][0];
+#pragma unroll
+					for (uint32_t r = 1; r < FT; ++r) gf = f == r ? g[u][r] : gf;
+					const float v = (float)to_f16(w * gf);
+#if NGP_ACC_SKIP0
+					if (v != 0.f) atomicAdd(&acc[f * TEP + e], (unsigned long long)(long long)(v * FIX_SCALE));
+#else
+					atomicAdd(&acc[f * TEP + e], (unsigned long long)(long long)(v * FIX_SCALE));
+#endif
+				}
+			}
+		}
+	}
+}
+
+template <uint32_t D, uint32_t F>
+__device__ __forceinline__ void accumulate_direct(const GridConst& c, const Levels& lv, const GridBwdArgs& a, uint32_t B, uint32_t x,
+                                                  unsigned long long* acc, unsigned long long* __restrict__ scratch) {
+	const uint32_t nd_b = lv.vb_base[lv.nd], v = x % nd_b, r = x / nd_b, NE = 1u << B;
+	uint32_t l = 0;
+	while (lv.vb_base[l + 1] <= v) ++l;
+	const uint32_t nb = lv.vb_base[l + 1] - lv.vb_base[l], sub = v - lv.vb_base[l], n_l = c.offsets[l + 1] - c.offsets[l];
+	const uint32_t i0 = min(r * lv.dS, a.n), i1 = min(i0 + lv.dS, a.n);
+	if (i0 >= i1) return;
+	const size_t pstride = (size_t)NE * F;
+	if constexpr (F >= 2) {
+		if (nb == 2) {
+			constexpr uint32_t FH = F / 2;
+			const uint32_t TEP = n_l + 1, f0 = sub * FH;
+			for (uint32_t k = threadIdx.x; k < TEP * FH; k += blockDim.x) acc[k] = 0ull;
+			__syncthreads();
+			direct_samples<D, F, FH>(c, a, l, i0, i1, f0, 0u, n_l, acc);
+			__syncthreads();
+			for (uint32_t k = threadIdx.x; k < n_l * FH; k += blockDim.x) {
+				const uint32_t f = k / n_l, e = k % n_l, b = e >> B;
+				scratch[((size_t)(lv.vb_base[l] + b) * lv.dP + r) * pstride + (size_t)(f0 + f) * NE + (e & (NE - 1))] = acc[f * TEP + e];
+			}
+			return;
+		}
+	}
+	const uint32_t t0 = sub << B, TE = min(NE, n_l - t0), TEP = TE + 1;
+	for (uint32_t k = threadIdx.x; k < TEP * F; k += blockDim.x) acc[k] = 0ull;
+	__syncthreads();
+	direct_samples<D, F, F>(c, a, l, i0, i1, 0u, t0, TE, acc);
+	__syncthreads();
+	unsigned long long* dst = scratch + ((size_t)v * lv.dP + r) * pstride;
+	for (uint32_t k = threadIdx.x; k < TE * F; k += blockDim.x) dst[(size_t)(k / TE) * NE + k % TE] = acc[(k / TE) * TEP + k % TE];
+}
+
+template <uint32_t F, uint32_t MODE, uint32_t DD = 0, bool INL = false>
 __global__ void __launch_bounds__(SC_BT) k_sc_accumulate(const GridConst c, const Levels lv, const BrickConst bk, const GridBwdArgs a,
                                                          const uint32_t* __restrict__ tot,
                                                          const uint32_t* __restrict__ lo_arr, uint32_t B, uint32_t split_limit,
@@ -755,28 +905,56 @@
                                                          const f16* __restrict__ item_val, f16* __restrict__ grad, bool overwrite,
                                                          const uint32_t* __restrict__ split, unsigned long long* __restrict__ scratch,
                                                          uint32_t debug, const FusedAdam fa, const BrickFallback fb, uint32_t vb_off,
-                                                         uint32_t part_lo, uint32_t part_hi) {
+                                                         uint32_t part_lo, uint32_t part_hi, uint32_t n_direct, uint32_t inline_part) {
+	if constexpr (!INL) inline_part = 0u;
 	constexpr bool FUSED = MODE == SC_FUSED_ADAM, G32 = MODE == SC_STORE_F32;
 	extern __shared__ unsigned long long acc[];
+	__shared__ PlanShared psh;
 	const uint32_t NE = 1u << B, NEP = NE + 1;
-	if (blockIdx.x < max_parts) {
-		if (blockIdx.x >= split[0]) return;
-		const uint32_t* d = split + 2 + 3 * (size_t)blockIdx.x;
-		if (d[0] < part_lo || d[0] >= part_hi) return;
-		const uint32_t lo = d[1], hi = d[2];
-		if (d[0] - bk.vb0 < bk.NBK) {
-			accumulate_brick<F>(c, bk, a, d[0] - bk.vb0, lo, hi, item_idx, item_val, acc, scratch + (size_t)blockIdx.x * NE * F, NE, fb);
+	uint32_t bx = blockIdx.x;
+	if constexpr (DD != 0) {
+		if (bx < n_direct) {
+			accumulate_direct<DD, F>(c, lv, a, B, bx, acc, scratch);
+			return;
+		}
+		bx -= n_direct;
+	}
+	if (bx < max_parts) {
+		const uint32_t slot = bx + lv.vb_base[lv.nd] * lv.dP;
+		uint32_t pvb, lo, hi;
+		if (inline_part) {
+			if (threadIdx.x == 0) psh.res[0] = ~0u;
+			plan_scan(tot, lv.vb_base[c.n_levels], split_limit, inline_part, lv.vb_base[lv.nd] * lv.dP, 0u, psh,
+			          [&](uint32_t vb, uint32_t t, uint32_t lo_b, uint32_t first, uint32_t, uint32_t np) {
+				          if (slot - first < np) {
+					          const uint32_t q = slot - first;
+					          psh.res[0] = vb; psh.res[1] = lo_b + q * inline_part; psh.res[2] = min(lo_b + (q + 1) * inline_part, lo_b + t);
+				          }
+			          });
+			__syncthreads();
+			pvb = __builtin_amdgcn_readfirstlane(psh.res[0]); lo = __builtin_amdgcn_readfirstlane(psh.res[1]);
+			hi = __builtin_amdgcn_readfirstlane(psh.res[2]);
+			if (pvb == ~0u) return;
+		} else {
+			if (slot >= split[0]) return;
+			const uint32_t* d = split + 2 + 3 * (size_t)slot;
+			pvb = d[0]; lo = d[1]; hi = d[2];
+		}
+		if (pvb < part_lo || pvb >= part_hi) return;
+		if (pvb - bk.vb0 < bk.NBK) {
+			accumulate_brick<F>(c, bk, a, pvb - bk.vb0, lo, hi, item_idx, item_val, acc, scratch + (size_t)slot * NE * F, NE, fb);
 			return;
 		}
 		for (uint32_t k = threadIdx.x; k < NEP * F; k += blockDim.x) acc[k] = 0ull;
 		__syncthreads();
 		if (!(debug & 1)) accumulate_items<F>(acc, NE, lo, hi, item_idx, item_val, debug);
 		__syncthreads();
-		unsigned long long* dst = scratch + (size_t)blockIdx.x * NE * F;
+		unsigned long long* dst = scratch + (size_t)slot * NE * F;
 		for (uint32_t k = threadIdx.x; k < NE * F; k += blockDim.x) dst[k] = acc[(k / NE) * NEP + k % NE];
 		return;
 	}
-	const uint32_t vb = blockIdx.x - max_parts + vb_off;
+	const uint32_t vb = bx - max_parts + vb_off;
+	if (vb < lv.vb_base[lv.nd]) return;
 	if (vb - bk.vb0 < bk.NBK) return;
 	const uint32_t t = tot[vb];
 	if (t > split_limit) return;
@@ -788,7 +966,12 @@
 			for (uint32_t k = threadIdx.x; k < n_e * F / 2; k += blockDim.x) store_pair<G32>(grad, fa.g32, (size_t)e0 * F / 2 + k, 0.f, 0.f);
 		return;
 	}
-	const uint32_t lo = lo_arr[vb];
+	uint32_t lo;
+	if (inline_part) {
+		uint32_t l = 0;
+		while (lv.vb_base[l + 1] <= vb) ++l;
+		lo = plan_bucket_lo(tot, lv.level_items * (l - lv.nd), lv.vb_base[l], vb, psh);
+	} else lo = lo_arr[vb];
 	for (uint32_t k = threadIdx.x; k < NEP * F; k += blockDim.x) acc[k] = 0ull;
 	__syncthreads();
 	if (!(debug & 1)) accumulate_items<F>(acc, NE, lo, lo + t, item_idx, item_val, debug);
@@ -843,14 +1026,16 @@
 	}
 }
 
-template <uint32_t F, uint32_t MODE>
+template <uint32_t F, uint32_t MODE, bool INL = false>
 __global__ void __launch_bounds__(SC_THREADS) k_sc_split_reduce(const GridConst c, const Levels lv, uint32_t B,
                                                                 const uint32_t* __restrict__ split, const uint32_t* __restrict__ splitb,
                                                                 const unsigned long long* __restrict__ scratch, f16* __restrict__ grad,
                                                                 bool overwrite, const SlabJob sj, uint32_t slab_x0, const FusedAdam fa,
                                                                 const BrickConst bk, const uint32_t* __restrict__ bp, const BrickFallback fb,
-                                                                uint32_t fin_x0, uint32_t part_lo, uint32_t part_hi) {
+                                                                uint32_t fin_x0, uint32_t part_lo, uint32_t part_hi,
+                                                                const uint32_t* __restrict__ tot, uint32_t split_limit, uint32_t inline_part) {
 	static_assert(SC_THREADS == SLAB_THREADS, "slab blocks share the split-reduce block shape");
+	if constexpr (!INL) inline_part = 0u;
 	constexpr bool FUSED = MODE == SC_FUSED_ADAM, G32 = MODE == SC_STORE_F32;
 	if (blockIdx.x >= fin_x0) {
 		constexpr uint32_t EPT = F == 1 ? 2 : 1;
@@ -916,8 +1101,27 @@
 		lazy_update(st, cfg, step, fa.mlp_n, G);
 		return;
 	}
-	if (blockIdx.x >= split[1]) return;
-	const uint32_t vb = splitb[3 * blockIdx.x], first = splitb[3 * blockIdx.x + 1], parts = splitb[3 * blockIdx.x + 2];
+	uint32_t vb, first, parts;
+	if (inline_part) {
+		const uint32_t nd_b = lv.vb_base[lv.nd];
+		if (blockIdx.x < nd_b) { vb = blockIdx.x; first = vb * lv.dP; parts = lv.dP; }
+		else {
+			__shared__ PlanShared psh;
+			if (threadIdx.x == 0) psh.res[0] = ~0u;
+			const uint32_t want = blockIdx.x;
+			plan_scan(tot, lv.vb_base[c.n_levels], split_limit, inline_part, nd_b * lv.dP, nd_b, psh,
+			          [&](uint32_t b, uint32_t, uint32_t, uint32_t first_b, uint32_t sb, uint32_t np) {
+				          if (np && sb == want) { psh.res[0] = b; psh.res[1] = first_b; psh.res[2] = np; }
+			          });
+			__syncthreads();
+			vb = __builtin_amdgcn_readfirstlane(psh.res[0]); first = __builtin_amdgcn_readfirstlane(psh.res[1]);
+			parts = __builtin_amdgcn_readfirstlane(psh.res[2]);
+			if (vb == ~0u) return;
+		}
+	} else {
+		if (blockIdx.x >= split[1]) return;
+		vb = splitb[3 * blockIdx.x]; first = splitb[3 * blockIdx.x + 1]; parts = splitb[3 * blockIdx.x + 2];
+	}
 	if (vb < part_lo || vb >= part_hi) return;
 	const uint32_t NE = 1u << B;
 	uint32_t e0, n_e;
@@ -958,8 +1162,9 @@
 	return (size_t)(3 * max_lb + 1) * 4 + nit * 4 + 16 + nit * F * 2;
 }
 
-Levels make_levels(const GridDesc& g, uint32_t B, const BrickConst& bk) {
+Levels make_levels(const GridDesc& g, uint32_t B, const BrickConst& bk, uint32_t nd = 0, uint32_t dS = 0, uint32_t dP = 0) {
 	Levels lv{};
+	lv.nd = nd; lv.dS = dS; lv.dP = dP;
 	uint32_t vb = 0;
 	for (uint32_t l = 0; l < g.n_levels; ++l) {
 		lv.vb_base[l] = vb;
@@ -967,6 +1172,11 @@
 		else if (!(l >= bk.LB && l < bk.LD)) vb += (g.offsets[l + 1] - g.offsets[l] + (1u << B) - 1) >> B;
 	}
 	for (uint32_t l = g.n_levels; l <= 32; ++l) lv.vb_base[l] = vb;
+	return lv;
+}
+Levels make_levels(const GridDesc& g, const ScatterPlan& p) {
+	Levels lv = make_levels(g, p.B, p.bk, p.direct_levels, p.direct_part, p.direct_parts);
+	lv.level_items = g.n_levels > p.direct_levels ? (uint32_t)(p.n_items / (g.n_levels - p.direct_levels)) : 0u;
 	return lv;
 }
 
@@ -985,13 +1195,15 @@
 	const BrickFallback fb{(unsigned long long*)(ws + p.off_fb), (uint32_t*)(ws + p.off_fb + (size_t)c.offsets[p.bk.LD] * c.n_features * 8)};
 	const size_t lds_s = scatter_lds_bytes(p.max_lb, p.spb, D, F);
 	const uint32_t xcd_map = p.xcd_map;
-	const uint32_t n_slots = c.n_levels - (p.bk.LD - p.bk.LB) + (p.bk.LD ? 1u : 0u);
+	const uint32_t n_slots = c.n_levels - (p.bk.LD - p.bk.LB) + (p.bk.LD ? 1u : 0u) - p.direct_levels;
+	const uint32_t n_direct = p.direct_buckets * p.direct_parts;
+	const uint32_t inline_part = p.plan_inline ? p.part : 0u;
 	const dim3 grid_s(xcd_map ? (uint32_t)div_round_up(p.n_chunks, 8) * 8 * n_slots : p.n_chunks * n_slots);
 	auto go = [&](auto scatter, auto accum, auto splitr) {
 		ensure_dynamic_lds((const void*)scatter, lds_s);
-		if (!(debug & 4))
+		if (!(debug & 4) && n_slots)
 			scatter<<<grid_s, p.spb == 512 ? 512 : 1024, lds_s, s>>>(c, lv, p.bk, a, p.B, p.n_buckets, p.n_chunks, xcd_map, cur_t, lo, idx, val,
-			                                                          debug);
+			                                                          debug, p.plan_inline ? tot : nullptr);
 		NGP_HIP(hipGetLastError());
 		const size_t lds_a = ((size_t)8 << p.B) * c.n_features + SC_LDS_PAD_BYTES + (fa.rec ? SC_LIST_BYTES : 0);
 		ensure_dynamic_lds((const void*)accum, lds_a);
@@ -1003,13 +1215,13 @@
 		const size_t fin_threads = c.n_features == 1 ? div_round_up(fin_entries, 2) : fin_entries;
 		const uint32_t fin_x = (uint32_t)div_round_up(div_round_up(fin_threads, SC_THREADS), gy);
 		if (!parted) {
-			accum<<<p.max_split_blocks + p.n_buckets, p.bt, lds_a, s>>>(c, lv, p.bk, a, tot, lo, p.B, p.split_limit, p.max_split_blocks,
-			                                                             idx, val, a.grad, overwrite, split, scratch, debug, fa, fb, 0u,
-			                                                             0u, ~0u);
+			accum<<<n_direct + p.max_split_blocks + p.n_buckets, p.bt, lds_a, s>>>(c, lv, p.bk, a, tot, lo, p.B, p.split_limit,
+			                                                                        p.max_split_blocks, idx, val, a.grad, overwrite, split, scratch,
+			                                                                        debug, fa, fb, 0u, 0u, ~0u, n_direct, inline_part);
 			NGP_HIP(hipGetLastError());
 			const dim3 grid_r(p.max_split_buckets + slab_x + fin_x, gy);
 			splitr<<<grid_r, SC_THREADS, 0, s>>>(c, lv, p.B, split, splitb, scratch, a.grad, overwrite, sj, p.max_split_buckets, fa, p.bk, bp,
-			                                     fb, p.max_split_buckets + slab_x, 0u, ~0u);
+			                                     fb, p.max_split_buckets + slab_x, 0u, ~0u, tot, p.split_limit, inline_part);
 			NGP_HIP(hipGetLastError());
 			return;
 		}
@@ -1019,14 +1231,15 @@
 			const uint32_t v0 = j ? std::min(parts->vb_end[j - 1], p.n_buckets) : 0u;
 			const uint32_t v1 = j + 1 == parts->k ? p.n_buckets : std::min(parts->vb_end[j], p.n_buckets);
 			NGP_CHECK(v0 <= v1, "grid backward parts: bucket ranges out of order");
-			accum<<<p.max_split_blocks + (v1 - v0), p.bt, lds_a, s>>>(c, lv, p.bk, a, tot, lo, p.B, p.split_limit, p.max_split_blocks,
-			                                                           idx, val, a.grad, overwrite, split, scratch, debug, fa, fb, v0,
-			                                                           v0, v1);
+			const uint32_t nd_j = jj == 0 ? n_direct : 0u;
+			accum<<<nd_j + p.max_split_blocks + (v1 - v0), p.bt, lds_a, s>>>(c, lv, p.bk, a, tot, lo, p.B, p.split_limit, p.max_split_blocks,
+			                                                                  idx, val, a.grad, overwrite, split, scratch, debug, fa, fb, v0,
+			                                                                  v0, v1, nd_j, inline_part);
 			NGP_HIP(hipGetLastError());
 			const uint32_t sx = j == 0 ? slab_x : 0u;
 			const dim3 grid_r(p.max_split_buckets + sx, gy);
 			splitr<<<grid_r, SC_THREADS, 0, s>>>(c, lv, p.B, split, splitb, scratch, a.grad, overwrite, sj, p.max_split_buckets, fa, p.bk, bp,
-			                                     fb, p.max_split_buckets + sx, v0, v1);
+			                                     fb, p.max_split_buckets + sx, v0, v1, tot, p.split_limit, inline_part);
 			NGP_HIP(hipGetLastError());
 			if (parts->after) parts->after(parts->user, j, s);
 		}
@@ -1035,21 +1248,33 @@
 		if (p.spb == 512) go(sc512, accum, splitr);
 		else go(sc1024, accum, splitr);
 	};
-#define NGP_SC_F(FF)                                                                                                 \
-	if (fa.rec) by_chunk(k_sc_scatter<D, FF, 512, 512>, k_sc_scatter<D, FF, 1024, 1024>, k_sc_accumulate<FF, SC_FUSED_ADAM>, \
-	                     k_sc_split_reduce<FF, SC_FUSED_ADAM>);                                                      \
-	else if (fa.g32) by_chunk(k_sc_scatter<D, FF, 512, 512>, k_sc_scatter<D, FF, 1024, 1024>,                       \
-	                          k_sc_accumulate<FF, SC_STORE_F32>, k_sc_split_reduce<FF, SC_STORE_F32>);              \
-	else by_chunk(k_sc_scatter<D, FF, 512, 512>, k_sc_scatter<D, FF, 1024, 1024>, k_sc_accumulate<FF, SC_STORE_F16>,  \
-	              k_sc_split_reduce<FF, SC_STORE_F16>)
+#define NGP_SC_K(FF, MM, DDD, II)                                                                                                 \
+	by_chunk(k_sc_scatter<D, FF, 512, 512, II>, k_sc_scatter<D, FF, 1024, 1024, II>, k_sc_accumulate<FF, MM, DDD, II>,            \
+	         k_sc_split_reduce<FF, MM, II>)
+#define NGP_SC_M(FF, MM)                                     \
+	if (n_direct && p.plan_inline) NGP_SC_K(FF, MM, D, true); \
+	else if (n_direct) NGP_SC_K(FF, MM, D, false);            \
+	else if (p.plan_inline) NGP_SC_K(FF, MM, 0, true);        \
+	else NGP_SC_K(FF, MM, 0, false)
+#define NGP_SC_F(FF)                                   \
+	if (fa.rec) { NGP_SC_M(FF, SC_FUSED_ADAM); }       \
+	else if (fa.g32) { NGP_SC_M(FF, SC_STORE_F32); }   \
+	else { NGP_SC_M(FF, SC_STORE_F16); }
 	switch (F) {
 		case 1: NGP_SC_F(1); break;
 		case 2: NGP_SC_F(2); break;
 		case 4: NGP_SC_F(4); break;
-		case 8: NGP_SC_F(8); break;
-		default: throw Error("grid backward: unsupported F");
-	}
+		default: break;
+	}
+#undef NGP_SC_M
+#define NGP_SC_M(FF, MM)                                \
+	if (p.plan_inline) NGP_SC_K(FF, MM, 0, true);       \
+	else NGP_SC_K(FF, MM, 0, false)
+	if (F == 8) { NGP_SC_F(8); }
+	else if (F != 1 && F != 2 && F != 4) throw Error("grid backward: unsupported F");
 #undef NGP_SC_F
+#undef NGP_SC_M
+#undef NGP_SC_K
 }
 
 static BrickConst make_bricks(const GridDesc& g, uint32_t n, uint32_t B, uint32_t brick_part) {
@@ -1111,7 +1336,7 @@
 
 }
 
-ScatterPlan make_scatter_plan(const GridDesc& g, uint32_t n, bool bricks) {
+ScatterPlan make_scatter_plan(const GridDesc& g, uint32_t n, bool bricks, bool direct, bool plan_inline) {
 	ScatterPlan p;
 	const uint32_t F = g.n_features;
 	p.B = 0;
@@ -1120,12 +1345,25 @@
 	while (((size_t)2 << p.B) * F * 8 <= lds_budget && p.B < 16) ++p.B;
 	if (const char* e = getenv("NGP_SC_BRICK_PART")) p.brick_part = std::max(1, atoi(e));
 	if (bricks) p.bk = make_bricks(g, n, p.B, p.brick_part);
-	const Levels lv = make_levels(g, p.B, p.bk);
+	p.direct_part = 16384;
+	if (const char* e = getenv("NGP_SC_DIRECT")) direct = atoi(e) != 0;
+	if (direct && !p.bk.LD && n > 0 && F <= 4) {
+		if (const char* e = getenv("NGP_SC_DIRECT_PART")) p.direct_part = (uint32_t)std::max(1, atoi(e));
+		while (p.direct_levels < g.n_levels && g.offsets[p.direct_levels + 1] - g.offsets[p.direct_levels] <= (2u << p.B)) {
+			p.direct_mask |= 1u << p.direct_levels;
+			++p.direct_levels;
+		}
+		p.direct_parts = p.direct_levels ? (uint32_t)div_round_up(n, p.direct_part) : 0u;
+	}
+	const Levels lv = make_levels(g, p.B, p.bk, p.direct_levels, p.direct_part, p.direct_parts);
+	p.direct_buckets = lv.vb_base[p.direct_levels];
 	p.n_buckets = lv.vb_base[g.n_levels];
+	if (const char* e = getenv("NGP_SC_PLAN_INLINE")) plan_inline = atoi(e) != 0;
+	p.plan_inline = plan_inline && !p.bk.LD && p.n_buckets <= SC_PLAN_THREADS;
 	p.max_lb = p.bk.NBK;
 	for (uint32_t l = 0; l < g.n_levels; ++l) p.max_lb = std::max(p.max_lb, lv.vb_base[l + 1] - lv.vb_base[l]);
 	NGP_CHECK((size_t)p.max_lb * 4 <= 32 * 1024, "grid backward: level too large for the bucket histogram");
-	const uint64_t items_per_sample = ((uint64_t)(g.n_levels - (p.bk.LD - p.bk.LB)) << g.n_dims) + (p.bk.LD ? 1u : 0u);
+	const uint64_t items_per_sample = ((uint64_t)(g.n_levels - (p.bk.LD - p.bk.LB) - p.direct_levels) << g.n_dims) + (p.bk.LD ? 1u : 0u);
 	p.spb = 512;
 	if (512ull * items_per_sample < 16ull * p.n_buckets && scatter_lds_bytes(p.max_lb, 1024, g.n_dims, F) <= 160 * 1024) p.spb = 1024;
 	if (const char* e = getenv("NGP_SC_CHUNK")) p.spb = (uint32_t)atoi(e);
@@ -1140,7 +1378,8 @@
 	if (const char* e = getenv("NGP_SC_LIMIT")) p.split_limit = (uint32_t)atoi(e);
 	p.max_split_blocks = (uint32_t)(div_round_up(p.n_items, (uint64_t)p.part) + div_round_up(p.n_items, (uint64_t)p.split_limit) + 1);
 	if (p.bk.LD) p.max_split_blocks += (uint32_t)(std::min<uint64_t>(p.bk.NBK, n) + div_round_up((uint64_t)n, (uint64_t)p.brick_part));
-	p.max_split_buckets = (uint32_t)(div_round_up(p.n_items, (uint64_t)p.split_limit) + 1);
+	p.max_split_buckets = (uint32_t)(div_round_up(p.n_items, (uint64_t)p.split_limit) + 1) + p.direct_buckets;
+	const size_t n_slots = (size_t)p.direct_buckets * p.direct_parts + p.max_split_blocks;
 	p.xcd_map = 2;
 	if (const char* e = getenv("NGP_SC_XCD")) p.xcd_map = (uint32_t)atoi(e);
 	p.bt = F == 2 ? 512 : 1024;
@@ -1153,10 +1392,10 @@
 	p.off_cur = align(p.off_hist + len * 4);
 	p.off_tot = align(p.off_cur + len * 4);
 	p.off_split = align(p.off_tot + (size_t)p.n_buckets * 4);
-	p.off_lo = align(p.off_split + (2 + 3 * (size_t)p.max_split_blocks) * 4);
+	p.off_lo = align(p.off_split + (2 + 3 * n_slots) * 4);
 	p.off_splitb = align(p.off_lo + (size_t)p.n_buckets * 4);
 	p.off_scratch = align(p.off_splitb + 3 * (size_t)p.max_split_buckets * 4);
-	p.off_idx = align(p.off_scratch + (size_t)p.max_split_blocks * ((size_t)1 << p.B) * g.n_features * 8);
+	p.off_idx = align(p.off_scratch + n_slots * ((size_t)1 << p.B) * g.n_features * 8);
 	p.off_val = align(p.off_idx + p.n_items * 2);
 	p.off_bp = align(p.off_val + p.n_items * F * 2);
 	p.off_fb = align(p.off_bp + (size_t)p.bk.NBK * 8);
@@ -1166,12 +1405,13 @@
 
 bool scatter_hist(const GridDesc& g, const ScatterPlan& p, void* workspace, GridHist& h) {
 	if ((size_t)p.n_buckets * 4 > 48 * 1024 || p.spb != 512) return false;
-	const Levels lv = make_levels(g, p.B, p.bk);
+	const Levels lv = make_levels(g, p);
 	h.hist = (uint32_t*)((char*)workspace + p.off_hist);
 	h.B = p.B; h.n_chunks = p.n_chunks; h.chunk = p.spb;
 	for (int l = 0; l <= 32; ++l) h.vb_base[l] = lv.vb_base[l];
 	h.brick_first = p.bk.LB; h.brick_levels = p.bk.LD; h.n_bricks = p.bk.NBK; h.brick_cells = p.bk.K; h.bricks_per_dim = p.bk.NB;
 	h.brick_vb0 = p.bk.vb0;
+	h.direct_levels = p.direct_levels;
 	return true;
 }
 
@@ -1181,7 +1421,7 @@
 	uint32_t* hist = (uint32_t*)(ws + p.off_hist);
 	if (!hist_done) {
 		const GridConst c = make_grid_const(g);
-		const Levels lv = make_levels(g, p.B, p.bk);
+		const Levels lv = make_levels(g, p);
 		const dim3 grid_h(p.n_chunks, g.n_levels);
 		const size_t lds_h = (size_t)p.max_lb * 4;
 		auto go = [&](auto k3, auto k2) {
@@ -1194,16 +1434,18 @@
 	}
 	k_sc_scan<<<div_round_up(p.n_buckets, 64), 64 * SCAN_SEG, 0, s>>>(hist, p.n_chunks, p.n_buckets, (uint32_t*)(ws + p.off_cur), (uint32_t*)(ws + p.off_tot));
 	NGP_HIP(hipGetLastError());
+	if (p.plan_inline) return;
 	const auto plan = p.n_buckets <= SC_PLAN_THREADS ? k_sc_plan<1> : p.n_buckets <= 8 * SC_PLAN_THREADS ? k_sc_plan<8> : k_sc_plan<32>;
 	plan<<<1, SC_PLAN_THREADS, 0, s>>>((const uint32_t*)(ws + p.off_tot), p.n_buckets, p.split_limit, p.part,
 	                                        (uint32_t*)(ws + p.off_lo), (uint32_t*)(ws + p.off_split), (uint32_t*)(ws + p.off_splitb),
 	                                        p.bk.vb0, p.bk.NBK, p.brick_part, (uint32_t*)(ws + p.off_bp),
-	                                        p.bk.LD ? (uint32_t*)(ws + p.off_fb + (size_t)g.offsets[p.bk.LD] * g.n_features * 8) : nullptr);
+	                                        p.bk.LD ? (uint32_t*)(ws + p.off_fb + (size_t)g.offsets[p.bk.LD] * g.n_features * 8) : nullptr,
+	                                        p.direct_buckets, p.direct_parts);
 	NGP_HIP(hipGetLastError());
 }
 
 uint32_t scatter_bucket_at_param(const GridDesc& g, const ScatterPlan& p, uint64_t param) {
-	const Levels lv = make_levels(g, p.B, p.bk);
+	const Levels lv = make_levels(g, p);
 	for (uint32_t vb = 0; vb < p.n_buckets; ++vb) {
 		uint32_t l = 0;
 		while (lv.vb_base[l + 1] <= vb) ++l;
@@ -1221,7 +1463,7 @@
 	NGP_CHECK(!parts || !parts->k || (!p.bk.LD && !(fused && fused->rec) && parts->k <= BwdParts::MAX),
 	          "grid backward parts: not with bricks or the fused update");
 	const GridConst c = make_grid_const(g);
-	const Levels lv = make_levels(g, p.B, p.bk);
+	const Levels lv = make_levels(g, p);
 	const FusedAdam fa = fused ? *fused : FusedAdam{};
 	if (g.n_dims == 3) launch_backward<3>(g.n_features, c, lv, b, p, (char*)workspace, s, overwrite, debug, slab, fa, parts);
 	else launch_backward<2>(g.n_features, c, lv, b, p, (char*)workspace, s, overwrite, debug, slab, fa, parts);
```

After: 1.761 billion samples/s (median of 6 runs). +6.4%, better.
